# ZenGo-X/multi-party-ecdsa

Hardware: AMD Instinct MI355X
Metric: GG20 signatures/sec (t=1, n=3; all parties of each session on the node's GPUs) + Paillier-2048 modexp/s per GPU (higher is better)
Workload: dtype u32 limbs (radix 2^29) / u64 accumulators

## Files before the change

### multi_party_ecdsa_amd/csrc/mpe_gg20.h

```cpp
#pragma once
#include <cstdio>
#include <cstdlib>

#include "mpe_gg20_msg.h"
#include "mpe_gg20_nonces.h"
#include "mpe_proofs.h"

namespace mpe {
namespace smp {
struct Bounds { uint32_t *q, *q3, *Nm2, *qNt, *q3Nt; };
__global__ void bounds_kernel(int count, const uint32_t* __restrict__ N, const uint32_t* __restrict__ Nt, Bounds b) {
  const int g = blockIdx.x * blockDim.x + threadIdx.x;
  if (g > count) return;
  const uint32_t q[8] = {0xD0364141u, 0xBFD25E8Cu, 0xAF48A03Bu, 0xBAAEDCE6u, 0xFFFFFFFEu, 0xFFFFFFFFu, 0xFFFFFFFFu, 0xFFFFFFFFu};
  uint32_t q2[16], q3[24];
  sm::mul(q2, q, 8, q, 8);
  sm::mul(q3, q2, 16, q, 8);
  if (g == count) {
    for (int j = 0; j < 8; ++j) b.q[j] = q[j];
    for (int j = 0; j < 24; ++j) b.q3[j] = q3[j];
    return;
  }
  const uint32_t two[1] = {2u};
  sm::sub(b.Nm2 + (size_t)g * 64, 64, N + (size_t)g * 64, 64, two, 1);
// ... 668 lines not shown
  int st = 0;
  for (int li = 0; li < L; ++li) { const int s = pst[(size_t)li * B + b]; if (s && (!st || s < st)) st = s; }
  const size_t o = (size_t)b0 + b;
  for (int j = 0; j < 8; ++j) { r_out[o * 8 + j] = st ? 0u : pr[(size_t)b * 8 + j]; s_out[o * 8 + j] = st ? 0u : ps[(size_t)b * 8 + j]; }
  recid_out[o] = st ? 0 : prec[b];
  if (R_out) for (int j = 0; j < 16; ++j) R_out[o * 16 + j] = pR[(size_t)b * 16 + j];
  status[o] = st;
}

enum class PdlStage { idle, first_queued, ready };
struct Ahead {
  bool lockstep = false;
  uint32_t* cinv = nullptr;
  uint8_t* cinv_ok = nullptr; bool cinv_done = false;
  uint32_t* ped = nullptr;
  uint32_t *pdl_bn = nullptr, *pdl_scratch = nullptr;
  PdlStage pdl = PdlStage::idle;
};

}
}

struct mpe_gg20_session {
  mpe_ctx* ctx = nullptr;
  const mpe_gg20_keys* K = nullptr;
  int B = 0, L = 0, dedup = 0, next_round = 0;
  bool tweaked = false;
  bool any_set = false;
  uint32_t *tw = nullptr, *ty = nullptr, *tgw = nullptr;
  bool failed = false;
  mpe::gg::Dim d{};
  mpe_gg20_nonces Z{};
  void* mem = nullptr;
  size_t mem_bytes = 0;
  bool from_cache = false;
  mpe::gg::Idx ix{};
  uint32_t *kq = nullptr, *gq = nullptr, *w = nullptr, *k64 = nullptr, *g_gamma = nullptr, *com = nullptr, *c_a = nullptr, *beta = nullptr;
  uint32_t *ca_all = nullptr, *com_all = nullptr, *bpk_in = nullptr, *delta_i = nullptr, *sigma_i = nullptr, *lq = nullptr, *pedT = nullptr;
  uint32_t *tvec = nullptr, *dinv = nullptr, *R = nullptr, *Rbar = nullptr, *mq = nullptr, *rq = nullptr, *s_i = nullptr, *bad = nullptr;
  uint32_t *sig_r = nullptr, *sig_s = nullptr;
  uint32_t* miu = nullptr;
  int32_t *status = nullptr, *sig_recid = nullptr;
  int32_t *sub0_vi = nullptr, *sub4_pv = nullptr, *rdash_pv = nullptr;
  uint8_t *ok_vi = nullptr, *ok_pv = nullptr;
  mpe::gg::Ahead ahead{};
  int fault_step = 0;
  uint32_t fault_mask = 0;
  char* tmp = nullptr;
  size_t tmp_bytes = 0;
};

namespace mpe {
namespace gg {

static void gg_trace(const mpe_ctx* ctx, hipStream_t st, const char* what, int rc) {
  if (!ctx->gg20_trace) return;
  const hipError_t e = hipStreamSynchronize(st);
  fprintf(stderr, "[gg20] %-28s rc=%d sync=%s\n", what, rc, hipGetErrorString(e));
  fflush(stderr);
}
#define GG_LAUNCH(kernel, nitems, ...)                                                                   \
  do {                                                                                                    \
    if (rc == MPE_OK && (nitems) > 0)                                                                     \
      hipLaunchKernelGGL(kernel, dim3(blocks_for((int)(nitems), 64)), dim3(64), 0, st, __VA_ARGS__);      \
    gg_trace(s->ctx, st, #kernel, rc);                                                                            \
  } while (0)

static Counts counts_of(const Dim& d) { return counts_of(d.B, d.S, d.n, d.L, d.V, d.PV); }
static void dim_of_keys(Dim& d, const mpe_gg20_keys* K, const int32_t* d_keyset, const int32_t* d_sigset) {
  d.S = K->S; d.n = K->n; d.K = K->K; d.n_own = K->n_own; d.ks = d_keyset;
  d.ss = d_sigset; d.sets = K->d_sets; d.sg4 = K->sets4[0]; d.nsets = K->nsets; d.lparty = -1;
  for (int i = 0; i < 8; ++i) { d.sg[i] = K->signers[i]; d.oslot[i] = K->own_slot[i] < 0 ? 0 : K->own_slot[i]; }
}
static int local_parties(Dim& d, const mpe_gg20_keys* K, int n_local, const int32_t* h_local, const int32_t* d_sigset, int by_party) {
  if (n_local < 1 || n_local > K->S || !h_local) return MPE_E_ARG;
  d.L = n_local;
  for (int i = 0; i < 8; ++i) d.loc[i] = 0;
  if (by_party) {
    if (n_local != 1) { mpe_set_error_msg("gg20: one local party by index"); return MPE_E_ARG; }
    const int p = h_local[0];
    if (p < 0 || p >= K->n || K->own_slot[p] < 0) { mpe_set_error_msg("gg20: the local party's secrets are not in the key object"); return MPE_E_ARG; }
    if (d_sigset) { d.lparty = p; return MPE_OK; }
    for (int i = 0; i < K->S; ++i) if (K->signers[i] == p) { d.loc[0] = i; return MPE_OK; }
    mpe_set_error_msg("gg20: the local party is not a signer"); return MPE_E_ARG;
  }
  for (int i = 0; i < n_local; ++i) {
    if (h_local[i] < 0 || h_local[i] >= K->S || (i && h_local[i] <= h_local[i - 1])) return MPE_E_ARG;
    d.loc[i] = h_local[i];
    for (int k = 0; k < (d_sigset ? K->nsets : 1); ++k)
      if (K->own_slot[(K->sets4[k] >> (4 * h_local[i])) & 15u] < 0) { mpe_set_error_msg("gg20: a local party's secrets are not in the key object"); return MPE_E_ARG; }
  }
  return MPE_OK;
}
static bool small_batch(const mpe_ctx* ctx, size_t items) { return ctx->allow_par && items <= (size_t)ctx->par_items; }
static size_t ec_lanes_fit(const mpe_ctx* ctx) { return ctx->ec_lane_groups ? (size_t)ctx->cus * 4 * 64 * 2 / ctx->device_share : 0; }
static size_t layout(mpe_gg20_session* s, char* base) {
  const Dim& d = s->d;
  const Counts c = counts_of(d);
  Bump m(base);
  Idx& x = s->ix;
  x.kown_pi = m.i(c.nPI);
  x.pi_ap = m.i(c.nAP); x.kown_ap = m.i(c.nAP); x.st_ap = m.i(c.nAP);
  x.ca_vi = m.i(c.nVI); x.kpub_vi = m.i(c.nVI); x.st_vi = m.i(c.nVI);
  x.ca_mb = m.i(c.nMB); x.kpub_mb = m.i(c.nMB); x.kown_mb = m.i(c.nMB);
  x.pi_pp = m.i(c.nPP); x.kown_pp = m.i(c.nPP); x.st_pp = m.i(c.nPP);
  x.ca_pv = m.i(c.nPV); x.pi_pv = m.i(c.nPV); x.kpub_pv = m.i(c.nPV); x.st_pv = m.i(c.nPV);
  if (s->tweaked) { s->tw = m.w((size_t)d.B * 8); s->ty = m.w((size_t)d.B * 16); s->tgw = m.w((size_t)d.B * d.S * 16); }
  s->kq = m.w(c.nPI * 8); s->gq = m.w(c.nPI * 8); s->w = m.w(c.nPI * 8); s->k64 = m.w(c.nPI * 64);
  s->g_gamma = m.w(c.nPI * 16); s->com = m.w(c.nPI * 8); s->c_a = m.w(c.nPI * 128); s->beta = m.w(c.nMB * 8);
  s->ca_all = m.w(c.SB * 128); s->com_all = m.w(c.SB * 8); s->bpk_in = m.w(c.nPP * 16);
  s->delta_i = m.w(c.nPI * 8); s->sigma_i = m.w(c.nPI * 8); s->lq = m.w(c.nPI * 8); s->pedT = m.w(c.nPI * 16);
  s->tvec = m.w(c.SB * 16); s->dinv = m.w(c.nPI * 8); s->R = m.w(c.nPI * 16); s->Rbar = m.w(c.nPI * 16);
  s->mq = m.w(c.nPI * 8); s->rq = m.w(c.nPI * 8); s->s_i = m.w(c.nPI * 8); s->bad = m.w(c.nPI * NR);
  s->sig_r = m.w(c.nPI * 8); s->sig_s = m.w(c.nPI * 8); s->miu = m.w(c.nPP * 64);
  s->status = m.i(c.nPI * NR); s->sig_recid = m.i(c.nPI);
  s->sub0_vi = m.i(c.nVI); s->ok_vi = m.f(c.nVI); s->sub4_pv = m.i(c.nPV); s->rdash_pv = m.i(c.nPV); s->ok_pv = m.f(c.nPV);
  Ahead& a = s->ahead; const bool small = small_batch(s->ctx, c.nVI);
  a.cinv = small ? m.w(c.nVI * 128) : nullptr; a.cinv_ok = small ? m.f(c.nVI) : nullptr;
  a.ped = m.w(c.nPI * 48);
  a.pdl_bn = small ? m.w(c.nPP * 128) : nullptr; a.pdl_scratch = small ? m.w(modexp_nn_scratch_words(c.nPP)) : nullptr;
  s->tmp_bytes = tmp_bytes_of(c);
  s->tmp = (char*)m.take(s->tmp_bytes);
  return m.off;
}
static Slab slab_of(const mpe_gg20_session* s, const uint32_t* p, const int64_t* h_off, int round) {
  Slab sl;
  sl.p = p; sl.W = msg_words(s->d.S, s->d.n, round);
  for (int j = 0; j < 8; ++j) sl.off[j] = j < s->d.S ? (h_off ? (long long)h_off[j] : (long long)j * s->B) : 0;
  return sl;
}
static int round_enter(mpe_gg20_session* s, int round, const void* in, const void* out, bool need_in, bool need_out) {
  if (!s || (need_in && !in) || (need_out && !out)) return MPE_E_ARG;
  if (s->failed) { mpe_set_error_msg("gg20: a round call of this batch failed (or the batch was aborted): re-arm the session"); return MPE_E_ARG; }
  if (s->next_round != round) { mpe_set_error_msg("gg20: rounds must be run in order"); return MPE_E_ARG; }
  s->d.enc = s->ctx->enc;
  return MPE_OK;
}
static int round_exit(mpe_gg20_session* s, int rc, const char* what) {
  if (rc != MPE_OK) { s->failed = true; return rc; }
  const hipError_t e = hipGetLastError();
  if (e != hipSuccess) { s->failed = true; mpe_set_error(what, e); return MPE_E_HIP; }
  s->next_round++;
  return MPE_OK;
}
#define STAT(r) (s->status + (size_t)(r) * c.nPI)
#define BADR(r) (s->bad + (size_t)(r) * c.nPI)
#define PACK(nitems, per, nsub, sub0, subw, field, src)                                                                                 \
  GG_LAUNCH(pack_field_kernel, (size_t)(nitems) * (field).words, (int)(nitems), (int)(per), d.L, d.B, (int)(nsub), (int)(sub0), (int)(subw),   \
            (field).off, (const uint32_t*)(src), (field).words, s->status, s->next_round, d_out)

static bool round1_merges(const mpe_ctx* ctx, const Counts& c) {
  const bool par = small_batch(ctx, c.nVI);
  const size_t resident_groups = (size_t)ctx->cus * ctx->modexp_waves_per_cu * 16 / ctx->device_share;
  return ctx->merge_r1 && ctx->use_pair && ctx->use_multiexp && c.nVI > 0 && c.nMB > 0 && c.nVI + c.nMB < ((size_t)1 << 30) &&
         (!par || 4 * (c.nVI + c.nMB) > (size_t)ctx->merge_r1_quarters * resident_groups);
}
__global__ void ca_all_from_local_kernel(int S, int B, const uint32_t* __restrict__ c_a, uint32_t* __restrict__ ca_all) {
  const size_t g = (size_t)blockIdx.x * blockDim.x + threadIdx.x;
  if (g >= (size_t)S * B * 128) return;
  const int w = (int)(g % 128);
  const size_t jb = g / 128;
  const int ind = (int)(jb / B), b = (int)(jb % B);
  ca_all[g] = c_a[((size_t)b * S + ind) * 128 + w];
}

static bool pdl_ahead_eligible(const mpe_gg20_session* s, const Counts& c) {
  const mpe_ctx* ctx = s->ctx; const Ahead& a = s->ahead;
  return a.lockstep && a.pdl_bn && ctx->use_prio && !ctx->no_pdl_ahead && ctx->use_pair && ctx->use_crt && ctx->use_pown && c.nPP > 0 && small_batch(ctx, c.nPP);
}
static int pdl_ahead_queue(mpe_gg20_session* s, const Counts& c, bool finish) {
  mpe_ctx* ctx = s->ctx; const mpe_paillier* prv = s->K->prv; Ahead& a = s->ahead; hipStream_t sa = ctx->aux[1];
  const int phase = !finish ? 1 : (a.pdl == PdlStage::first_queued ? 2 : 0);
  const int keep = ctx->ladder_prio;
  ctx->ladder_prio = 0;
  const int rc = modexp_nn(ctx, prv, (int)c.nPP, sel_of(s->ix.kown_pp, prv->nkeys), rows(s->Z.pdl_beta, 64, nullptr, 64),
                           tab_rows(prv->N, 64, s->ix.kown_pp, prv->nkeys), 64, true, a.pdl_bn, sa, true, a.pdl_scratch, phase);
  ctx->ladder_prio = keep;
  if (rc == MPE_OK && !finish) a.pdl = PdlStage::first_queued;
  else if (rc == MPE_OK) { (void)hipEventRecord(ctx->ev_ahead, sa); a.pdl = PdlStage::ready; }
  gg_trace(ctx, sa, finish ? "PDL beta^N, ahead" : "PDL beta^N, first ladder, ahead", rc);
  return rc;
}
static Handed pdl_ahead_take(const mpe_gg20_session* s) { return s->ahead.pdl == PdlStage::ready ? Handed{s->ahead.pdl_bn, s->ctx->ev_ahead} : Handed{}; }
static void pdl_ahead_consumed(mpe_gg20_session* s) { if (s->ahead.pdl == PdlStage::ready) s->ahead.pdl = PdlStage::idle; }
static void ahead_drain(mpe_gg20_session* s, hipStream_t st) {
  mpe_ctx* ctx = s->ctx; Ahead& a = s->ahead;
  if (a.pdl == PdlStage::idle) return;
  if (a.pdl == PdlStage::first_queued) (void)hipEventRecord(ctx->ev_ahead, ctx->aux[1]);
  (void)hipStreamWaitEvent(st, ctx->ev_ahead, 0);
  a.pdl = PdlStage::idle;
}

static int round0(mpe_gg20_session* s, uint32_t* d_out, hipStream_t st) {
  int rc = round_enter(s, 0, nullptr, d_out, false, true);
  if (rc != MPE_OK) return rc;
  mpe_ctx* ctx = s->ctx; const mpe_gg20_keys* K = s->K; const Dim& d = s->d; const Counts c = counts_of(d); const mpe_gg20_nonces& Z = s->Z; Ahead& a = s->ahead;
  const int n = d.n;
  (void)hipMemsetAsync(d_out, 0, c.nPI * (size_t)msg_words(d.S, n, 0) * 4, st);
  const bool par = small_batch(ctx, c.nAP);
  const size_t nXN = c.nPI + c.nAP;
  bool all_local_in_order = d.L == d.S;
  for (int l = 0; l < d.L && all_local_in_order; ++l) all_local_in_order = d.loc[l] == l;
  const bool ahead = par && a.lockstep && a.cinv && all_local_in_order && !ctx->no_r1_inversion_ahead && round1_merges(ctx, c);
  a.cinv_done = false;
  if (par && rc == MPE_OK) rc = ws_begin(ctx, st);
  const bool held = par && rc == MPE_OK;
  WsHold hold(ctx->ws, held);
  const uint32_t *rn_pre = nullptr, *bn_pre = nullptr;
  Fork g(ctx, st, 2, held, 2);
  GG_LAUNCH(r0_kernel, c.nPI, d, K->x, Z.k, Z.gamma, Z.blind, s->kq, s->gq, s->w, s->k64, s->g_gamma, s->com, STAT(0), BADR(0));
  if (g.on) (void)hipEventRecord(ctx->ev_fork[0], st);
  GG_LAUNCH(ped_ahead_kernel, c.nPI, d, Z.l, Z.ped_s1, Z.ped_s2, a.ped);
  hipEvent_t xn_ready = nullptr;
  if (held && ctx->merge_xn) {
    hipStream_t sx = g.s(1);
    uint32_t* xs = ws_array<uint32_t>(ctx, nXN * 64);
    uint32_t* xn = ws_array<uint32_t>(ctx, nXN * 128);
    int32_t* kx = ws_array<int32_t>(ctx, nXN);
    rc = ws_ok(ctx);
    if (rc == MPE_OK) {
      (void)hipMemcpyAsync(xs, Z.r_a, c.nPI * 64 * 4, hipMemcpyDeviceToDevice, sx);
      (void)hipMemcpyAsync(xs + c.nPI * 64, Z.al_beta, c.nAP * 64 * 4, hipMemcpyDeviceToDevice, sx);
      (void)hipMemcpyAsync(kx, s->ix.kown_pi, c.nPI * 4, hipMemcpyDeviceToDevice, sx);
      (void)hipMemcpyAsync(kx + c.nPI, s->ix.kown_ap, c.nAP * 4, hipMemcpyDeviceToDevice, sx);
      rc = modexp_nn(ctx, K->prv, (int)nXN, key_selector(K->prv, kx), rows(xs, 64, nullptr, 64), key_rows(K->prv, K->prv->N, 64, kx), 64, true, xn, sx, true);
      rn_pre = xn; bn_pre = xn + c.nPI * 128;
      if (rc == MPE_OK && g.on) { (void)hipEventRecord(ctx->ev_mid, sx); xn_ready = ctx->ev_mid; }
    }
  }
  if (g.on) (void)hipStreamWaitEvent(g.s(1), ctx->ev_fork[0], 0);
  if (rc == MPE_OK) rc = paillier_encrypt(ctx, K->prv, (int)c.nPI, s->ix.kown_pi, s->k64, Z.r_a, s->c_a, true, g.s(1), rn_pre);
  gg_trace(s->ctx, st, "encrypt k", rc);
  hipEvent_t c_ready = nullptr;
  if (ahead && held && g.on && xn_ready && rc == MPE_OK) {
    hipStream_t sx = g.s(1);
    (void)hipEventRecord(ctx->ev_mid, sx); c_ready = ctx->ev_mid;
    hipLaunchKernelGGL(ca_all_from_local_kernel, dim3((unsigned)((c.SB * 128 + 255) / 256)), dim3(256), 0, sx, d.S, d.B, s->c_a, s->ca_all);
    Seq q{ctx, sx, (int)c.nVI};
    const Rows ksel = sel_of(s->ix.kpub_vi, K->pub->nkeys);
    uint8_t* ok = q.flags();
    uint32_t* cred = q.modmul(K->pub->ms_nn, ksel, rows(s->ca_all, 128, s->ix.ca_vi), rows(K->pub->ms_nn->one_words, 0, nullptr, 1));
    uint32_t* cinv = q.modinv(K->pub->ms_nn, ksel, rows(cred, 128), ok);
    rc = q.rc;
    if (rc == MPE_OK) {
      (void)hipMemcpyAsync(a.cinv, cinv, c.nVI * 128 * 4, hipMemcpyDeviceToDevice, sx);
      (void)hipMemcpyAsync(a.cinv_ok, ok, c.nVI, hipMemcpyDeviceToDevice, sx);
      a.cinv_done = true;
    }
    gg_trace(s->ctx, sx, "round 1's inversion, ahead", rc);
  }
  Bump t(s->tmp);
  const Round0Tmp r0 = Round0Tmp::carve(t, c);
  mpe_alice_proof ap{r0.z, r0.e, r0.s, r0.s1, r0.s2};
  mpe_alice_nonces an{Z.al_alpha, Z.al_beta, Z.al_gamma, Z.al_rho};
  if (rc == MPE_OK)
    rc = alice_generate(ctx, K->prv, K->stm, (int)c.nAP, s->ix.kown_ap, s->ix.st_ap, rows(s->kq, 8, s->ix.pi_ap),
                        rows(s->c_a, 128, s->ix.pi_ap), rows(Z.r_a, 64, s->ix.pi_ap), &an, &ap, st, &g, Handed{bn_pre, c_ready ? c_ready : xn_ready}, c_ready);
  g.join();
  if (rc == MPE_OK && c_ready && pdl_ahead_eligible(s, c)) { (void)hipStreamWaitEvent(ctx->aux[1], c_ready, 0); rc = pdl_ahead_queue(s, c, false); }
  gg_trace(s->ctx, st, "alice_generate", rc);
  PACK(c.nAP, n, n + 1, 0, SUB0, M0A.z, ap.z); PACK(c.nAP, n, n + 1, 0, SUB0, M0A.e, ap.e); PACK(c.nAP, n, n + 1, 0, SUB0, M0A.s, ap.s);
  PACK(c.nAP, n, n + 1, 0, SUB0, M0A.s1, ap.s1); PACK(c.nAP, n, n + 1, 0, SUB0, M0A.s2, ap.s2);
  PACK(c.nPI, 1, n + 1, n, SUB0, M0L.c, s->c_a); PACK(c.nPI, 1, n + 1, n, SUB0, M0L.com, s->com);
  return round_exit(s, rc, "gg20 round0");
}

__global__ void gather_rows_kernel(int n, Rows src, int src_words, int words, uint32_t* __restrict__ dst) {
  const size_t g = (size_t)blockIdx.x * blockDim.x + threadIdx.x;
  if (g >= (size_t)n * words) return;
  const int w = (int)(g % words), i = (int)(g / words);
  dst[g] = w < src_words ? row_of(src, i)[w] : 0u;
}
static int round1_merged_ladders(mpe_ctx* ctx, const mpe_paillier* pk, size_t nVI, const int32_t* kpub_vi, Rows cipher_vi, Rows s_vi, Rows e_vi,
                                 size_t nMB, const int32_t* kpub_mb, Rows ca_mb, const uint32_t* bsel, const uint32_t* mb_r,
                                 const uint32_t** m_vi, const uint8_t** inv_ok_vi, const uint32_t** x_mb, hipStream_t st,
                                 Handed cinv_pre = {}, const uint8_t* cinv_ok_pre = nullptr) {
  const size_t n = nVI + nMB;
  Seq q{ctx, st, (int)nVI};
  const Rows ksel = sel_of(kpub_vi, pk->nkeys);
  const uint8_t* inv_ok = cinv_ok_pre;
  const uint32_t* cinv = cinv_pre.p;
  cinv_pre.wait(st);
  if (!cinv_pre) {
    uint8_t* ok = q.flags();
    uint32_t* cred = q.modmul(pk->ms_nn, ksel, cipher_vi, rows(pk->ms_nn->one_words, 0, nullptr, 1));
    cinv = q.modinv(pk->ms_nn, ksel, rows(cred, 128), ok);
    inv_ok = ok;
  }
  if (q.rc != MPE_OK) return q.rc;
  uint32_t* b1 = ws_array<uint32_t>(ctx, n * 64);
  uint32_t* b2 = ws_array<uint32_t>(ctx, n * 128);
  uint32_t* e2 = ws_array<uint32_t>(ctx, n * 8);
  int32_t* key = ws_array<int32_t>(ctx, n);
  uint32_t* out = ws_array<uint32_t>(ctx, n * 128);
  MPE_TRY(ws_ok(ctx));
  auto gather = [&](size_t cnt, Rows src, int sw, int words, uint32_t* dst) {
    if (cnt) hipLaunchKernelGGL(gather_rows_kernel, dim3((unsigned)((cnt * words + 255) / 256)), dim3(256), 0, st, (int)cnt, src, sw, words, dst);
  };
  gather(nVI, s_vi, 64, 64, b1);              gather(nMB, rows(mb_r, 64), 64, 64, b1 + nVI * 64);
  gather(nVI, rows(cinv, 128), 128, 128, b2); gather(nMB, ca_mb, 128, 128, b2 + nVI * 128);
  gather(nVI, e_vi, 8, 8, e2);                gather(nMB, rows(bsel, 8), 8, 8, e2 + nVI * 8);
  (void)hipMemcpyAsync(key, kpub_vi, nVI * 4, hipMemcpyDeviceToDevice, st);
  (void)hipMemcpyAsync(key + nVI, kpub_mb, nMB * 4, hipMemcpyDeviceToDevice, st);
  MPE_TRY(modexp_nn2(ctx, pk, (int)n, key_selector(pk, key), rows(b1, 64, nullptr, 64), key_rows(pk, pk->N, 64, key), 64, rows(b2, 128), rows(e2, 8), 8, out, st));
  *m_vi = out; *inv_ok_vi = inv_ok; *x_mb = out + nVI * 128;
  return MPE_OK;
}

static int round1(mpe_gg20_session* s, const uint32_t* d_in, const int64_t* h_off, uint32_t* d_out, hipStream_t st) {
  int rc = round_enter(s, 1, d_in, d_out, true, true);
  if (rc != MPE_OK) return rc;
  mpe_ctx* ctx = s->ctx; const mpe_gg20_keys* K = s->K; const Dim& d = s->d; const Counts c = counts_of(d); const mpe_gg20_nonces& Z = s->Z;
  const int n = d.n, P1 = d.S - 1;
  const Slab in0 = slab_of(s, d_in, h_off, 0);
  (void)hipMemsetAsync(d_out, 0, c.nPI * (size_t)msg_words(d.S, n, 1) * 4, st);
  GG_LAUNCH(gather_field_kernel, c.SB * M0L.c.words, in0, d.S, d.B, n * SUB0 + M0L.c.off, M0L.c.words, s->ca_all);
  GG_LAUNCH(gather_field_kernel, c.SB * M0L.com.words, in0, d.S, d.B, n * SUB0 + M0L.com.off, M0L.com.words, s->com_all);
  Bump t(s->tmp);
  int32_t* sub0_vi = s->sub0_vi;
  uint8_t* ok_vi = s->ok_vi;
  const Round1Tmp r1 = Round1Tmp::carve(t, c);
  uint32_t *bsel = r1.bsel, *btq = r1.btq, *c_b = r1.c_b;
  uint32_t *Bpk = r1.Bpk, *BR = r1.BR, *Bz = r1.Bz, *BTpk = r1.BTpk, *BTR = r1.BTR, *BTz = r1.BTz;
  GG_LAUNCH(idx1_kernel, c.nVI, d, in0, sub0_vi);
  const bool par = small_batch(ctx, c.nVI);
  const bool merged = round1_merges(ctx, c);
  const bool ahead = merged && s->ahead.cinv_done;
  s->ahead.cinv_done = false;
  if ((par || merged) && rc == MPE_OK) rc = ws_begin(ctx, st);
  const bool held = (par || merged) && rc == MPE_OK;
  WsHold hold(ctx->ws, held);
  const uint32_t *m_vi = nullptr, *x_mb = nullptr;
  const uint8_t* inv_ok_vi = nullptr;
  AliceProofRows pr{rows(d_in + M0A.z.off, SUB0, sub0_vi), rows(d_in + M0A.e.off, SUB0, sub0_vi), rows(d_in + M0A.s.off, SUB0, sub0_vi),
                    rows(d_in + M0A.s1.off, SUB0, sub0_vi), rows(d_in + M0A.s2.off, SUB0, sub0_vi)};
  if (rc == MPE_OK && c.nMB > 0)
    hipLaunchKernelGGL(mb_prep_kernel, dim3(blocks_for((int)c.nMB, 64)), dim3(64), 0, st, d, s->gq, s->w, Z.mb_beta_tag, bsel, btq, s->beta);
  Fork g(ctx, st, 2, held && par, 2);
  hipEvent_t m_ready = nullptr;
  auto dlog_proofs = [&](hipStream_t sd) {
    if (rc != MPE_OK || c.nMB == 0) return;
    hipLaunchKernelGGL(dlog_prove_kernel, dim3(blocks_for((int)c.nMB, 64)), dim3(64), 0, sd, (int)c.nMB, ctx->enc, bsel, Z.mb_nonce_b, Bpk, BR, Bz);
    hipLaunchKernelGGL(dlog_prove_kernel, dim3(blocks_for((int)c.nMB, 64)), dim3(64), 0, sd, (int)c.nMB, ctx->enc, btq, Z.mb_nonce_bt, BTpk, BTR, BTz);
  };
  const bool dlog_first = ahead && g.on && !ctx->no_r1_dlog_first;
  if (dlog_first) dlog_proofs(st);
  {
    hipStream_t st2 = g.s(1);
    if (merged && rc == MPE_OK) {
      rc = round1_merged_ladders(ctx, K->pub, c.nVI, s->ix.kpub_vi, rows(s->ca_all, 128, s->ix.ca_vi), with_words(pr.s, 64), pr.e, c.nMB, s->ix.kpub_mb,
                                 rows(s->ca_all, 128, s->ix.ca_mb), bsel, Z.mb_r, &m_vi, &inv_ok_vi, &x_mb, st2,
                                 ahead ? Handed{s->ahead.cinv} : Handed{}, ahead ? s->ahead.cinv_ok : nullptr);
      if (rc == MPE_OK && g.on) { (void)hipEventRecord(ctx->ev_mid, st2); m_ready = ctx->ev_mid; }
      gg_trace(s->ctx, st2, "round 1 merged ladders", rc);
    }
    if (rc == MPE_OK)
      rc = paillier_mul_add_enc(ctx, K->pub, (int)c.nMB, s->ix.kpub_mb, rows(s->ca_all, 128, s->ix.ca_mb), rows(bsel, 8), 8, Z.mb_beta_tag,
                                Z.mb_r, c_b, st2, x_mb);
    gg_trace(s->ctx, st2, "MessageB ciphertext", rc);
    if (!dlog_first) dlog_proofs(st2);
  }
  if (rc == MPE_OK)
    rc = alice_verify(ctx, K->pub, K->stm, (int)c.nVI, s->ix.kpub_vi, s->ix.st_vi, rows(s->ca_all, 128, s->ix.ca_vi), pr, ok_vi, st, Handed{m_vi, m_ready}, inv_ok_vi);
  gg_trace(s->ctx, st, "alice_verify", rc);
  g.join();
  GG_LAUNCH(status1_kernel, c.nPI, d, ok_vi, STAT(1), BADR(1));
  const int per = 2 * P1;
  PACK(c.nMB, per, per, 0, SUB1, M1.c, c_b); PACK(c.nMB, per, per, 0, SUB1, M1.b_pk, Bpk); PACK(c.nMB, per, per, 0, SUB1, M1.b_R, BR);
  PACK(c.nMB, per, per, 0, SUB1, M1.b_z, Bz); PACK(c.nMB, per, per, 0, SUB1, M1.bt_pk, BTpk); PACK(c.nMB, per, per, 0, SUB1, M1.bt_R, BTR);
  PACK(c.nMB, per, per, 0, SUB1, M1.bt_z, BTz);
  return round_exit(s, rc, "gg20 round1");
}

static int round2(mpe_gg20_session* s, const uint32_t* d_in, const int64_t* h_off, uint32_t* d_out, hipStream_t st) {
  int rc = round_enter(s, 2, d_in, d_out, true, true);
  if (rc != MPE_OK) return rc;
  mpe_ctx* ctx = s->ctx; const mpe_gg20_keys* K = s->K; const Dim& d = s->d; const Counts c = counts_of(d); const mpe_gg20_nonces& Z = s->Z;
  const Slab in1 = slab_of(s, d_in, h_off, 1);
  (void)hipMemsetAsync(d_out, 0, c.nPI * (size_t)W2 * 4, st);
  GG_LAUNCH(validate_kernel, c.nPI, d, in1, 2, STAT(2), BADR(2));
  Bump t(s->tmp);
  const Round2Tmp r2 = Round2Tmp::carve(t, c);
  int32_t* sub1_rv = r2.sub1_rv;
  uint32_t *alpha_full = r2.alpha_full, *alpha = r2.alpha;
  uint8_t* code = r2.code;
  Ped ped{s->pedT, r2.e, r2.a1, r2.a2, r2.z1, r2.z2};
  GG_LAUNCH(idx2_kernel, c.nMB, d, in1, sub1_rv);
  const bool pdl_ahead = rc == MPE_OK && pdl_ahead_eligible(s, c) && ensure_aux(ctx);
  if (pdl_ahead) { (void)hipEventRecord(ctx->ev_fork[0], st); (void)hipStreamWaitEvent(ctx->aux[1], ctx->ev_fork[0], 0); }
  if (rc == MPE_OK)
    rc = paillier_decrypt(ctx, K->prv, (int)c.nMB, s->ix.kown_mb, rows(d_in + M1.c.off, SUB1, sub1_rv), alpha_full, st);
  gg_trace(s->ctx, st, "decrypt", rc);
  if (pdl_ahead && rc == MPE_OK) rc = pdl_ahead_queue(s, c, true);
  if (c.nMB * 4 <= ec_lanes_fit(ctx)) GG_LAUNCH(r2a_group_kernel, c.nMB * 4, d, sub1_rv, d_in, alpha_full, s->kq, K->gw, alpha, s->bpk_in, code);
  else GG_LAUNCH(r2a_kernel, c.nMB, d, sub1_rv, d_in, alpha_full, s->kq, K->gw, alpha, s->bpk_in, code);
  GG_LAUNCH(r2b_kernel, c.nPI, d, s->kq, s->gq, s->w, alpha, s->beta, code, Z.l, Z.ped_s1, Z.ped_s2, s->delta_i, s->sigma_i, s->lq, ped,
            STAT(2), BADR(2), alpha_full, s->miu, s->fault_step, s->fault_mask, s->ahead.ped);
  PACK(c.nPI, 1, 1, 0, W2, M2.delta, s->delta_i); PACK(c.nPI, 1, 1, 0, W2, M2.T, ped.T); PACK(c.nPI, 1, 1, 0, W2, M2.e, ped.e);
  PACK(c.nPI, 1, 1, 0, W2, M2.a1, ped.a1); PACK(c.nPI, 1, 1, 0, W2, M2.a2, ped.a2); PACK(c.nPI, 1, 1, 0, W2, M2.com, ped.T);
  PACK(c.nPI, 1, 1, 0, W2, M2.z1, ped.z1); PACK(c.nPI, 1, 1, 0, W2, M2.z2, ped.z2);
  return round_exit(s, rc, "gg20 round2");
}

static int round3(mpe_gg20_session* s, const uint32_t* d_in, const int64_t* h_off, uint32_t* d_out, hipStream_t st) {
  int rc = round_enter(s, 3, d_in, d_out, true, true);
  if (rc != MPE_OK) return rc;
  mpe_ctx* ctx = s->ctx; const Dim& d = s->d; const Counts c = counts_of(d);
  const Slab in2 = slab_of(s, d_in, h_off, 2);
  (void)hipMemsetAsync(d_out, 0, c.nPI * (size_t)W3 * 4, st);
  GG_LAUNCH(validate_kernel, c.nPI, d, in2, 3, STAT(3), BADR(3));
  GG_LAUNCH(gather_field_kernel, c.SB * M2.T.words, in2, d.S, d.B, M2.T.off, M2.T.words, s->tvec);
  const int g3 = 2 * d.S <= 4 ? 4 : (2 * d.S <= 8 ? 8 : 16);
  if (c.nPI * g3 <= ec_lanes_fit(ctx)) GG_LAUNCH(r3_group_kernel, c.nPI * g3, d, g3, in2, s->dinv, STAT(3), BADR(3));
  else GG_LAUNCH(r3_kernel, c.nPI, d, in2, s->dinv, STAT(3), BADR(3));
  PACK(c.nPI, 1, 1, 0, W3, M3.blind, s->Z.blind); PACK(c.nPI, 1, 1, 0, W3, M3.g_gamma, s->g_gamma);
  return round_exit(s, rc, "gg20 round3");
}

static int round4(mpe_gg20_session* s, const uint32_t* d_in, const int64_t* h_off, uint32_t* d_out, hipStream_t st) {
  int rc = round_enter(s, 4, d_in, d_out, true, true);
  if (rc != MPE_OK) return rc;
  mpe_ctx* ctx = s->ctx; const mpe_gg20_keys* K = s->K; const Dim& d = s->d; const Counts c = counts_of(d); const mpe_gg20_nonces& Z = s->Z;
  const int S = d.S, P1 = S - 1;
  const Slab in3 = slab_of(s, d_in, h_off, 3);
  (void)hipMemsetAsync(d_out, 0, c.nPI * (size_t)msg_words(S, d.n, 4) * 4, st);
  GG_LAUNCH(validate_kernel, c.nPI, d, in3, 4, STAT(4), BADR(4));
  Fork g(ctx, st, 2, small_batch(ctx, c.nPP), 2);
  hipEvent_t R_ready = nullptr;
  if (rc == MPE_OK && c.nPI > 0) {
    hipLaunchKernelGGL(r4_kernel, dim3(blocks_for((int)c.nPI, 64)), dim3(64), 0, g.s(1), d, in3, s->dinv, s->com_all, s->bpk_in, s->kq, s->R, s->Rbar,
                       STAT(4), BADR(4), g.on ? 0 : 1);
    if (g.on) {
      (void)hipEventRecord(ctx->ev_mid, g.s(1)); R_ready = ctx->ev_mid;
      hipLaunchKernelGGL(r4_rbar_kernel, dim3(blocks_for((int)c.nPI, 64)), dim3(64), 0, g.s(1), d, s->kq, s->R, s->Rbar);
    }
  }
  Bump t(s->tmp);
  const Round4Tmp r4 = Round4Tmp::carve(t, c);
  mpe_pdl_proof pp{r4.z, r4.u1, r4.u2, r4.u3, r4.s1, r4.s2, r4.s3};
  mpe_pdl_nonces pn{Z.pdl_alpha, Z.pdl_beta, Z.pdl_rho, Z.pdl_gamma};
  if (rc == MPE_OK)
    rc = pdl_prove(ctx, K->prv, K->stm, (int)c.nPP, s->ix.kown_pp, s->ix.st_pp, rows(s->c_a, 128, s->ix.pi_pp), rows(s->Rbar, 16, s->ix.pi_pp),
                   rows(s->R, 16, s->ix.pi_pp), rows(s->kq, 8, s->ix.pi_pp), rows(Z.r_a, 64, s->ix.pi_pp), &pn, &pp, st, &g,
                   pdl_ahead_take(s), R_ready);
  else g.join();
  if (rc == MPE_OK) pdl_ahead_consumed(s);
  gg_trace(s->ctx, st, "pdl_prove", rc);
  PACK(c.nPP, P1, S, 0, SUB4, M4P.z, pp.z); PACK(c.nPP, P1, S, 0, SUB4, M4P.u1, pp.u1); PACK(c.nPP, P1, S, 0, SUB4, M4P.u2, pp.u2);
  PACK(c.nPP, P1, S, 0, SUB4, M4P.u3, pp.u3); PACK(c.nPP, P1, S, 0, SUB4, M4P.s1, pp.s1); PACK(c.nPP, P1, S, 0, SUB4, M4P.s2, pp.s2);
  PACK(c.nPP, P1, S, 0, SUB4, M4P.s3, pp.s3);
  PACK(c.nPI, 1, S, P1, SUB4, M4R.R_dash, s->Rbar);
  return round_exit(s, rc, "gg20 round4");
}

static int round5(mpe_gg20_session* s, const uint32_t* d_in, const int64_t* h_off, uint32_t* d_out, hipStream_t st) {
  int rc = round_enter(s, 5, d_in, d_out, true, true);
  if (rc != MPE_OK) return rc;
  mpe_ctx* ctx = s->ctx; const mpe_gg20_keys* K = s->K; const Dim& d = s->d; const Counts c = counts_of(d); const mpe_gg20_nonces& Z = s->Z;
  const Slab in4 = slab_of(s, d_in, h_off, 4);
  (void)hipMemsetAsync(d_out, 0, c.nPI * (size_t)W5 * 4, st);
  GG_LAUNCH(validate_kernel, c.nPI, d, in4, 5, STAT(5), BADR(5));
  Bump t(s->tmp);
  int32_t *sub4_pv = s->sub4_pv, *rdash_pv = s->rdash_pv;
  uint8_t* ok_pv = s->ok_pv;
  const Round5Tmp r5 = Round5Tmp::carve(t, c);
  Heg heg{r5.S, r5.T, r5.A3, r5.z1, r5.z2};
  GG_LAUNCH(idx5_kernel, c.nPV, d, in4, sub4_pv, rdash_pv);
  const bool par = small_batch(ctx, c.nPV);
  PdlProofRows pr{rows(d_in + M4P.z.off, SUB4, sub4_pv), rows(d_in + M4P.u1.off, SUB4, sub4_pv), rows(d_in + M4P.u2.off, SUB4, sub4_pv),
                  rows(d_in + M4P.u3.off, SUB4, sub4_pv), rows(d_in + M4P.s1.off, SUB4, sub4_pv), rows(d_in + M4P.s2.off, SUB4, sub4_pv),
                  rows(d_in + M4P.s3.off, SUB4, sub4_pv)};
  Fork g(ctx, st, 2, par, 2);
  if (rc == MPE_OK && c.nPI > 0)
    hipLaunchKernelGGL(r5_prove_kernel, dim3(blocks_for((int)c.nPI, 64)), dim3(64), 0, g.s(1), d, s->R, s->sigma_i, s->lq, s->pedT, Z.heg_s1, Z.heg_s2, heg);
  if (rc == MPE_OK)
    rc = pdl_verify(ctx, K->pub, K->stm, (int)c.nPV, s->ix.kpub_pv, s->ix.st_pv, rows(s->ca_all, 128, s->ix.ca_pv), rows(d_in + M4R.R_dash.off, SUB4, rdash_pv),
                    rows(s->R, 16, s->ix.pi_pv), pr, ok_pv, st);
  gg_trace(s->ctx, st, "pdl_verify", rc);
  g.join();
  GG_LAUNCH(r5_status_kernel, c.nPI, d, in4, ok_pv, STAT(5), BADR(5));
  PACK(c.nPI, 1, 1, 0, W5, M5.S, heg.S); PACK(c.nPI, 1, 1, 0, W5, M5.T, heg.T); PACK(c.nPI, 1, 1, 0, W5, M5.A3, heg.A3);
  PACK(c.nPI, 1, 1, 0, W5, M5.z1, heg.z1); PACK(c.nPI, 1, 1, 0, W5, M5.z2, heg.z2);
  return round_exit(s, rc, "gg20 round5");
}

static int round6(mpe_gg20_session* s, const uint32_t* d_in, const int64_t* h_off, hipStream_t st) {
  int rc = round_enter(s, 6, d_in, nullptr, true, false);
  if (rc != MPE_OK) return rc;
  mpe_ctx* ctx = s->ctx; const Dim& d = s->d; const Counts c = counts_of(d);
  const Slab in5 = slab_of(s, d_in, h_off, 5);
  GG_LAUNCH(validate_kernel, c.nPI, d, in5, 6, STAT(6), BADR(6));
  const int g6 = 3 * d.S <= 8 ? 8 : (3 * d.S <= 16 ? 16 : 32);
  if (c.nPI * g6 <= ec_lanes_fit(ctx)) GG_LAUNCH(r6_group_kernel, c.nPI * g6, d, g6, in5, s->R, s->tvec, s->K->y, STAT(6), BADR(6));
  else GG_LAUNCH(r6_kernel, c.nPI, d, in5, s->R, s->tvec, s->K->y, STAT(6), BADR(6));
  return round_exit(s, rc, "gg20 round6");
}

static int round7(mpe_gg20_session* s, const uint32_t* d_msg, uint32_t* d_out, hipStream_t st) {
  int rc = round_enter(s, 7, d_msg, d_out, true, true);
  if (rc != MPE_OK) return rc;
  const Dim& d = s->d; const Counts c = counts_of(d);
  GG_LAUNCH(r7_kernel, c.nPI, d, d_msg, s->R, s->kq, s->sigma_i, s->mq, s->rq, s->s_i, s->fault_step, s->fault_mask);
  PACK(c.nPI, 1, 1, 0, W6, M7.s_i, s->s_i);
  return round_exit(s, rc, "gg20 round7");
}
static int complete(mpe_gg20_session* s, const uint32_t* d_in, const int64_t* h_off, hipStream_t st) {
  int rc = round_enter(s, 8, d_in, nullptr, true, false);
  if (rc != MPE_OK) return rc;
  const Dim& d = s->d; const Counts c = counts_of(d);
  const Slab in6 = slab_of(s, d_in, h_off, 7);
  GG_LAUNCH(complete_kernel, c.nPI, d, in6, s->R, s->mq, s->rq, s->s_i, s->K->y, s->status, s->bad, s->sig_r, s->sig_s, s->sig_recid);
  return round_exit(s, rc, "gg20 complete");
}

static void launch_idx(mpe_gg20_session* s, hipStream_t st) {
  const Counts c = counts_of(s->d);
  size_t total = 0;
  for (const size_t v : {c.nVI, c.nMB, c.nAP, c.nPV, c.nPI}) if (v > total) total = v;
  hipLaunchKernelGGL(idx_kernel, dim3(blocks_for((int)total, 64)), dim3(64), 0, st, s->d, s->ix, (int)total);
}
static void launch_tweaks(mpe_gg20_session* s, const uint32_t* d_tweak, hipStream_t st) {
  Dim& d = s->d;
  d.tw = d.ty = d.tgw = nullptr;
  if (!d_tweak) return;
  (void)hipMemcpyAsync(s->tw, d_tweak, (size_t)d.B * 32, hipMemcpyDeviceToDevice, st);
  hipLaunchKernelGGL(tweak_kernel, dim3(blocks_for(d.B * (d.S + 1), 64)), dim3(64), 0, st, d, s->tw, s->K->gw, s->K->y, s->tgw, s->ty);
  d.tw = s->tw; d.ty = s->ty; d.tgw = s->tgw;
}
static hipError_t wipe_batch_state(mpe_gg20_session* s, hipStream_t st) {
  ahead_drain(s, st);
  return hipMemsetAsync(s->kq, 0, (size_t)((char*)s->mem + s->mem_bytes - (char*)s->kq), st);
}

static void session_release(mpe_gg20_session* s, hipStream_t st) {
  if (!s) return;
  ahead_drain(s, st);
  if (s->mem) {
    (void)hipMemsetAsync(s->mem, 0, s->mem_bytes, st);
    if (s->from_cache) s->ctx->sess_in_use = false;
    else { (void)hipStreamSynchronize(st); (void)hipFree(s->mem); }
  }
  delete s;
}

}
}

extern "C" {

int mpe_gg20_keys_create(mpe_ctx* ctx, int t, int n, int n_signers, const int32_t* h_signers, int nkeysets, int n_own,
                         const int32_t* h_own, const uint32_t* d_x, const uint32_t* d_p, const uint32_t* d_q, const uint32_t* d_N,
                         const uint32_t* d_Nt, const uint32_t* d_h1, const uint32_t* d_h2, const uint32_t* d_y, const uint32_t* d_X,
                         mpe_gg20_keys** out, void* stream) {
  return mpe_gg20_keys_create_sets(ctx, t, n, n_signers, 1, h_signers, nkeysets, n_own, h_own, d_x, d_p, d_q, d_N, d_Nt, d_h1, d_h2, d_y, d_X, out, stream);
}

int mpe_gg20_keys_create_sets(mpe_ctx* ctx, int t, int n, int n_signers, int n_sets, const int32_t* h_sets, int nkeysets, int n_own,
                              const int32_t* h_own, const uint32_t* d_x, const uint32_t* d_p, const uint32_t* d_q, const uint32_t* d_N,
                              const uint32_t* d_Nt, const uint32_t* d_h1, const uint32_t* d_h2, const uint32_t* d_y, const uint32_t* d_X,
                              mpe_gg20_keys** out, void* stream) {
  const int32_t* h_signers = h_sets;
  if (!ctx || !h_signers || !h_own || !d_x || !d_p || !d_q || !d_N || !d_Nt || !d_h1 || !d_h2 || !d_y || !d_X || !out) return MPE_E_ARG;
  if (n < 2 || n > 8 || n_signers < 2 || n_signers > n || t < 1 || n_signers <= t || nkeysets < 1 || n_own < 1 || n_own > n) return MPE_E_ARG;
  if (n_sets < 1 || n_sets > 256) return MPE_E_ARG;
  uint32_t sets4[256], masks[256];
  for (int k = 0; k < n_sets; ++k) {
    const int32_t* row = h_sets + (size_t)k * n_signers;
    sets4[k] = 0; masks[k] = 0;
    for (int i = 0; i < n_signers; ++i) {
      if (row[i] < 0 || row[i] >= n || (i && row[i] <= row[i - 1])) return MPE_E_ARG;
      sets4[k] |= (uint32_t)row[i] << (4 * i); masks[k] |= 1u << row[i];
    }
    for (int m = 0; m < k; ++m) if (sets4[m] == sets4[k]) { mpe_set_error_msg("gg20 keys: two equal signer sets"); return MPE_E_ARG; }
  }
  for (int i = 0; i < n_own; ++i)
    if (h_own[i] < 0 || h_own[i] >= n || (i && h_own[i] <= h_own[i - 1])) return MPE_E_ARG;
  hipStream_t st = (hipStream_t)stream;
  mpe_gg20_keys* K = new (std::nothrow) mpe_gg20_keys();
  if (!K) return MPE_E_NOMEM;
  K->t = t; K->n = n; K->S = n_signers; K->K = nkeysets; K->n_own = n_own; K->nsets = n_sets;
  for (int k = 0; k < n_sets; ++k) { K->sets4[k] = sets4[k]; K->masks[k] = masks[k]; }
  for (int a = 0; a < 8; ++a) K->own_slot[a] = -1;
  for (int i = 0; i < n_signers; ++i) K->signers[i] = h_signers[i];
  for (int i = 0; i < n_own; ++i) { K->own[i] = h_own[i]; K->own_slot[h_own[i]] = i; }
  const size_t kk = (size_t)nkeysets;
  const size_t ngw = kk * n_sets * n_signers;
  const size_t words = kk * n_own * 8 + kk * n * 16 + kk * 16 + ngw * 16 + 32 + kk * n * (64 + 72 + 88) + 2 * (size_t)n_sets;
  hipError_t e = hipMalloc(&K->blob, words * 4);
  if (e != hipSuccess) { delete K; mpe_set_error("hipMalloc(gg20 keys)", e); return MPE_E_NOMEM; }
  K->blob_bytes = words * 4;
  K->x = (uint32_t*)K->blob; K->X = K->x + kk * n_own * 8; K->y = K->X + kk * n * 16; K->gw = K->y + kk * 16;
  K->bounds.q = K->gw + ngw * 16; K->bounds.q3 = K->bounds.q + 8; K->bounds.Nm2 = K->bounds.q3 + 24;
  K->bounds.qNt = K->bounds.Nm2 + kk * n * 64; K->bounds.q3Nt = K->bounds.qNt + kk * n * 72;
  K->d_sets = K->bounds.q3Nt + kk * n * 88;
  (void)hipMemcpyAsync(K->d_sets, K->sets4, (size_t)n_sets * 4, hipMemcpyHostToDevice, st);
  (void)hipMemcpyAsync(K->d_sets + n_sets, K->masks, (size_t)n_sets * 4, hipMemcpyHostToDevice, st);
  hipLaunchKernelGGL(mpe::smp::bounds_kernel, dim3(mpe::blocks_for(nkeysets * n + 1, 64)), dim3(64), 0, st, nkeysets * n, d_N, d_Nt, K->bounds);
  (void)hipMemcpyAsync(K->x, d_x, kk * n_own * 8 * 4, hipMemcpyDeviceToDevice, st);
  (void)hipMemcpyAsync(K->X, d_X, kk * n * 16 * 4, hipMemcpyDeviceToDevice, st);
  (void)hipMemcpyAsync(K->y, d_y, kk * 16 * 4, hipMemcpyDeviceToDevice, st);
  {
    mpe::gg::Dim d{};
    d.S = n_signers; d.n = n; d.K = nkeysets; d.nsets = n_sets; d.sets = K->d_sets; d.lparty = -1;
    hipLaunchKernelGGL(mpe::gg::gw_kernel, dim3(mpe::blocks_for((int)ngw, 64)), dim3(64), 0, st, d, K->X, K->gw);
  }
  int rc = mpe_paillier_create_public(ctx, nkeysets * n, d_N, &K->pub, stream);
  if (rc == MPE_OK) rc = mpe_paillier_create_private(ctx, nkeysets * n_own, d_p, d_q, &K->prv, stream);
// ... 282 lines not shown
```

### multi_party_ecdsa_amd/csrc/mpe_internal.h

```cpp
#pragma once
#include <hip/hip_runtime.h>
#include <stdint.h>
#include <new>
#include <utility>
#include <string>
#include <vector>

#include "../../include/mpecdsa_hip.h"
#include "mpe_kernels_heavy.h"
#include "mpe_sched.h"
#include "mpe_ws.h"

void mpe_set_error(const char* what, hipError_t e);
void mpe_set_error_msg(const char* what);

namespace mpe {
struct WsHip {
  static void* alloc(size_t bytes) {
    void* p = nullptr;
    const hipError_t e = hipMalloc(&p, bytes);
    if (e != hipSuccess) { mpe_set_error("hipMalloc(workspace)", e); return nullptr; }
    return p;
  }
  static void free(void* p) { (void)hipFree(p); }
  static void zero(void* p, size_t bytes, void* stream) { (void)hipMemsetAsync(p, 0, bytes, (hipStream_t)stream); }
  static void sync(void* stream) { (void)hipStreamSynchronize((hipStream_t)stream); }
};
}

struct mpe_ctx {
  int device = 0;
  int cus = 256;
  int fb_window_bits = 13;
  int window_bits = 0;
  bool ec_lane_groups = true;
  bool adaptive_lanes = true;
  bool use_pown = true;
  bool use_pair = true;
  bool use_multiexp = true;
  bool use_crt = true;
  bool use_fixed_base = true;
  bool use_sliding = true;
  int wide_div = 4;
  int device_share = 1;
  int xwide_div = 16;
  bool merge_xn = true;
  int use_prio = 1;
  int ladder_prio = 1;
  int use_crt_n = 1;
  int no_pdl_ahead = 0;
  int no_r1_dlog_first = 0;
  int no_r1_inversion_ahead = 0;
  int merge_r1_quarters = 1;
  bool merge_r1 = true;
  size_t fb_budget_bytes = 0;
  int modexp_waves_per_cu = 8;
  int fb_split = 0;
  int gg20_trace = 0;
  int safe_pass_log = 24;
  int sampler_max_attempts = 128;
  int no_primaries = 0;
  int no_elect = 0;
  int grid_mode = 2;
  void* tables[4] = {nullptr, nullptr, nullptr, nullptr};
  size_t tables_bytes[4] = {0, 0, 0, 0};
  hipStream_t aux[3] = {nullptr, nullptr, nullptr};
  hipEvent_t ev_fork[2] = {nullptr, nullptr}, ev_join[3] = {nullptr, nullptr, nullptr};
  hipEvent_t ev_ahead = nullptr;
  hipEvent_t ev_mid = nullptr;
  bool aux_ready = false;
  bool allow_par = true;
  int par_items = 32768;
  mpe::WsArena<mpe::WsHip> ws;
  void* sess_buf = nullptr;
  size_t sess_bytes = 0;
  bool sess_in_use = false;
  void* slab_buf = nullptr;
  size_t slab_bytes = 0;
  mpe_launch_info last = {};
  long long search_counts[9] = {0, 0, 0, 0, 0, 0, 0, 0, 0};
  mpe_encoding enc = {};
  bool prof_on = false;
  struct ProfEvt { hipEvent_t a, b; int kind, bits, exp_words, batch, exp2_words; int wave_trips; };
  std::vector<ProfEvt> prof;
  uint32_t* prof_ctr = nullptr;
  int prof_ctr_cap = 0;
};

struct mpe_modset {
  int bits = 0;
  int count = 0;
  int K = 0;
  void* blob = nullptr;
  uint32_t* n_limbs = nullptr;
  uint32_t* one_limbs = nullptr;
  uint32_t* r2_limbs = nullptr;
  uint32_t* r2h_limbs = nullptr;
  uint32_t* n0inv = nullptr;
  uint32_t* words = nullptr;
  uint32_t* one_words = nullptr;
};

struct mpe_pairset {
  int half_bits = 0;
  int count = 0;
  void* blob = nullptr;
  uint32_t *n_limbs = nullptr, *n0inv = nullptr, *one = nullptr, *r2 = nullptr, *tp = nullptr, *kc = nullptr;
  const uint32_t* mod_words = nullptr;
};

namespace mpe {

inline Rows rows(const uint32_t* p, int stride, const int32_t* idx = nullptr, int words = 0) {
  return Rows{p, idx, stride, words};
}
inline Rows no_rows() { return Rows{nullptr, nullptr, 0, 0}; }

int launch_modexp(mpe_ctx* ctx, const mpe_modset* ms, int batch, Rows mod_sel, Rows base_lo, Rows base_hi, Rows exps,
                  int exp_words, uint32_t* out, hipStream_t st);
int launch_modexp2(mpe_ctx* ctx, const mpe_modset* ms, int batch, Rows mod_sel, Rows base, Rows exps, int exp_words,
                   Rows base2, Rows exps2, int exp2_words, uint32_t* out, hipStream_t st);
int launch_modmul(mpe_ctx* ctx, const mpe_modset* ms, int batch, Rows mod_sel, Rows a, Rows b, uint32_t* out,
                  hipStream_t st);
int modset_create_dev(mpe_ctx* ctx, int bits, int count, const uint32_t* d_moduli, mpe_modset** out, hipStream_t st);

void ctx_copy_options(mpe_ctx* dst, const mpe_ctx* src);
void prof_begin(mpe_ctx* ctx, hipStream_t st, int kind, int bits, int exp_words, int batch, int exp2_words = 0);
void prof_end(mpe_ctx* ctx, hipStream_t st);
uint32_t* prof_counter(mpe_ctx* ctx, int wave_trips);

int pairset_create_2048(int count, const uint32_t* d_moduli, mpe_pairset** out, hipStream_t st);
int pairset_create_1024(int count, const uint32_t* d_moduli, mpe_pairset** out, hipStream_t st);
int pair_modexp_2048(mpe_ctx* ctx, const mpe_pairset* ps, int batch, Rows mod_sel, Rows base, Rows exps, int exp_words,
                     Rows base2, Rows exps2, int exp2_words, int half, uint32_t* out, hipStream_t st, int public_exp);
int pair_modexp_1024(mpe_ctx* ctx, const mpe_pairset* ps, int batch, Rows mod_sel, Rows base, Rows exps, int exp_words,
                     Rows base2, Rows exps2, int exp2_words, int half, uint32_t* out, hipStream_t st, int public_exp);

inline int ws_begin(mpe_ctx* ctx, hipStream_t st) { return ctx->ws.begin(st) ? MPE_OK : MPE_E_NOMEM; }
inline void* ws_alloc(mpe_ctx* ctx, size_t bytes) { return ctx->ws.alloc(bytes); }
inline int ws_ok(const mpe_ctx* ctx) { return ctx->ws.failed ? MPE_E_NOMEM : MPE_OK; }
using WsHold = WsArena<WsHip>::Hold;
using WsKeep = WsArena<WsHip>::Keep;
uint32_t* tables_for(mpe_ctx* ctx, size_t need, hipStream_t st);
bool ensure_aux(mpe_ctx* ctx);

struct Fork {
  mpe_ctx* ctx; hipStream_t main; int n, first; bool on;
  Fork(mpe_ctx* c, hipStream_t m, int branches, bool enable, int first_aux = 0);
  hipStream_t s(int i) const { return (on && i > 0) ? ctx->aux[first + i - 1] : main; }
  void join();
  void branch_done_wait(int i, hipStream_t waiter);
};
template <class T>
inline T* ws_array(mpe_ctx* ctx, size_t count) { return (T*)ws_alloc(ctx, count * sizeof(T)); }

inline int blocks_for(int n, int threads) { return (n + threads - 1) / threads; }

inline int persistent_grid(const mpe_ctx* ctx, int need, int cap);
inline int ladder_grid(const mpe_ctx* ctx, int units, int cap) {
  if (ctx->no_elect) return persistent_grid(ctx, units, cap);
  if (units <= cap) return (2 * units <= cap && !ctx->no_primaries) ? 2 * units : units;
  return cap;
}
inline SchedArgs ladder_sched(const mpe_ctx* ctx, int units, int cap, int32_t* state, hipStream_t st) {
  SchedArgs a{nullptr, SCHED_STATIC, units, ctx->use_prio ? ctx->ladder_prio : 0};
  if (ctx->no_elect || !state) return a;
  if (2 * units <= cap) { if (!ctx->no_primaries) { a.state = state; a.mode = SCHED_PRIMARIES; } }
  else if (units > cap) { a.state = state; a.mode = SCHED_ALL; }
  if (a.state) (void)hipMemsetAsync(a.state, 0, SCHED_WORDS * sizeof(int32_t), st);
  return a;
}
inline int persistent_grid(const mpe_ctx* ctx, int need, int cap) {
  if (need <= cap) return need;
  const int rem = need % cap;
  if (rem == 0) return cap;
  if (ctx->grid_mode == 1 || (ctx->grid_mode == 2 && 2 * rem <= cap)) return cap;
  const int trips = (need + cap - 1) / cap;
  return (need + trips - 1) / trips;
}

}
```

### multi_party_ecdsa_amd/csrc/mpe_lib.hip

```cpp
#include <string.h>
#include <array>
#include <initializer_list>
#include <mutex>
#include "mpe_internal.h"
#include "mpe_ec.h"

using namespace mpe;

thread_local std::string g_last_error;
void mpe_set_error(const char* what, hipError_t e) { g_last_error = std::string(what) + ": " + hipGetErrorString(e); }
void mpe_set_error_msg(const char* what) { g_last_error = what; }

namespace mpe {

static int slot_of(const mpe_ctx* ctx, hipStream_t st) {
  for (int i = 0; i < 3; ++i) if (ctx->aux[i] && st == ctx->aux[i]) return i + 1;
  return 0;
}
uint32_t* tables_for(mpe_ctx* ctx, size_t need, hipStream_t st) {
  const int sl = slot_of(ctx, st);
  if (need > ctx->tables_bytes[sl]) {
    if (ctx->tables[sl]) { (void)hipStreamSynchronize(st); (void)hipFree(ctx->tables[sl]); ctx->tables[sl] = nullptr; ctx->tables_bytes[sl] = 0; }
    hipError_t e = hipMalloc(&ctx->tables[sl], need);
    if (e != hipSuccess) { mpe_set_error("hipMalloc(window tables)", e); return nullptr; }
    ctx->tables_bytes[sl] = need;
  }
  return (uint32_t*)ctx->tables[sl];
}
bool ensure_aux(mpe_ctx* ctx) {
  if (ctx->aux_ready) return true;
  for (int i = 0; i < 3; ++i) if (hipStreamCreateWithFlags(&ctx->aux[i], hipStreamNonBlocking) != hipSuccess) return false;
  for (int i = 0; i < 2; ++i) if (hipEventCreateWithFlags(&ctx->ev_fork[i], hipEventDisableTiming) != hipSuccess) return false;
  for (int i = 0; i < 3; ++i) if (hipEventCreateWithFlags(&ctx->ev_join[i], hipEventDisableTiming) != hipSuccess) return false;
  if (hipEventCreateWithFlags(&ctx->ev_mid, hipEventDisableTiming) != hipSuccess) return false;
  if (hipEventCreateWithFlags(&ctx->ev_ahead, hipEventDisableTiming) != hipSuccess) return false;
  ctx->aux_ready = true;
  return true;
}
Fork::Fork(mpe_ctx* c, hipStream_t m, int branches, bool enable, int first_aux) : ctx(c), main(m), n(branches), first(first_aux) {
  on = enable && c->allow_par && branches > 1 && first_aux + branches - 1 <= 3 && ensure_aux(c);
  if (!on) return;
  hipEvent_t ev = c->ev_fork[first_aux ? 1 : 0];
  (void)hipEventRecord(ev, m);
  for (int i = 1; i < n; ++i) (void)hipStreamWaitEvent(c->aux[first + i - 1], ev, 0);
}
void Fork::branch_done_wait(int i, hipStream_t waiter) {
  if (!on || i <= 0 || waiter == ctx->aux[first + i - 1]) return;
  (void)hipEventRecord(ctx->ev_join[first + i - 1], ctx->aux[first + i - 1]);
  (void)hipStreamWaitEvent(waiter, ctx->ev_join[first + i - 1], 0);
}
void Fork::join() {
  if (!on) return;
  for (int i = 1; i < n; ++i) {
    (void)hipEventRecord(ctx->ev_join[first + i - 1], ctx->aux[first + i - 1]);
    (void)hipStreamWaitEvent(main, ctx->ev_join[first + i - 1], 0);
  }
}

void prof_begin(mpe_ctx* ctx, hipStream_t st, int kind, int bits, int exp_words, int batch, int exp2_words) {
  if (!ctx->prof_on) return;
  mpe_ctx::ProfEvt ev;
  ev.kind = kind; ev.bits = bits; ev.exp_words = exp_words; ev.batch = batch; ev.exp2_words = exp2_words; ev.wave_trips = 0;
  (void)hipEventCreate(&ev.a);
  (void)hipEventCreate(&ev.b);
  (void)hipEventRecord(ev.a, st);
  ctx->prof.push_back(ev);
}
uint32_t* prof_counter(mpe_ctx* ctx, int wave_trips) {
  if (!ctx->prof_on || ctx->prof.empty() || !ctx->prof_ctr || (int)ctx->prof.size() > ctx->prof_ctr_cap) return nullptr;
  ctx->prof.back().wave_trips = wave_trips;
  return ctx->prof_ctr + (ctx->prof.size() - 1);
}
void prof_end(mpe_ctx* ctx, hipStream_t st) {
  if (ctx->prof_on && !ctx->prof.empty()) (void)hipEventRecord(ctx->prof.back().b, st);
}

static ModsetView view_of(const mpe_modset* ms) {
  ModsetView v;
  v.n_limbs = ms->n_limbs; v.one_limbs = ms->one_limbs; v.r2_limbs = ms->r2_limbs; v.r2h_limbs = ms->r2h_limbs;
  v.n0inv = ms->n0inv; v.count = ms->count;
  return v;
}

template <class C>
static int grid_for(const mpe_ctx* ctx, int batch, int waves_per_cu) {
  return persistent_grid(ctx, (batch + C::GROUPS - 1) / C::GROUPS, ctx->cus * waves_per_cu);
}

template <class C>
static int modset_create_impl(int count, const uint32_t* d_moduli, mpe_modset** out, hipStream_t st) {
  mpe_modset* ms = new (std::nothrow) mpe_modset();
  if (!ms) return MPE_E_NOMEM;
  ms->bits = C::BITS;
  ms->count = count;
  ms->K = C::K;
  const size_t words = (size_t)count * C::K;
  const size_t iw = (size_t)count * C::K32;
  const size_t total = (4 * words + (size_t)count + iw + 4) * sizeof(uint32_t);
  hipError_t e = hipMalloc(&ms->blob, total);
  if (e != hipSuccess) { delete ms; mpe_set_error("hipMalloc(modset)", e); return MPE_E_NOMEM; }
  uint32_t* p = (uint32_t*)ms->blob;
  ms->n_limbs = p;
  ms->one_limbs = p + words;
  ms->r2_limbs = p + 2 * words;
  ms->r2h_limbs = p + 3 * words;
  ms->n0inv = p + 4 * words;
  ms->words = ms->n0inv + count;
  ms->one_words = ms->words + iw;
  (void)hipMemcpyAsync(ms->words, d_moduli, iw * sizeof(uint32_t), hipMemcpyDeviceToDevice, st);
  (void)hipMemsetD32Async((hipDeviceptr_t)ms->one_words, 1, 1, st);
  const int blocks = (count + C::GROUPS - 1) / C::GROUPS;
  hipLaunchKernelGGL(modset_setup_kernel<C>, dim3(blocks), dim3(64), 0, st, count, d_moduli, ms->n_limbs,
                     ms->one_limbs, ms->r2_limbs, ms->r2h_limbs, ms->n0inv);
  e = hipGetLastError();
  if (e != hipSuccess) { (void)hipFree(ms->blob); delete ms; mpe_set_error("modset_setup_kernel", e); return MPE_E_HIP; }
  *out = ms;
  return MPE_OK;
}

int modset_create_dev(mpe_ctx* ctx, int bits, int count, const uint32_t* d_moduli, mpe_modset** out, hipStream_t st) {
  (void)ctx;
  if (bits == 4096) return modset_create_impl<Cfg4096>(count, d_moduli, out, st);
  if (bits == 2048) return modset_create_impl<Cfg2048>(count, d_moduli, out, st);
  return MPE_E_ARG;
}

template <class C>
static int modexp_impl(mpe_ctx* ctx, const mpe_modset* ms, int batch, Rows mod_sel, Rows base_lo, Rows base_hi, Rows exps,
                       int exp_words, Rows base2, Rows exps2, int exp2_words, uint32_t* d_out, hipStream_t st) {
  const int units = (batch + C::GROUPS - 1) / C::GROUPS, cap = ctx->cus * ctx->modexp_waves_per_cu;
  const int grid = ladder_grid(ctx, units, cap);
  int wb = exp_words <= 8 ? 4 : (exp_words < 48 ? 5 : 6);
  if (ctx->window_bits) wb = ctx->window_bits;
  const bool dual = base2.p != nullptr;
  if (dual && (base_hi.p != nullptr || exp2_words <= 0 || 32 * exp2_words > ((exp_words * 32 + wb - 1) / wb - 1) * wb)) {
    mpe_set_error_msg("modexp: the second exponent must be shorter than the first");
    return MPE_E_ARG;
  }
  const size_t need = (size_t)grid * C::GROUPS * (((size_t)1 << wb) + (dual ? 16 : 0)) * C::K * sizeof(uint32_t);
  uint32_t* tabs = tables_for(ctx, need + SCHED_WORDS * sizeof(int32_t), st);
  if (!tabs) return MPE_E_NOMEM;
  const SchedArgs sched = ladder_sched(ctx, units, cap, (int32_t*)((char*)tabs + need), st);
  prof_begin(ctx, st, 0, C::BITS, exp_words, batch, dual ? exp2_words : 0);
  hipLaunchKernelGGL(modexp_kernel<C>, dim3(grid), dim3(64), 0, st, batch, view_of(ms), mod_sel, base_lo, base_hi, exps,
                     exp_words, wb, base2, exps2, exp2_words, d_out, tabs, sched);
  prof_end(ctx, st);
  hipError_t e = hipGetLastError();
  if (e != hipSuccess) { mpe_set_error("modexp_kernel", e); return MPE_E_HIP; }
  ctx->last.waves = grid;
  ctx->last.ints_per_wave = C::GROUPS;
  ctx->last.limbs = C::K;
  ctx->last.limb_bits = C::W;
  ctx->last.lds_bytes_per_wave = C::LDS_WORDS * 4;
  ctx->last.table_scratch_bytes = need;
  return MPE_OK;
}

int launch_modexp2(mpe_ctx* ctx, const mpe_modset* ms, int batch, Rows mod_sel, Rows base, Rows exps, int exp_words,
                   Rows base2, Rows exps2, int exp2_words, uint32_t* out, hipStream_t st) {
  if (batch == 0) return MPE_OK;
  if (ms->bits == 4096)
    return modexp_impl<Cfg4096>(ctx, ms, batch, mod_sel, base, no_rows(), exps, exp_words, base2, exps2, exp2_words, out, st);
  if (ms->bits == 2048)
    return modexp_impl<Cfg2048>(ctx, ms, batch, mod_sel, base, no_rows(), exps, exp_words, base2, exps2, exp2_words, out, st);
  return MPE_E_ARG;
}
int launch_modexp(mpe_ctx* ctx, const mpe_modset* ms, int batch, Rows mod_sel, Rows base_lo, Rows base_hi, Rows exps,
                  int exp_words, uint32_t* out, hipStream_t st) {
  if (batch == 0) return MPE_OK;
  if (ms->bits == 4096)
    return modexp_impl<Cfg4096>(ctx, ms, batch, mod_sel, base_lo, base_hi, exps, exp_words, no_rows(), no_rows(), 0, out, st);
  if (ms->bits == 2048)
    return modexp_impl<Cfg2048>(ctx, ms, batch, mod_sel, base_lo, base_hi, exps, exp_words, no_rows(), no_rows(), 0, out, st);
  return MPE_E_ARG;
}

template <class C>
static int modmul_impl(mpe_ctx* ctx, const mpe_modset* ms, int batch, Rows mod_sel, Rows a, Rows b, uint32_t* d_out,
                       hipStream_t st) {
  const int grid = grid_for<C>(ctx, batch, 16);
  prof_begin(ctx, st, 1, C::BITS, 0, batch);
  hipLaunchKernelGGL(modmul_kernel<C>, dim3(grid), dim3(64), 0, st, batch, view_of(ms), mod_sel, a, b, d_out);
  prof_end(ctx, st);
  hipError_t e = hipGetLastError();
  if (e != hipSuccess) { mpe_set_error("modmul_kernel", e); return MPE_E_HIP; }
  return MPE_OK;
}

int launch_modmul(mpe_ctx* ctx, const mpe_modset* ms, int batch, Rows mod_sel, Rows a, Rows b, uint32_t* out,
                  hipStream_t st) {
  if (batch == 0) return MPE_OK;
  if (ms->bits == 4096) return modmul_impl<Cfg4096>(ctx, ms, batch, mod_sel, a, b, out, st);
  if (ms->bits == 2048) return modmul_impl<Cfg2048>(ctx, ms, batch, mod_sel, a, b, out, st);
  return MPE_E_ARG;
}

static Rows mod_selector(const mpe_modset* ms, const int32_t* d_mod_idx) {
  return Rows{nullptr, d_mod_idx, (d_mod_idx == nullptr && ms->count != 1) ? 1 : 0, 0};
}

}

#include "mpe_small.h"

namespace mpe {
static void pairset_free(mpe_pairset* ps) {
  if (!ps) return;
  if (ps->blob) (void)hipFree(ps->blob);
  delete ps;
}
static int pairset_create(int half_bits, int count, const uint32_t* d_moduli, mpe_pairset** out, hipStream_t st) {
  if (half_bits == 2048) return pairset_create_2048(count, d_moduli, out, st);
  if (half_bits == 1024) return pairset_create_1024(count, d_moduli, out, st);
  return MPE_E_ARG;
}
static int launch_pair_modexp(mpe_ctx* ctx, const mpe_pairset* ps, int batch, Rows mod_sel, Rows base, Rows exps, int exp_words,
                              Rows base2, Rows exps2, int exp2_words, uint32_t* out, hipStream_t st, int half = 0, int public_exp = 0) {
  if (batch == 0) return MPE_OK;
  if (ps->half_bits == 2048)
    return pair_modexp_2048(ctx, ps, batch, mod_sel, base, exps, exp_words, base2, exps2, exp2_words, half, out, st, public_exp);
  if (ps->half_bits == 1024)
    return pair_modexp_1024(ctx, ps, batch, mod_sel, base, exps, exp_words, base2, exps2, exp2_words, half, out, st, public_exp);
  return MPE_E_ARG;
}
}
#include "mpe_paillier.h"
#include "mpe_proofs.h"
#include "mpe_mta.h"
#include "mpe_bob.h"
#include "mpe_gg20.h"
#include "mpe_presig.h"
#include "mpe_sample.h"
#include "mpe_seal.h"
#include "mpe_sha512.h"
#include "mpe_bip32.h"
#include "mpe_pipeline.h"
#include "mpe_comm.h"
#include "mpe_sigma.h"
#include "mpe_blame.h"
#include "mpe_keygen.h"
#include "mpe_keygen_deal.h"
#include "mpe_primes.h"
#include "mpe_lindell.h"
#include "mpe_lindell_keygen.h"
#include "mpe_gg18.h"

extern "C" {

const char* mpe_version(void) { return "mpecdsa-hip 0.7.0 (gfx950)"; }
const char* mpe_last_error(void) { return g_last_error.c_str(); }

void mpe_encoding_default(mpe_encoding* e) {
  if (!e) return;
  memset(e, 0, sizeof *e);
  e->ck_salt = 0x4B5A656Eu;
  for (int i = 0; i < 4; ++i) e->ord_dlog[i] = e->ord_cdlog[i] = (uint8_t)i;
  for (int i = 0; i < 8; ++i) e->ord_pedersen[i] = e->ord_heg[i] = e->ord_ecddh[i] = (uint8_t)i;
}
static bool is_perm(const uint8_t* o, int n) {
  unsigned seen = 0;
  for (int i = 0; i < n; ++i) { if (o[i] >= n || (seen >> o[i]) & 1u) return false; seen |= 1u << o[i]; }
  return true;
}
int mpe_ctx_set_encoding(mpe_ctx* ctx, const mpe_encoding* e) {
  if (!ctx || !e) return MPE_E_ARG;
  if (e->chain_point > 1 || e->zero_bytes > 1 || e->ck_mask_order > 1 || e->reserved != 0 || !is_perm(e->ord_dlog, 3) ||
      !is_perm(e->ord_pedersen, 5) || !is_perm(e->ord_heg, 7) || !is_perm(e->ord_ecddh, 6) || !is_perm(e->ord_cdlog, 4)) {
    mpe_set_error_msg("mpe_ctx_set_encoding: a flag is not 0/1 or an order is not a permutation");
    return MPE_E_ARG;
  }
  ctx->enc = *e;
  return MPE_OK;
}
int mpe_ctx_set_device_share(mpe_ctx* ctx, int contexts) {
  if (!ctx || contexts < 1 || contexts > 64) return MPE_E_ARG;
  ctx->device_share = contexts;
  return MPE_OK;
}
int mpe_ctx_get_encoding(const mpe_ctx* ctx, mpe_encoding* out) {
  if (!ctx || !out) return MPE_E_ARG;
  *out = ctx->enc;
  return MPE_OK;
}

namespace mpe {
struct CtxOption {
  const char* key;
  long lo, hi;
  void (*set)(mpe_ctx*, long);
  long (*get)(const mpe_ctx*);
};
#define MPE_OPT_BOOL_OFF(name, field) {name, 0, 1, [](mpe_ctx* c, long v) { c->field = !v; }, [](const mpe_ctx* c) -> long { return c->field ? 0 : 1; }}
#define MPE_OPT_INT(name, lo, hi, field) {name, lo, hi, [](mpe_ctx* c, long v) { c->field = (decltype(c->field))v; }, [](const mpe_ctx* c) -> long { return (long)c->field; }}
static const CtxOption kCtxOptions[] = {
    MPE_OPT_BOOL_OFF("no_fixed_base", use_fixed_base),
    MPE_OPT_BOOL_OFF("no_crt", use_crt),
    MPE_OPT_BOOL_OFF("no_multiexp", use_multiexp),
    MPE_OPT_BOOL_OFF("no_pair", use_pair),
    MPE_OPT_BOOL_OFF("no_pown", use_pown),
    MPE_OPT_BOOL_OFF("no_sliding", use_sliding),
    MPE_OPT_BOOL_OFF("no_par", allow_par),
    MPE_OPT_BOOL_OFF("no_wide", adaptive_lanes),
    MPE_OPT_BOOL_OFF("no_ec_lane_groups", ec_lane_groups),
    MPE_OPT_BOOL_OFF("no_merge_xn", merge_xn),
    MPE_OPT_BOOL_OFF("no_merge_r1", merge_r1),
    MPE_OPT_INT("fb_window_bits", 4, 16, fb_window_bits),
    MPE_OPT_INT("window_bits", 0, 6, window_bits),
    MPE_OPT_INT("wide_div", 1, 64, wide_div),
    MPE_OPT_INT("merge_r1_quarters", 0, 64, merge_r1_quarters),
    MPE_OPT_INT("no_r1_inversion_ahead", 0, 1, no_r1_inversion_ahead),
    MPE_OPT_BOOL_OFF("no_prio", use_prio),
    MPE_OPT_INT("no_pdl_ahead", 0, 1, no_pdl_ahead),
    MPE_OPT_BOOL_OFF("no_crt_n", use_crt_n),
    MPE_OPT_INT("no_r1_dlog_first", 0, 1, no_r1_dlog_first),
    MPE_OPT_INT("xwide_div", 0, 1 << 20, xwide_div),
    MPE_OPT_INT("waves_per_cu", 1, 8, modexp_waves_per_cu),
    MPE_OPT_INT("grid_mode", 0, 2, grid_mode),
    MPE_OPT_INT("fb_split", 0, 64, fb_split),
    MPE_OPT_INT("gg20_trace", 0, 1, gg20_trace),
    MPE_OPT_INT("sampler_max_attempts", 1, 1 << 20, sampler_max_attempts),
    MPE_OPT_INT("safe_pass_log", 16, 26, safe_pass_log),
    MPE_OPT_INT("no_primaries", 0, 1, no_primaries),
    MPE_OPT_INT("no_elect", 0, 1, no_elect),
    {"fb_budget_mb", 0, 1 << 20, [](mpe_ctx* c, long v) { c->fb_budget_bytes = (size_t)v << 20; }, [](const mpe_ctx* c) -> long { return (long)(c->fb_budget_bytes >> 20); }},
};
#undef MPE_OPT_BOOL_OFF
#undef MPE_OPT_INT
extern "C++" void ctx_copy_options(mpe_ctx* dst, const mpe_ctx* src) {
  for (const CtxOption& o : kCtxOptions) o.set(dst, o.get(src));
}
}

int mpe_ctx_set_option(mpe_ctx* ctx, const char* key, const char* value) {
  if (!ctx || !key || !value) return MPE_E_ARG;
  if (!strcmp(key, "grid")) {
    const int m = !strcmp(value, "equal") ? 0 : (!strcmp(value, "full") ? 1 : (!strcmp(value, "hybrid") ? 2 : -1));
    if (m < 0) { mpe_set_error_msg("mpe_ctx_set_option: grid = equal | full | hybrid"); return MPE_E_ARG; }
    ctx->grid_mode = m;
    return MPE_OK;
  }
  if (!strcmp(key, "no_adaptive_lanes")) {
    const bool off = atoi(value) != 0;
    ctx->adaptive_lanes = !off; ctx->ec_lane_groups = !off;
    return MPE_OK;
  }
  for (const mpe::CtxOption& o : mpe::kCtxOptions) {
    if (strcmp(key, o.key)) continue;
    char* end = nullptr;
    const long v = strtol(value, &end, 10);
    if (end == value || *end || v < o.lo || v > o.hi) {
      mpe_set_error_msg((std::string("mpe_ctx_set_option: ") + key + " takes an integer in [" + std::to_string(o.lo) + ", " + std::to_string(o.hi) + "]").c_str());
      return MPE_E_ARG;
    }
    if (!strcmp(key, "window_bits") && v == 1) { mpe_set_error_msg("mpe_ctx_set_option: window_bits takes 0 (auto) or 2..6"); return MPE_E_ARG; }
    o.set(ctx, v);
    return MPE_OK;
  }
  mpe_set_error_msg((std::string("mpe_ctx_set_option: unknown option ") + key).c_str());
  return MPE_E_ARG;
}
int mpe_ctx_get_option(const mpe_ctx* ctx, const char* key, long* value) {
  if (!ctx || !key || !value) return MPE_E_ARG;
  for (const mpe::CtxOption& o : mpe::kCtxOptions)
    if (!strcmp(key, o.key)) { *value = o.get(ctx); return MPE_OK; }
  return MPE_E_ARG;
}
int mpe_ctx_option_count(void) { return (int)(sizeof(mpe::kCtxOptions) / sizeof(mpe::kCtxOptions[0])); }
const char* mpe_ctx_option_name(int i) { return (i >= 0 && i < mpe_ctx_option_count()) ? mpe::kCtxOptions[i].key : nullptr; }

int mpe_ctx_create(mpe_ctx** out, int device) {
  if (!out) return MPE_E_ARG;
  hipError_t e = hipSetDevice(device);
  if (e != hipSuccess) { mpe_set_error("hipSetDevice", e); return MPE_E_HIP; }
  hipDeviceProp_t prop;
  e = hipGetDeviceProperties(&prop, device);
  if (e != hipSuccess) { mpe_set_error("hipGetDeviceProperties", e); return MPE_E_HIP; }
  mpe_ctx* c = new (std::nothrow) mpe_ctx();
  if (!c) return MPE_E_NOMEM;
  c->device = device;
  c->cus = prop.multiProcessorCount;
  mpe_encoding_default(&c->enc);
  static std::once_flag comb_once[64];
  static hipError_t comb_err[64];
  if (device < 0 || device >= 64) { delete c; return MPE_E_ARG; }
  std::call_once(comb_once[device], [device]() {
    hipLaunchKernelGGL(mpe::ec::ec_comb_build_kernel, dim3(2), dim3(64), 0, 0);
    comb_err[device] = hipDeviceSynchronize();
  });
  e = comb_err[device];
  if (e != hipSuccess) { mpe_set_error("ec_comb_build_kernel", e); delete c; return MPE_E_HIP; }
  *out = c;
  return MPE_OK;
}

struct CtxBuf { void* p; size_t bytes; };
static std::vector<CtxBuf> ctx_bufs(const mpe_ctx* ctx, bool all) {
  std::vector<CtxBuf> b;
  for (int i = 0; i < 4; ++i) b.push_back({ctx->tables[i], ctx->tables_bytes[i]});
  for (const auto& blk : ctx->ws.blocks) b.push_back({blk.p, blk.bytes});
  if (all) { b.push_back({ctx->sess_buf, ctx->sess_bytes}); b.push_back({ctx->slab_buf, ctx->slab_bytes}); }
  return b;
}

int mpe_ctx_wipe(mpe_ctx* ctx, void* stream) {
  if (!ctx) return MPE_E_ARG;
  hipStream_t st = (hipStream_t)stream;
  for (const CtxBuf& b : ctx_bufs(ctx, false)) if (b.p) (void)hipMemsetAsync(b.p, 0, b.bytes, st);
  const hipError_t e = hipGetLastError();
  if (e != hipSuccess) { mpe_set_error("mpe_ctx_wipe", e); return MPE_E_HIP; }
  return MPE_OK;
}

__global__ void count_nonzero_kernel(const uint32_t* __restrict__ p, size_t words, unsigned long long* __restrict__ out) {
  size_t g = (size_t)blockIdx.x * blockDim.x + threadIdx.x;
  const size_t step = (size_t)gridDim.x * blockDim.x;
  unsigned long long c = 0;
  for (; g < words; g += step) c += p[g] != 0u;
  if (c) atomicAdd(out, c);
}
int mpe_ctx_scratch_audit(mpe_ctx* ctx, uint64_t* nonzero_words, uint64_t* total_bytes, void* stream) {
  if (!ctx || !nonzero_words) return MPE_E_ARG;
  hipStream_t st = (hipStream_t)stream;
  unsigned long long* d = nullptr;
  hipError_t e = hipMalloc((void**)&d, 8);
  if (e != hipSuccess) { mpe_set_error("hipMalloc(audit)", e); return MPE_E_NOMEM; }
  (void)hipMemsetAsync(d, 0, 8, st);
  uint64_t tot = 0;
  for (const CtxBuf& b : ctx_bufs(ctx, true)) {
    if (!b.p || !b.bytes) continue;
    tot += b.bytes;
    hipLaunchKernelGGL(count_nonzero_kernel, dim3(4096), dim3(256), 0, st, (const uint32_t*)b.p, b.bytes / 4, d);
  }
  unsigned long long h = 0;
  e = hipMemcpyAsync(&h, d, 8, hipMemcpyDeviceToHost, st);
  if (e == hipSuccess) e = hipStreamSynchronize(st);
  (void)hipFree(d);
  if (e != hipSuccess) { mpe_set_error("mpe_ctx_scratch_audit", e); return MPE_E_HIP; }
  *nonzero_words = h;
  if (total_bytes) *total_bytes = tot;
  return MPE_OK;
}

int mpe_ctx_destroy(mpe_ctx* ctx) {
  if (!ctx) return MPE_E_ARG;
  for (const CtxBuf& b : ctx_bufs(ctx, true)) if (b.p) (void)hipMemsetAsync(b.p, 0, b.bytes, nullptr);
  (void)hipDeviceSynchronize();
  for (const CtxBuf& b : ctx_bufs(ctx, true)) if (b.p) (void)hipFree(b.p);
  if (ctx->aux_ready) {
    for (int i = 0; i < 3; ++i) { (void)hipStreamDestroy(ctx->aux[i]); (void)hipEventDestroy(ctx->ev_join[i]); }
    for (int i = 0; i < 2; ++i) (void)hipEventDestroy(ctx->ev_fork[i]);
    if (ctx->ev_mid) (void)hipEventDestroy(ctx->ev_mid);
    if (ctx->ev_ahead) (void)hipEventDestroy(ctx->ev_ahead);
  }
  for (auto& ev : ctx->prof) { (void)hipEventDestroy(ev.a); (void)hipEventDestroy(ev.b); }
  if (ctx->prof_ctr) (void)hipFree(ctx->prof_ctr);
  delete ctx;
  return MPE_OK;
}

int mpe_sync(mpe_ctx* ctx, void* stream) {
  (void)ctx;
  hipError_t e = hipStreamSynchronize((hipStream_t)stream);
  if (e != hipSuccess) { mpe_set_error("hipStreamSynchronize", e); return MPE_E_HIP; }
  return MPE_OK;
}

int mpe_last_launch_info(const mpe_ctx* ctx, mpe_launch_info* out) {
  if (!ctx || !out) return MPE_E_ARG;
  *out = ctx->last;
  return MPE_OK;
}

int mpe_prof_enable(mpe_ctx* ctx, int on) {
  if (!ctx) return MPE_E_ARG;
  for (auto& ev : ctx->prof) { (void)hipEventDestroy(ev.a); (void)hipEventDestroy(ev.b); }
  ctx->prof.clear();
  ctx->prof_on = on != 0;
  if (ctx->prof_on) {
    if (!ctx->prof_ctr) {
      ctx->prof_ctr_cap = 1 << 16;
      if (hipMalloc((void**)&ctx->prof_ctr, (size_t)ctx->prof_ctr_cap * sizeof(uint32_t)) != hipSuccess) { ctx->prof_ctr = nullptr; ctx->prof_ctr_cap = 0; }
    }
    if (ctx->prof_ctr) (void)hipMemset(ctx->prof_ctr, 0, (size_t)ctx->prof_ctr_cap * sizeof(uint32_t));
  }
  return MPE_OK;
}

int mpe_prof_collect(mpe_ctx* ctx, mpe_prof_rec* out, int max_records, int* n_out) {
  if (!ctx || !out || !n_out) return MPE_E_ARG;
  int n = 0;
  std::vector<uint32_t> ctr;
  size_t ix = 0;
  if (ctx->prof_ctr && !ctx->prof.empty()) (void)hipDeviceSynchronize();
  for (auto& ev : ctx->prof) {
    const size_t my = ix++;
    if (n >= max_records) break;
    if (hipEventSynchronize(ev.b) != hipSuccess) continue;
    float ms = 0.f;
    if (hipEventElapsedTime(&ms, ev.a, ev.b) != hipSuccess) continue;
    if (ctr.empty() && ctx->prof_ctr) {
      ctr.resize(ctx->prof.size() < (size_t)ctx->prof_ctr_cap ? ctx->prof.size() : (size_t)ctx->prof_ctr_cap);
      if (hipMemcpy(ctr.data(), ctx->prof_ctr, ctr.size() * sizeof(uint32_t), hipMemcpyDeviceToHost) != hipSuccess) ctr.assign(ctr.size(), 0u);
    }
    out[n].kind = ev.kind; out[n].bits = ev.bits; out[n].exp_words = ev.exp_words; out[n].batch = ev.batch; out[n].ms = ms;
    out[n].exp2_words = ev.exp2_words;
    out[n].sliding_frac = (ev.wave_trips > 0 && my < ctr.size()) ? (float)ctr[my] / (float)ev.wave_trips : (ev.kind == 6 ? -1.f : 0.f);
    ++n;
  }
  *n_out = n;
  return MPE_OK;
}

int mpe_modset_count(const mpe_modset* ms) { return ms ? ms->count : MPE_E_ARG; }
int mpe_modset_bits(const mpe_modset* ms) { return ms ? ms->bits : MPE_E_ARG; }

int mpe_modset_destroy(mpe_modset* ms) {
  if (!ms) return MPE_E_ARG;
  if (ms->blob) (void)hipFree(ms->blob);
  delete ms;
  return MPE_OK;
}

int mpe_modset_create(mpe_ctx* ctx, int bits, int count, const uint32_t* d_moduli, mpe_modset** out, void* stream) {
  if (!ctx || !out || !d_moduli || count <= 0) return MPE_E_ARG;
  return modset_create_dev(ctx, bits, count, d_moduli, out, (hipStream_t)stream);
// ... 33 lines not shown
```

### multi_party_ecdsa_amd/csrc/mpe_paillier.h

```cpp
#pragma once
#include "mpe_internal.h"
#include "mpe_small.h"

struct mpe_paillier {
  int nkeys = 0;
  bool has_private = false;
  void* blob = nullptr;
  uint32_t* N = nullptr;
  uint32_t* NN = nullptr;
  mpe_modset* ms_nn = nullptr;
  mpe_modset* ms_n = nullptr;
  uint32_t* pq32 = nullptr;
  uint32_t* pq64 = nullptr;
  uint32_t* sq64 = nullptr;
  uint32_t* em1 = nullptr;
  uint32_t* em2 = nullptr;
  uint32_t* inv2 = nullptr;
  uint32_t* h64 = nullptr;
  uint32_t* ab64 = nullptr;
  uint32_t* eq1 = nullptr;
  uint32_t* ecrt = nullptr;
  uint32_t* e128 = nullptr;
  int32_t* swap_idx = nullptr;
  mpe_modset* ms_pp = nullptr;
  mpe_modset* ms_p = nullptr;
  mpe_pairset* ps_nn = nullptr;
  mpe_pairset* ps_pp = nullptr;
};

namespace mpe {

__device__ __forceinline__ int key_of(const int32_t* key_idx, int nkeys, int i) {
  return key_idx ? key_idx[i] : (nkeys == 1 ? 0 : i);
}

__global__ void pk_square_kernel(int nk, const uint32_t* __restrict__ N, uint32_t* __restrict__ NN) {
  const int k = blockIdx.x * blockDim.x + threadIdx.x;
  if (k >= nk) return;
  uint32_t n[64], r[128];
  sm::copy(n, N + (size_t)k * 64, 64);
  sm::mul(r, n, 64, n, 64);
  sm::copy(NN + (size_t)k * 128, r, 128);
}

__global__ void sk_setup_a_kernel(int nk, const uint32_t* __restrict__ p, const uint32_t* __restrict__ q,
                                  uint32_t* __restrict__ N, uint32_t* __restrict__ pq32, uint32_t* __restrict__ pq64,
                                  uint32_t* __restrict__ sq64, uint32_t* __restrict__ em1, uint32_t* __restrict__ em2,
                                  uint32_t* __restrict__ inv2, uint32_t* __restrict__ ecrt, uint32_t* __restrict__ eq1,
                                  int32_t* __restrict__ swap_idx) {
  const int j = blockIdx.x * blockDim.x + threadIdx.x;
  if (j >= 2 * nk) return;
  const int k = j >> 1;
  uint32_t x[32], y[32], r[64], t1[32], t2[32], one[1] = {1}, two[1] = {2};
  sm::copy(x, ((j & 1) ? q : p) + (size_t)k * 32, 32);
  sm::copy(y, ((j & 1) ? p : q) + (size_t)k * 32, 32);
  sm::copy(pq32 + (size_t)j * 32, x, 32);
  sm::copy(pq64 + (size_t)j * 64, x, 32);
  sm::zero(pq64 + (size_t)j * 64 + 32, 32);
  sm::mul(r, x, 32, x, 32);
  sm::copy(sq64 + (size_t)j * 64, r, 64);
  sm::sub(t1, 32, x, 32, one, 1);
  sm::copy(em1 + (size_t)j * 32, t1, 32);
  {
    uint32_t e[32];
    sm::copy(e, y, 32);
    for (int it = 0; it < 3; ++it)
      if (sm::cmp(e, 32, t1, 32) >= 0) sm::sub(e, 32, e, 32, t1, 32);
    sm::copy(eq1 + (size_t)j * 32, e, 32);
  }
  sm::mul(r, x, 32, t1, 32);
  sm::sub(r, 64, r, 64, one, 1);
  sm::copy(ecrt + (size_t)j * 64, r, 64);
  sm::sub(t1, 32, x, 32, two, 1);
  sm::copy(em2 + (size_t)j * 32, t1, 32);
  uint32_t iv[32];
  sm::inv2adic(iv, x, 32, t1, t2);
  sm::copy(inv2 + (size_t)j * 32, iv, 32);
  swap_idx[j] = j ^ 1;
  if ((j & 1) == 0) {
    sm::mul(r, x, 32, y, 32);
    sm::copy(N + (size_t)k * 64, r, 64);
  }
}

__global__ void sk_setup_b_kernel(int nk2, const uint32_t* __restrict__ pq32, const uint32_t* __restrict__ inv_other,
                                  uint32_t* __restrict__ h64, uint32_t* __restrict__ ab64) {
  const int j = blockIdx.x * blockDim.x + threadIdx.x;
  if (j >= nk2) return;
  uint32_t x[32], y[32], iv[32], r[64];
  sm::copy(x, pq32 + (size_t)j * 32, 32);
  sm::copy(y, pq32 + (size_t)(j ^ 1) * 32, 32);
  sm::copy(iv, inv_other + (size_t)j * 64, 32);
  sm::sub(r, 32, x, 32, iv, 32);
  sm::copy(h64 + (size_t)j * 64, r, 32);
  sm::zero(h64 + (size_t)j * 64 + 32, 32);
  sm::mul(r, y, 32, iv, 32);
  sm::copy(ab64 + (size_t)j * 64, r, 64);
}

__global__ void sk_setup_c_kernel(int nk2, const uint32_t* __restrict__ sq64, const uint32_t* __restrict__ inv_sq,
                                  uint32_t* __restrict__ e128) {
  const int j = blockIdx.x * blockDim.x + threadIdx.x;
  if (j >= nk2) return;
  uint32_t a[64], b[64], r[128];
  sm::copy(a, sq64 + (size_t)(j ^ 1) * 64, 64);
  sm::copy(b, inv_sq + (size_t)j * 64, 64);
  sm::mul(r, a, 64, b, 64);
  sm::copy(e128 + (size_t)j * 128, r, 128);
}

__global__ void crt_half_kernel(int B2, Rows ksel, int32_t* __restrict__ half_of) {
  MPE_FOREGROUND();
  const int j = blockIdx.x * blockDim.x + threadIdx.x;
  if (j >= B2) return;
  half_of[j] = 2 * sel_index(ksel, j >> 1) + (j & 1);
}
__global__ void crt_add_kernel(int B, Rows ksel, const uint32_t* __restrict__ NN, const uint32_t* __restrict__ y,
                               uint32_t* __restrict__ out) {
  MPE_FOREGROUND();
  const int i = blockIdx.x * blockDim.x + threadIdx.x;
  if (i >= B) return;
  uint32_t a[129], b[128];
  sm::copy(a, y + (size_t)(2 * i) * 128, 128);
  sm::copy(b, y + (size_t)(2 * i + 1) * 128, 128);
  a[128] = sm::add(a, 128, a, 128, b, 128);
  sm::copy(b, NN + (size_t)sel_index(ksel, i) * 128, 128);
  if (sm::cmp(a, 129, b, 128) >= 0) sm::sub(a, 129, a, 129, b, 128);
  sm::copy(out + (size_t)i * 128, a, 128);
}

__global__ void enc_gm_kernel(int B, int nkeys, const uint32_t* __restrict__ m, const int32_t* __restrict__ key_idx,
                              const uint32_t* __restrict__ N, uint32_t* __restrict__ gm) {
  const int i = blockIdx.x * blockDim.x + threadIdx.x;
  if (i >= B) return;
  uint32_t a[64], n[64], r[128], one[1] = {1};
  sm::copy(a, m + (size_t)i * 64, 64);
  sm::copy(n, N + (size_t)key_of(key_idx, nkeys, i) * 64, 64);
  sm::mul(r, a, 64, n, 64);
  sm::add(r, 128, r, 128, one, 1);
  sm::copy(gm + (size_t)i * 128, r, 128);
}

__global__ void dec_index_kernel(int B2, int nkeys, const int32_t* __restrict__ key_idx, int32_t* __restrict__ item_of,
                                 int32_t* __restrict__ half_of, int32_t* __restrict__ keyj) {
  MPE_FOREGROUND();
  const int j = blockIdx.x * blockDim.x + threadIdx.x;
  if (j >= B2) return;
  const int i = j >> 1, k = key_of(key_idx, nkeys, i);
  item_of[j] = i;
  half_of[j] = 2 * k + (j & 1);
  keyj[j] = k;
}
__global__ void dec_lfunc_kernel(int B2, const uint32_t* __restrict__ u, const int32_t* __restrict__ half_of,
                                 const uint32_t* __restrict__ inv2, uint32_t* __restrict__ t) {
  MPE_FOREGROUND();
  const int j = blockIdx.x * blockDim.x + threadIdx.x;
  if (j >= B2) return;
  uint32_t a[32], iv[32], r[32], one[1] = {1};
  sm::copy(a, u + (size_t)j * 64, 32);
  sm::sub(a, 32, a, 32, one, 1);
  sm::copy(iv, inv2 + (size_t)half_of[j] * 32, 32);
  sm::mullo(r, a, iv, 32);
  sm::copy(t + (size_t)j * 32, r, 32);
}
__global__ void dec_combine_kernel(int B, int nkeys, const uint32_t* __restrict__ y, const int32_t* __restrict__ key_idx,
                                   const uint32_t* __restrict__ N, uint32_t* __restrict__ m) {
  MPE_FOREGROUND();
  const int i = blockIdx.x * blockDim.x + threadIdx.x;
  if (i >= B) return;
  uint32_t a[65], b[64], n[64];
  sm::copy(a, y + (size_t)(2 * i) * 64, 64);
  sm::copy(b, y + (size_t)(2 * i + 1) * 64, 64);
  sm::copy(n, N + (size_t)key_of(key_idx, nkeys, i) * 64, 64);
  a[64] = sm::add(a, 64, a, 64, b, 64);
  if (sm::cmp(a, 65, n, 64) >= 0) sm::sub(a, 65, a, 65, n, 64);
  sm::copy(m + (size_t)i * 64, a, 64);
}

#define MPE_LAUNCH_1D(kernel, n, st, ...)                                                        \
  do {                                                                                            \
    if ((n) > 0) {                                                                                \
      hipLaunchKernelGGL(kernel, dim3(blocks_for((n), 64)), dim3(64), 0, st, __VA_ARGS__);        \
      hipError_t e_ = hipGetLastError();                                                          \
      if (e_ != hipSuccess) { mpe_set_error(#kernel, e_); return MPE_E_HIP; }                     \
    }                                                                                             \
  } while (0)
#define MPE_TRY(expr) do { int rc_ = (expr); if (rc_ != MPE_OK) return rc_; } while (0)

static void paillier_free(mpe_paillier* pk) {
  if (!pk) return;
  if (pk->ms_nn) mpe_modset_destroy(pk->ms_nn);
  if (pk->ms_n) mpe_modset_destroy(pk->ms_n);
  if (pk->ms_pp) mpe_modset_destroy(pk->ms_pp);
  if (pk->ms_p) mpe_modset_destroy(pk->ms_p);
  pairset_free(pk->ps_nn);
  pairset_free(pk->ps_pp);
  if (pk->blob) (void)hipFree(pk->blob);
  delete pk;
}

static int paillier_create(mpe_ctx* ctx, int nk, const uint32_t* d_N, const uint32_t* d_p, const uint32_t* d_q,
                           mpe_paillier** out, hipStream_t st) {
  mpe_paillier* pk = new (std::nothrow) mpe_paillier();
  if (!pk) return MPE_E_NOMEM;
  pk->nkeys = nk;
  pk->has_private = d_p != nullptr;
  const size_t nk2 = 2 * (size_t)nk;
  size_t words = (size_t)nk * (64 + 128);
  if (pk->has_private) words += nk2 * (32 + 64 + 64 + 32 + 32 + 32 + 64 + 64 + 64 + 128 + 32 + 1);
  hipError_t e = hipMalloc(&pk->blob, words * 4);
  if (e != hipSuccess) { delete pk; mpe_set_error("hipMalloc(paillier keys)", e); return MPE_E_NOMEM; }
  uint32_t* w = (uint32_t*)pk->blob;
  pk->N = w; w += (size_t)nk * 64;
  pk->NN = w; w += (size_t)nk * 128;
  int rc = MPE_OK;
  auto fail = [&](int code) { paillier_free(pk); return code; };
  if (pk->has_private) {
    pk->pq32 = w; w += nk2 * 32;
    pk->pq64 = w; w += nk2 * 64;
    pk->sq64 = w; w += nk2 * 64;
    pk->em1 = w; w += nk2 * 32;
    pk->em2 = w; w += nk2 * 32;
    pk->inv2 = w; w += nk2 * 32;
    pk->h64 = w; w += nk2 * 64;
    pk->ab64 = w; w += nk2 * 64;
    pk->ecrt = w; w += nk2 * 64;
    pk->eq1 = w; w += nk2 * 32;
    pk->e128 = w; w += nk2 * 128;
    pk->swap_idx = (int32_t*)w; w += nk2;
    hipLaunchKernelGGL(sk_setup_a_kernel, dim3(blocks_for((int)nk2, 64)), dim3(64), 0, st, nk, d_p, d_q, pk->N, pk->pq32,
                       pk->pq64, pk->sq64, pk->em1, pk->em2, pk->inv2, pk->ecrt, pk->eq1, pk->swap_idx);
    if ((rc = modset_create_dev(ctx, 2048, (int)nk2, pk->sq64, &pk->ms_pp, st)) != MPE_OK) return fail(rc);
    if ((rc = modset_create_dev(ctx, 2048, (int)nk2, pk->pq64, &pk->ms_p, st)) != MPE_OK) return fail(rc);
    if ((rc = ws_begin(ctx, st)) != MPE_OK) return fail(rc);
    uint32_t* inv_other = ws_array<uint32_t>(ctx, nk2 * 64);
    uint32_t* inv_sq = ws_array<uint32_t>(ctx, nk2 * 64);
    if ((rc = ws_ok(ctx)) != MPE_OK) return fail(rc);
    rc = launch_modexp(ctx, pk->ms_p, (int)nk2, rows(nullptr, 1), rows(pk->pq32, 32, pk->swap_idx, 32), no_rows(),
                       rows(pk->em2, 32), 32, inv_other, st);
    if (rc != MPE_OK) return fail(rc);
    hipLaunchKernelGGL(sk_setup_b_kernel, dim3(blocks_for((int)nk2, 64)), dim3(64), 0, st, (int)nk2, pk->pq32, inv_other,
                       pk->h64, pk->ab64);
    rc = launch_modexp(ctx, pk->ms_pp, (int)nk2, rows(nullptr, 1), rows(pk->sq64, 64, pk->swap_idx, 64), no_rows(),
                       rows(pk->ecrt, 64), 64, inv_sq, st);
    if (rc != MPE_OK) return fail(rc);
    hipLaunchKernelGGL(sk_setup_c_kernel, dim3(blocks_for((int)nk2, 64)), dim3(64), 0, st, (int)nk2, pk->sq64, inv_sq, pk->e128);
  } else {
    e = hipMemcpyAsync(pk->N, d_N, (size_t)nk * 64 * 4, hipMemcpyDeviceToDevice, st);
    if (e != hipSuccess) { mpe_set_error("hipMemcpyAsync(N)", e); return fail(MPE_E_HIP); }
  }
  hipLaunchKernelGGL(pk_square_kernel, dim3(blocks_for(nk, 64)), dim3(64), 0, st, nk, pk->N, pk->NN);
  if ((rc = modset_create_dev(ctx, 4096, nk, pk->NN, &pk->ms_nn, st)) != MPE_OK) return fail(rc);
  if ((rc = modset_create_dev(ctx, 2048, nk, pk->N, &pk->ms_n, st)) != MPE_OK) return fail(rc);
  if ((rc = pairset_create(2048, nk, pk->N, &pk->ps_nn, st)) != MPE_OK) return fail(rc);
  if (pk->has_private && (rc = pairset_create(1024, (int)nk2, pk->pq32, &pk->ps_pp, st)) != MPE_OK) return fail(rc);
  e = hipGetLastError();
  if (e != hipSuccess) { mpe_set_error("paillier key set-up", e); return fail(MPE_E_HIP); }
  *out = pk;
  return MPE_OK;
}

static Rows key_selector(const mpe_paillier* pk, const int32_t* d_key_idx) {
  return Rows{nullptr, d_key_idx, (d_key_idx == nullptr && pk->nkeys != 1) ? 1 : 0, 0};
}
static Rows key_rows(const mpe_paillier* pk, const uint32_t* table, int stride, const int32_t* d_key_idx, int words = 0) {
  if (d_key_idx) return Rows{table, d_key_idx, stride, words};
  return Rows{table, nullptr, pk->nkeys == 1 ? 0 : stride, words};
}

static inline size_t modexp_nn_scratch_words(size_t B) { return 2 * B * (1 + 64 + 128) + 256; }
static int modexp_nn(mpe_ctx* ctx, const mpe_paillier* pk, int B, Rows ksel, Rows base, Rows exps, int ew, bool holder,
                     uint32_t* out, hipStream_t st, bool pow_n = false, uint32_t* scratch = nullptr, int phase = 0) {
  if (!(holder && pk->has_private && ctx->use_crt)) {
    if (ctx->use_pair) return launch_pair_modexp(ctx, pk->ps_nn, B, ksel, base, exps, ew, no_rows(), no_rows(), 0, out, st, 0, exps.p == pk->N);
    return launch_modexp(ctx, pk->ms_nn, B, ksel, base, no_rows(), exps, ew, out, st);
  }
  const int B2 = 2 * B;
  int32_t* half_of = scratch ? (int32_t*)scratch : ws_array<int32_t>(ctx, B2);
  uint32_t* u = scratch ? scratch + (((size_t)B2 + 63) & ~(size_t)63) : ws_array<uint32_t>(ctx, (size_t)B2 * 64);
  uint32_t* y = scratch ? u + (size_t)B2 * 64 : ws_array<uint32_t>(ctx, (size_t)B2 * 128);
  if (!scratch) MPE_TRY(ws_ok(ctx));
  if (phase != 2) MPE_LAUNCH_1D(crt_half_kernel, B2, st, B2, ksel, half_of);
  const int bw = base.words ? base.words : 128;
  Rows lo{base.p, base.idx, base.stride, bw < 64 ? bw : 64, 1};
  Rows hi = bw > 64 ? Rows{base.p + 64, base.idx, base.stride, bw - 64, 1} : no_rows();
  Rows ex{exps.p, exps.idx, exps.stride, exps.words, 1};
  if (ctx->use_pair && pow_n && ctx->use_pown) {
    const Rows hsel{nullptr, half_of, 0, 0};
    if (phase != 2)
      MPE_TRY(launch_pair_modexp(ctx, pk->ps_pp, B2, hsel, Rows{base.p, base.idx, base.stride, bw, 1}, rows(pk->eq1, 32, half_of), 32,
                                 no_rows(), no_rows(), 0, y, st, 1));
    if (phase == 1) return MPE_OK;
    MPE_TRY(launch_pair_modexp(ctx, pk->ps_pp, B2, hsel, rows(y, 64, nullptr, 32), rows(pk->pq32, 32, half_of), 32,
                               no_rows(), no_rows(), 0, u, st));
  } else if (ctx->use_pair) {
    MPE_TRY(launch_pair_modexp(ctx, pk->ps_pp, B2, Rows{nullptr, half_of, 0, 0}, Rows{base.p, base.idx, base.stride, bw, 1}, ex, ew,
                               no_rows(), no_rows(), 0, u, st));
  } else {
    MPE_TRY(launch_modexp(ctx, pk->ms_pp, B2, Rows{nullptr, half_of, 0, 0}, lo, hi, ex, ew, u, st));
  }
  MPE_TRY(launch_modmul(ctx, pk->ms_nn, B2, Rows{nullptr, ksel.idx, ksel.stride, 0, 1}, rows(u, 64, nullptr, 64),
                        rows(pk->e128, 128, half_of), y, st));
  MPE_LAUNCH_1D(crt_add_kernel, B, st, B, ksel, pk->NN, y, out);
  return MPE_OK;
}

static int modexp_nn2(mpe_ctx* ctx, const mpe_paillier* pk, int B, Rows ksel, Rows base, Rows exps, int ew, Rows base2,
                      Rows exps2, int ew2, uint32_t* out, hipStream_t st) {
  if (ctx->use_pair) return launch_pair_modexp(ctx, pk->ps_nn, B, ksel, base, exps, ew, base2, exps2, ew2, out, st, 0, exps.p == pk->N);
  return launch_modexp2(ctx, pk->ms_nn, B, ksel, base, exps, ew, base2, exps2, ew2, out, st);
}

static int modexp_n_holder(mpe_ctx* ctx, const mpe_paillier* pk, int B, const int32_t* key_idx, Rows base, Rows exps, int ew, uint32_t* out,
                           hipStream_t st) {
  const int B2 = 2 * B;
  int32_t* item_of = ws_array<int32_t>(ctx, B2);
  int32_t* half_of = ws_array<int32_t>(ctx, B2);
  int32_t* keyj = ws_array<int32_t>(ctx, B2);
  uint32_t* u = ws_array<uint32_t>(ctx, (size_t)B2 * 64);
  uint32_t* y = ws_array<uint32_t>(ctx, (size_t)B2 * 64);
  MPE_TRY(ws_ok(ctx));
  MPE_LAUNCH_1D(dec_index_kernel, B2, st, B2, pk->nkeys, key_idx, item_of, half_of, keyj);
  MPE_TRY(launch_pair_modexp(ctx, pk->ps_pp, B2, Rows{nullptr, half_of, 0, 0}, Rows{base.p, base.idx, base.stride, base.words ? base.words : 64, 1},
                             Rows{exps.p, exps.idx, exps.stride, exps.words, 1}, ew, no_rows(), no_rows(), 0, u, st, 1));
  MPE_TRY(launch_modmul(ctx, pk->ms_n, B2, Rows{nullptr, keyj, 0, 0}, rows(u, 64, nullptr, 32), rows(pk->ab64, 64, half_of), y, st));
  MPE_LAUNCH_1D(dec_combine_kernel, B, st, B, pk->nkeys, y, key_idx, pk->N, out);
  return MPE_OK;
}

static int paillier_encrypt(mpe_ctx* ctx, const mpe_paillier* pk, int B, const int32_t* key_idx, const uint32_t* d_m,
                            const uint32_t* d_r, uint32_t* d_c, bool holder, hipStream_t st, const uint32_t* rn_pre = nullptr) {
  MPE_TRY(ws_begin(ctx, st));
  uint32_t* x = ws_array<uint32_t>(ctx, (size_t)B * 128);
  uint32_t* gm = ws_array<uint32_t>(ctx, (size_t)B * 128);
  MPE_TRY(ws_ok(ctx));
  if (rn_pre) x = const_cast<uint32_t*>(rn_pre);
  else
    MPE_TRY(modexp_nn(ctx, pk, B, key_selector(pk, key_idx), rows(d_r, 64, nullptr, 64), key_rows(pk, pk->N, 64, key_idx), 64,
                      holder, x, st, true));
  MPE_LAUNCH_1D(enc_gm_kernel, B, st, B, pk->nkeys, d_m, key_idx, pk->N, gm);
  return launch_modmul(ctx, pk->ms_nn, B, key_selector(pk, key_idx), rows(x, 128), rows(gm, 128), d_c, st);
}

static int paillier_mul_add_enc(mpe_ctx* ctx, const mpe_paillier* pk, int B, const int32_t* key_idx, Rows c_a, Rows k, int kw,
                                const uint32_t* d_m, const uint32_t* d_r, uint32_t* d_out, hipStream_t st, const uint32_t* x_pre = nullptr) {
  MPE_TRY(ws_begin(ctx, st));
  uint32_t* x = ws_array<uint32_t>(ctx, (size_t)B * 128);
  uint32_t* gm = ws_array<uint32_t>(ctx, (size_t)B * 128);
  uint32_t* y = ctx->use_multiexp || x_pre ? nullptr : ws_array<uint32_t>(ctx, (size_t)B * 128);
  MPE_TRY(ws_ok(ctx));
  const Rows ksel = key_selector(pk, key_idx), Nrow = key_rows(pk, pk->N, 64, key_idx);
  MPE_LAUNCH_1D(enc_gm_kernel, B, st, B, pk->nkeys, d_m, key_idx, pk->N, gm);
  if (x_pre) {
    x = const_cast<uint32_t*>(x_pre);
  } else if (ctx->use_multiexp) {
    MPE_TRY(modexp_nn2(ctx, pk, B, ksel, rows(d_r, 64, nullptr, 64), Nrow, 64, c_a, k, kw, x, st));
  } else {
    MPE_TRY(modexp_nn(ctx, pk, B, ksel, rows(d_r, 64, nullptr, 64), Nrow, 64, false, x, st));
    MPE_TRY(modexp_nn(ctx, pk, B, ksel, c_a, k, kw, false, y, st));
    MPE_TRY(launch_modmul(ctx, pk->ms_nn, B, ksel, rows(x, 128), rows(y, 128), x, st));
  }
  return launch_modmul(ctx, pk->ms_nn, B, ksel, rows(x, 128), rows(gm, 128), d_out, st);
}

static int paillier_decrypt(mpe_ctx* ctx, const mpe_paillier* pk, int B, const int32_t* key_idx, Rows c, uint32_t* d_m,
                            hipStream_t st) {
  const int B2 = 2 * B;
  MPE_TRY(ws_begin(ctx, st));
  int32_t* item_of = ws_array<int32_t>(ctx, B2);
  int32_t* half_of = ws_array<int32_t>(ctx, B2);
  int32_t* keyj = ws_array<int32_t>(ctx, B2);
  uint32_t* u = ws_array<uint32_t>(ctx, (size_t)B2 * 64);
  uint32_t* t = ws_array<uint32_t>(ctx, (size_t)B2 * 32);
  uint32_t* mh = ws_array<uint32_t>(ctx, (size_t)B2 * 64);
  uint32_t* y = ws_array<uint32_t>(ctx, (size_t)B2 * 64);
  MPE_TRY(ws_ok(ctx));
  MPE_LAUNCH_1D(dec_index_kernel, B2, st, B2, pk->nkeys, key_idx, item_of, half_of, keyj);
  if (ctx->use_pair) {
    MPE_TRY(launch_pair_modexp(ctx, pk->ps_pp, B2, Rows{nullptr, half_of, 0, 0}, Rows{c.p, c.idx, c.stride, 128, 1},
                               rows(pk->em1, 32, half_of), 32, no_rows(), no_rows(), 0, u, st));
  } else {
    MPE_TRY(launch_modexp(ctx, pk->ms_pp, B2, Rows{nullptr, half_of, 0, 0}, Rows{c.p, c.idx, c.stride, 64, 1},
                          Rows{c.p + 64, c.idx, c.stride, 64, 1}, rows(pk->em1, 32, half_of), 32, u, st));
  }
  MPE_LAUNCH_1D(dec_lfunc_kernel, B2, st, B2, u, half_of, pk->inv2, t);
  MPE_TRY(launch_modmul(ctx, pk->ms_p, B2, Rows{nullptr, half_of, 0, 0}, rows(t, 32, nullptr, 32),
                        rows(pk->h64, 64, half_of), mh, st));
  MPE_TRY(launch_modmul(ctx, pk->ms_n, B2, Rows{nullptr, keyj, 0, 0}, rows(mh, 64), rows(pk->ab64, 64, half_of), y, st));
  MPE_LAUNCH_1D(dec_combine_kernel, B, st, B, pk->nkeys, y, key_idx, pk->N, d_m);
  return MPE_OK;
}

}

extern "C" {

int mpe_paillier_create_public(mpe_ctx* ctx, int nkeys, const uint32_t* d_N, mpe_paillier** out, void* stream) {
  if (!ctx || !d_N || !out || nkeys <= 0) return MPE_E_ARG;
  return mpe::paillier_create(ctx, nkeys, d_N, nullptr, nullptr, out, (hipStream_t)stream);
}
int mpe_paillier_create_private(mpe_ctx* ctx, int nkeys, const uint32_t* d_p, const uint32_t* d_q, mpe_paillier** out,
                                void* stream) {
  if (!ctx || !d_p || !d_q || !out || nkeys <= 0) return MPE_E_ARG;
  return mpe::paillier_create(ctx, nkeys, nullptr, d_p, d_q, out, (hipStream_t)stream);
}
int mpe_paillier_destroy(mpe_paillier* pk) {
  if (!pk) return MPE_E_ARG;
  mpe::paillier_free(pk);
  return MPE_OK;
}
int mpe_paillier_nkeys(const mpe_paillier* pk) { return pk ? pk->nkeys : MPE_E_ARG; }
const uint32_t* mpe_paillier_n(const mpe_paillier* pk) { return pk ? pk->N : nullptr; }

int mpe_paillier_encrypt(mpe_ctx* ctx, const mpe_paillier* pk, int batch, const int32_t* d_key_idx, const uint32_t* d_m,
                         const uint32_t* d_r, uint32_t* d_c, void* stream) {
  if (!ctx || !pk || !d_m || !d_r || !d_c || batch < 0) return MPE_E_ARG;
  if (!d_key_idx && pk->nkeys != 1 && pk->nkeys < batch) return MPE_E_ARG;
  if (batch == 0) return MPE_OK;
  return mpe::paillier_encrypt(ctx, pk, batch, d_key_idx, d_m, d_r, d_c, pk->has_private, (hipStream_t)stream);
}
int mpe_paillier_decrypt(mpe_ctx* ctx, const mpe_paillier* sk, int batch, const int32_t* d_key_idx, const uint32_t* d_c,
                         uint32_t* d_m, void* stream) {
  if (!ctx || !sk || !d_c || !d_m || batch < 0) return MPE_E_ARG;
  if (!sk->has_private) { mpe_set_error_msg("mpe_paillier_decrypt: key set has no private part"); return MPE_E_ARG; }
  if (!d_key_idx && sk->nkeys != 1 && sk->nkeys < batch) return MPE_E_ARG;
  if (batch == 0) return MPE_OK;
  return mpe::paillier_decrypt(ctx, sk, batch, d_key_idx, mpe::rows(d_c, 128), d_m, (hipStream_t)stream);
}
int mpe_paillier_add(mpe_ctx* ctx, const mpe_paillier* pk, int batch, const int32_t* d_key_idx, const uint32_t* d_c1,
                     const uint32_t* d_c2, uint32_t* d_out, void* stream) {
  if (!ctx || !pk || !d_c1 || !d_c2 || !d_out || batch < 0) return MPE_E_ARG;
  if (!d_key_idx && pk->nkeys != 1 && pk->nkeys < batch) return MPE_E_ARG;
  return mpe::launch_modmul(ctx, pk->ms_nn, batch, mpe::key_selector(pk, d_key_idx), mpe::rows(d_c1, 128),
                            mpe::rows(d_c2, 128), d_out, (hipStream_t)stream);
}
int mpe_paillier_mul(mpe_ctx* ctx, const mpe_paillier* pk, int batch, const int32_t* d_key_idx, const uint32_t* d_c,
                     const uint32_t* d_k, int k_words, uint32_t* d_out, void* stream) {
  if (!ctx || !pk || !d_c || !d_k || !d_out || batch < 0 || k_words <= 0) return MPE_E_ARG;
  if (!d_key_idx && pk->nkeys != 1 && pk->nkeys < batch) return MPE_E_ARG;
  return mpe::modexp_nn(ctx, pk, batch, mpe::key_selector(pk, d_key_idx), mpe::rows(d_c, 128), mpe::rows(d_k, k_words), k_words,
                        false, d_out, (hipStream_t)stream);
}

}
```

### multi_party_ecdsa_amd/csrc/mpe_pair1024.hip

```cpp
#include "mpe_pairexp.h"

namespace mpe {

int pairset_create_1024(int count, const uint32_t* d_moduli, mpe_pairset** out, hipStream_t st) {
  return pairset_create_impl<Cfg1024>(count, d_moduli, out, st);
}
int pair_modexp_1024(mpe_ctx* ctx, const mpe_pairset* ps, int batch, Rows mod_sel, Rows base, Rows exps, int exp_words,
                     Rows base2, Rows exps2, int exp2_words, int half, uint32_t* out, hipStream_t st, int public_exp) {
  return pair_modexp_dispatch<1024, 2>(ctx, ps, batch, mod_sel, base, exps, exp_words, base2, exps2, exp2_words, half, out, st, public_exp);
}

}

#ifdef MPE_WAVE_TRACE
extern "C" int mpe_wave_trace_arm_1024(void* d_buf, unsigned cap) { return mpe::wave_trace_arm_impl(d_buf, cap); }
extern "C" int mpe_wave_trace_count_1024(unsigned* n) { return mpe::wave_trace_count_impl(n); }
#endif
```

### multi_party_ecdsa_amd/csrc/mpe_pair2048.hip

```cpp
#include "mpe_pairexp.h"

namespace mpe {

int pairset_create_2048(int count, const uint32_t* d_moduli, mpe_pairset** out, hipStream_t st) {
  return pairset_create_impl<Cfg2048>(count, d_moduli, out, st);
}
int pair_modexp_2048(mpe_ctx* ctx, const mpe_pairset* ps, int batch, Rows mod_sel, Rows base, Rows exps, int exp_words,
                     Rows base2, Rows exps2, int exp2_words, int half, uint32_t* out, hipStream_t st, int public_exp) {
  return pair_modexp_dispatch<2048, 4>(ctx, ps, batch, mod_sel, base, exps, exp_words, base2, exps2, exp2_words, half, out, st, public_exp);
}

}

#ifdef MPE_WAVE_TRACE
extern "C" int mpe_wave_trace_arm_2048(void* d_buf, unsigned cap) { return mpe::wave_trace_arm_impl(d_buf, cap); }
extern "C" int mpe_wave_trace_count_2048(unsigned* n) { return mpe::wave_trace_count_impl(n); }
#endif
```

### multi_party_ecdsa_amd/csrc/mpe_pairexp.h

```cpp
#pragma once
#include <type_traits>
#include "mpe_internal.h"
#include "mpe_small.h"

namespace mpe {

template <class C>
struct PairLds {
  static constexpr int B0 = 0;
  static constexpr int B1 = C::K;
  static constexpr int M = 2 * C::K;
  static constexpr int KC = 3 * C::K;
  static constexpr int pick_stride() {
    constexpr int per_half = (C::GROUPS >= 2) ? C::GROUPS / 2 : 1;
    for (int s = 4 * C::K + 2;; s += 2) {
      bool ok = true;
      for (int a = 0; a < per_half && ok; ++a)
        for (int b = a + 1; b < per_half; ++b)
          if (((a * s) & 31) == ((b * s) & 31)) { ok = false; break; }
      if (ok) return s;
    }
  }
  static constexpr int STRIDE = pick_stride();
  static constexpr int WORDS = STRIDE * C::GROUPS;
// ... 379 lines not shown
  constexpr int K2 = 2 * C::K;
  const int slot = blockIdx.x * C::GROUPS + ln.g;
  const int nslots = gridDim.x * C::GROUPS;
  const bool dual = base2.p != nullptr;
  const int TE = 1 << wb;
  uint32_t* tab = tables + (size_t)slot * (TE + (dual ? 16 : 0)) * K2;
  uint32_t* tab2 = tab + (size_t)TE * K2;
  const int nwin = (exp_words * 32 + wb - 1) / wb;
  const int nwin2 = dual ? exp2_words * 8 : 0;
  const int top_bit = (nwin - 1) * wb;
  const int words1 = base.words ? base.words : 2 * C::K32, words2 = base2.words ? base2.words : 2 * C::K32;
  WaveSched ws;
  ws.init(sched);

#pragma unroll 1
  for (;;) {
    int ubase;
    if (!ws.next(sched, batch, nslots, C::GROUPS, ubase)) break;
#ifdef MPE_WAVE_TRACE
    const int trip = ws.trip - 1;
    const unsigned long long wt_m0 = __builtin_amdgcn_s_memtime(), wt_r0 = __builtin_amdgcn_s_memrealtime();
#endif
    const int inst = ubase + ln.g;
    const bool active = inst < batch;
    const int pos = active ? inst : batch - 1;
    const int idx = (SLIDE && perm) ? perm[pos] : pos;
    const int mi = sel_index(mod_sel, idx);
    const uint32_t* ex = row_of(exps, idx);
    const uint32_t* ex2 = dual ? row_of(exps2, idx) : ex;
    bool sl_rt = false;
    int sw_lo = -1;
    uint32_t sw_val = 0;
    UniformWords exu = nullptr;
    if (SLIDE && slide) {
      const uint64_t ea = (uint64_t)(uintptr_t)ex;
      const uint32_t e_lo = __builtin_amdgcn_readfirstlane((uint32_t)ea), e_hi = __builtin_amdgcn_readfirstlane((uint32_t)(ea >> 32));
      sl_rt = __ballot(ea != (((uint64_t)e_hi << 32) | e_lo)) == 0;
      exu = (UniformWords)(((uint64_t)e_hi << 32) | e_lo);
      if (sl_rt) {
        sw_lo = slide_window(exu, exp_words, exp_words * 32 - 1, wb, sw_val);
        if (sw_lo < 0 || (dual && sw_lo < 32 * exp2_words)) sl_rt = false;
      }
    }

    uint32_t n[C::L];
    constexpr int KS = pair_kstore(C::BITS);
    load_owner<C>(n, ps.n_limbs + (size_t)mi * KS, ln);
    const uint32_t n0inv = ps.n0inv[mi];
    {
      const uint32_t* kc = ps.kc + (size_t)mi * KS;
#pragma unroll
      for (int i = 0; i < C::L; ++i)
        gl[PL::KC + ln.t + C::TPI * i] = kc[ln.t + C::TPI * i] + ((ln.t + C::TPI * i) < C::STEPS ? C::MASK : 0u);
      uint32_t t0[C::L], t1[C::L];
      load_owner<C>(t0, ps.one + (size_t)mi * 2 * KS, ln);
      load_owner<C>(t1, ps.one + (size_t)mi * 2 * KS + KS, ln);
      store_owner<C>(tab, t0, ln);
      store_owner<C>(tab + C::K, t1, ln);
    }

    const bool sl = SLIDE && sl_rt;
    uint32_t cur0[C::L], cur1[C::L];
    int which = 0;
    const uint32_t* bw = row_of(base, idx);
    int kin = (words1 + C::K32 - 1) / C::K32 - 1;
    load_words_as_limbs<C>(cur0, gl, bw + kin * C::K32, words1 - kin * C::K32, ln);
#pragma unroll
    for (int i = 0; i < C::L; ++i) cur1[i] = 0;
    int ph = kin > 0 ? PP_IN : PP_MONT;
    --kin;
    int k = 0, b = top_bit;
#pragma unroll 1
    while (ph != PP_DONE) {
      if (ph == PP_SQ || (SLIDE && ph == PP_TSQ)) {
        int run = 1;
        if (ph == PP_SQ) {
          int stop = sl ? (sw_lo < b ? sw_lo : 0) : ((b - 1) / wb) * wb;
          if (dual) {
            int s2 = (b - 1) & ~3;
            if ((s2 >> 2) >= nwin2) s2 = (nwin2 - 1) * 4;
            if (s2 > stop) stop = s2;
          }
          if (stop < 0) stop = 0;
          run = b - stop;
          b = stop;
        }
        run = __builtin_amdgcn_readfirstlane(run);
#pragma unroll 1
        do {
          put_limbs<C>(gl + PL::B0, cur0, ln);
          wave_lds_sync();
          pairsq<C>(cur0, cur1, gl, n, n0inv, half != 0, ln);
          wave_lds_sync();
        } while (--run > 0);
        if (SLIDE && ph == PP_TSQ) {
          put_limbs<C>(gl + PL::B0, cur0, ln);
          put_limbs<C>(gl + PL::B1, cur1, ln);
          __builtin_amdgcn_fence(__ATOMIC_SEQ_CST, "workgroup");
          load_owner<C>(cur0, tab + K2, ln);
          load_owner<C>(cur1, tab + K2 + C::K, ln);
          ph = PP_TAB;
        } else {
          const bool m1 = sl ? b == sw_lo : (b % wb) == 0;
          const bool m2 = dual && (b & 3) == 0 && (b >> 2) < nwin2;
          ph = m1 ? PP_MUL1 : (m2 ? PP_MUL2 : PP_FINAL);
        }
        continue;
      }
      if (ph == PP_IN) {
        copy_pair_to_lds<C>(gl, ps.tp + (size_t)mi * 2 * KS, ln, KS);
      } else if (ph == PP_MONT) {
        copy_pair_to_lds<C>(gl, ps.r2 + (size_t)mi * 2 * KS, ln, KS);
      } else if (ph == PP_TAB) {
        if (k == 1 && !(sl && !which)) { put_limbs<C>(gl + PL::B0, cur0, ln); put_limbs<C>(gl + PL::B1, cur1, ln); }
      } else if (ph == PP_MUL1) {
        const uint32_t w = sl ? sw_val : exp_window(ex, exp_words, b / wb, wb);
#ifndef MPE_NARROW_COPY
        copy_row_to_lds<C>(gl, tab + (size_t)w * K2, ln);
#else
        copy_pair_to_lds<C>(gl, tab + (size_t)w * K2, ln);
#endif
      } else if (ph == PP_MUL2) {
        const int wi = b >> 2;
        const uint32_t w = (ex2[wi >> 3] >> ((wi & 7) * 4)) & 15u;
#ifndef MPE_NARROW_COPY
        copy_row_to_lds<C>(gl, w ? tab2 + (size_t)w * K2 : tab, ln);
#else
        copy_pair_to_lds<C>(gl, w ? tab2 + (size_t)w * K2 : tab, ln);
#endif
      } else {
#pragma unroll
        for (int i = 0; i < C::L; ++i) {
          gl[PL::B0 + ln.t * C::L + i] = (ln.t == 0 && i == 0) ? 1u : 0u;
          gl[PL::B1 + ln.t * C::L + i] = 0u;
        }
      }
      wave_lds_sync();
      pairmul<C>(cur0, cur1, gl, n, n0inv, half != 0, ln);
      wave_lds_sync();

      bool tables_done = false;
      if (ph == PP_IN) {
        uint32_t ch[C::L];
        load_words_as_limbs<C>(ch, gl, bw + kin * C::K32, C::K32, ln);
        int64_t z[C::L];
#pragma unroll
        for (int i = 0; i < C::L; ++i) z[i] = (int64_t)cur0[i] + (int64_t)ch[i];
        full_normalize<C>(z, ln);
#pragma unroll
        for (int i = 0; i < C::L; ++i) cur0[i] = (uint32_t)z[i];
        if (--kin < 0) ph = PP_MONT;
      } else if (ph == PP_MONT) {
        uint32_t* T = which ? tab2 : tab;
        store_owner<C>(T + K2, cur0, ln);
        store_owner<C>(T + K2 + C::K, cur1, ln);
        k = 1;
        ph = (sl && !which) ? PP_TSQ : PP_TAB;
      } else if (ph == PP_TAB) {
        uint32_t* T = which ? tab2 : tab;
        const int step = (sl && !which) ? 2 : 1;
        k += step;
        store_owner<C>(T + (size_t)k * K2, cur0, ln);
        store_owner<C>(T + (size_t)k * K2 + C::K, cur1, ln);
        if (k > (which ? 14 : TE - 2)) {
          if (!which && dual) {
            which = 1;
            bw = row_of(base2, idx);
            kin = (words2 + C::K32 - 1) / C::K32 - 1;
            load_words_as_limbs<C>(cur0, gl, bw + kin * C::K32, words2 - kin * C::K32, ln);
#pragma unroll
            for (int i = 0; i < C::L; ++i) cur1[i] = 0;
            ph = kin > 0 ? PP_IN : PP_MONT;
            --kin;
          } else {
            tables_done = true;
          }
        }
      } else if (ph == PP_FINAL) {
        ph = PP_DONE;
      } else {
        if (ph == PP_MUL1 && sl) sw_lo = slide_window(exu, exp_words, b - 1, wb, sw_val);
        const bool m2 = ph != PP_MUL2 && dual && (b & 3) == 0 && (b >> 2) < nwin2;
        ph = m2 ? PP_MUL2 : (b == 0 ? PP_FINAL : PP_SQ);
      }
      if (tables_done) {
        __builtin_amdgcn_fence(__ATOMIC_SEQ_CST, "workgroup");
        const uint32_t w = sl ? sw_val : exp_window(ex, exp_words, nwin - 1, wb);
        load_owner<C>(cur0, tab + (size_t)w * K2, ln);
        load_owner<C>(cur1, tab + (size_t)w * K2 + C::K, ln);
        if (half) {
#pragma unroll
          for (int i = 0; i < C::L; ++i) cur1[i] = 0;
        }
        b = sl ? sw_lo : top_bit;
        if (sl) sw_lo = slide_window(exu, exp_words, b - 1, wb, sw_val);
        ph = b == 0 ? PP_FINAL : PP_SQ;
      }
    }
    {
      int64_t z[C::L];
#pragma unroll
      for (int i = 0; i < C::L; ++i) z[i] = (int64_t)cur0[i];
      full_normalize<C>(z, ln);
      const bool ge = cmp_ge<C>(z, n, ln);
      if (ge) {
#pragma unroll
        for (int i = 0; i < C::L; ++i) z[i] -= (int64_t)n[i];
        full_normalize<C>(z, ln);
      }
#pragma unroll
      for (int i = 0; i < C::L; ++i) { cur0[i] = (uint32_t)z[i]; z[i] = (int64_t)cur1[i]; }
      if (ge && !half && ln.t == 0) z[0] += 1;
      full_normalize<C>(z, ln);
#pragma unroll 1
      for (int pass = 0; pass < 2; ++pass) {
        if (cmp_ge<C>(z, n, ln)) {
#pragma unroll
          for (int i = 0; i < C::L; ++i) z[i] -= (int64_t)n[i];
          full_normalize<C>(z, ln);
        }
      }
#pragma unroll
      for (int i = 0; i < C::L; ++i) cur1[i] = (uint32_t)z[i];
    }
    store_limbs_as_words<C>(out + (size_t)idx * 2 * C::K32, gl, cur0, active, ln);
    store_limbs_as_words<C>(out + (size_t)idx * 2 * C::K32 + C::K32, gl, cur1, active, ln);
#ifdef MPE_WAVE_TRACE
    if (g_wave_trace && threadIdx.x == 0) {
      const unsigned long long wt_m1 = __builtin_amdgcn_s_memtime(), wt_r1 = __builtin_amdgcn_s_memrealtime();
      const unsigned at = atomicAdd(&g_wave_trace_n, 1u);
      if (at < g_wave_trace_cap) {
        unsigned long long* w = g_wave_trace + (size_t)at * 8;
        w[0] = ((unsigned long long)gridDim.x << 32) | blockIdx.x;
        w[1] = ((unsigned long long)(unsigned)batch << 32) | ((unsigned)trip << 16) | ((unsigned)C::L << 8) | ((unsigned)(ws.role != 0) << 2) | ((unsigned)(half != 0) << 1) | (unsigned)(SLIDE ? 1 : 0);
        w[2] = ((unsigned long long)__builtin_amdgcn_s_getreg((31 << 11) | 20) << 32) | __builtin_amdgcn_s_getreg((31 << 11) | 4);
        w[3] = wt_m0; w[4] = wt_m1; w[5] = wt_r0; w[6] = wt_r1;
        w[7] = ((unsigned long long)(unsigned)C::BITS << 32) | (unsigned)exp_words;
      }
    }
#endif
  }
}

template <int H>
__global__ void pair_finish_kernel(int B, Rows mod_sel, const uint32_t* __restrict__ mod_words, uint32_t* __restrict__ out) {
  MPE_FOREGROUND();
  const int i = blockIdx.x * blockDim.x + threadIdx.x;
  if (i >= B) return;
  uint32_t z0[H], z1[H], nn[H], r[2 * H];
  sm::copy(z0, out + (size_t)i * 2 * H, H);
  sm::copy(z1, out + (size_t)i * 2 * H + H, H);
  sm::copy(nn, mod_words + (size_t)sel_index(mod_sel, i) * H, H);
  sm::mul(r, z1, H, nn, H);
  sm::add(r, 2 * H, r, 2 * H, z0, H);
  sm::copy(out + (size_t)i * 2 * H, r, 2 * H);
}

}

namespace mpe {

#ifdef MPE_WAVE_TRACE
static int wave_trace_arm_impl(void* buf, unsigned cap) {
  const unsigned zero = 0;
  if (hipMemcpyToSymbol(HIP_SYMBOL(g_wave_trace), &buf, sizeof buf) != hipSuccess) return MPE_E_HIP;
  if (hipMemcpyToSymbol(HIP_SYMBOL(g_wave_trace_cap), &cap, sizeof cap) != hipSuccess) return MPE_E_HIP;
  if (hipMemcpyToSymbol(HIP_SYMBOL(g_wave_trace_n), &zero, sizeof zero) != hipSuccess) return MPE_E_HIP;
  return MPE_OK;
}
static int wave_trace_count_impl(unsigned* n) {
  return hipMemcpyFromSymbol(n, HIP_SYMBOL(g_wave_trace_n), sizeof *n) == hipSuccess ? MPE_OK : MPE_E_HIP;
}
#endif

template <class C>
int pairset_create_impl(int count, const uint32_t* d_moduli, mpe_pairset** out, hipStream_t st) {
  mpe_pairset* ps = new (std::nothrow) mpe_pairset();
  if (!ps) return MPE_E_NOMEM;
  ps->half_bits = C::BITS;
  ps->count = count;
  ps->mod_words = d_moduli;
  const size_t K = pair_kstore(C::BITS), words = (size_t)count * (K + 1 + 3 * 2 * K + K);
  static_assert(pair_kstore(C::BITS) >= C::K, "the stored constants must hold the layout's limbs");
  hipError_t e = hipMalloc(&ps->blob, words * 4);
  if (e != hipSuccess) { delete ps; mpe_set_error("hipMalloc(pairset)", e); return MPE_E_NOMEM; }
  (void)hipMemsetAsync(ps->blob, 0, words * 4, st);
  uint32_t* p = (uint32_t*)ps->blob;
  ps->n_limbs = p; p += count * K;
  ps->n0inv = p; p += count;
  ps->one = p; p += count * 2 * K;
  ps->r2 = p; p += count * 2 * K;
  ps->tp = p; p += count * 2 * K;
  ps->kc = p;
  hipLaunchKernelGGL(pairset_setup_kernel<C>, dim3((count + C::GROUPS - 1) / C::GROUPS), dim3(64), 0, st, count, d_moduli,
                     ps->n_limbs, ps->n0inv, ps->one, ps->r2, ps->tp, ps->kc);
  e = hipGetLastError();
  if (e != hipSuccess) { (void)hipFree(ps->blob); delete ps; mpe_set_error("pairset_setup_kernel", e); return MPE_E_HIP; }
  *out = ps;
  return MPE_OK;
}

template <class C>
int pair_modexp_impl(mpe_ctx* ctx, const mpe_pairset* ps, int batch, Rows mod_sel, Rows base, Rows exps, int exp_words,
                     Rows base2, Rows exps2, int exp2_words, int half, uint32_t* d_out, hipStream_t st, int public_exp) {
  const int units = (batch + C::GROUPS - 1) / C::GROUPS;
  const int grid = ladder_grid(ctx, units, ctx->cus * ctx->modexp_waves_per_cu);
  int wb = exp_words <= 8 ? 4 : (exp_words < 48 ? 5 : 6);
  if (ctx->window_bits) wb = ctx->window_bits;
  const bool dual = base2.p != nullptr;
  if (dual && (exp2_words <= 0 || 32 * exp2_words > ((exp_words * 32 + wb - 1) / wb - 1) * wb)) {
    mpe_set_error_msg("pair modexp: the second exponent must be shorter than the first");
    return MPE_E_ARG;
  }
  const size_t need = (size_t)grid * C::GROUPS * (((size_t)1 << wb) + (dual ? 16 : 0)) * 2 * C::K * sizeof(uint32_t);
  const int slide = (public_exp && ctx->use_sliding && !half && exp_words >= 16 && wb >= 5) ? 1 : 0;
  const bool by_key = slide && ps->count > 1 && (mod_sel.idx || mod_sel.stride) && ps->count <= 4096 && batch > C::GROUPS;
  const size_t extra = (by_key ? ((size_t)batch + 2 * (size_t)ps->count + 64) * sizeof(int32_t) : 0) + SCHED_WORDS * sizeof(int32_t);
  uint32_t* tabs = tables_for(ctx, need + extra, st);
  if (!tabs) return MPE_E_NOMEM;
  SchedArgs sched = ladder_sched(ctx, units, ctx->cus * ctx->modexp_waves_per_cu, (int32_t*)((char*)tabs + need + extra) - SCHED_WORDS, st);
  if (sched.prio == 1) sched.prio = 2;
  const int32_t* perm = nullptr;
  if (by_key) {
    int32_t* pm = (int32_t*)((char*)tabs + need);
    int32_t *cnt = pm + batch, *cursor = cnt + ps->count;
    (void)hipMemsetAsync(cnt, 0, (size_t)ps->count * sizeof(int32_t), st);
    const int nb = (batch + 255) / 256;
    hipLaunchKernelGGL(key_hist_kernel, dim3(nb), dim3(256), (size_t)ps->count * 4, st, batch, mod_sel, ps->count, cnt);
    hipLaunchKernelGGL(key_scan_kernel, dim3(1), dim3(64), 0, st, ps->count, cnt, cursor);
    hipLaunchKernelGGL(key_scatter_kernel, dim3(nb), dim3(256), (size_t)ps->count * 8, st, batch, mod_sel, ps->count, cursor, pm);
    perm = pm;
  }
  PairsetView v{ps->n_limbs, ps->n0inv, ps->one, ps->r2, ps->tp, ps->kc, ps->count};
  prof_begin(ctx, st, half ? 4 : (slide ? 6 : 3), half ? C::BITS : 2 * C::BITS, exp_words, batch, dual ? exp2_words : 0);
  if (slide)
    hipLaunchKernelGGL((pair_modexp_kernel<C, true>), dim3(grid), dim3(64), 0, st, batch, v, mod_sel, base, exps, exp_words, wb, base2,
                       exps2, exp2_words, half, d_out, tabs, perm, slide, sched);
  else
    hipLaunchKernelGGL((pair_modexp_kernel<C, false>), dim3(grid), dim3(64), 0, st, batch, v, mod_sel, base, exps, exp_words, wb, base2,
                       exps2, exp2_words, half, d_out, tabs, perm, slide, sched);
  prof_end(ctx, st);
  if (slide) {
    if (uint32_t* ctr = prof_counter(ctx, units))
      hipLaunchKernelGGL(pair_slide_audit_kernel, dim3(blocks_for(units, 64)), dim3(64), 0, st, batch, (int)C::GROUPS, exps,
                         exp_words, wb, dual ? exp2_words : 0, perm, ctr);
  }
  hipLaunchKernelGGL(pair_finish_kernel<C::K32>, dim3(blocks_for(batch, 64)), dim3(64), 0, st, batch, mod_sel, ps->mod_words, d_out);
  hipError_t e = hipGetLastError();
  if (e != hipSuccess) { mpe_set_error("pair_modexp_kernel", e); return MPE_E_HIP; }
  ctx->last.waves = grid;
  ctx->last.ints_per_wave = C::GROUPS;
  ctx->last.limbs = 2 * C::K;
  ctx->last.limb_bits = C::W;
  ctx->last.lds_bytes_per_wave = PairLds<C>::WORDS * 4;
  ctx->last.table_scratch_bytes = need;
  return MPE_OK;
}

template <int BITS, int TPI>
int pair_modexp_dispatch(mpe_ctx* ctx, const mpe_pairset* ps, int batch, Rows mod_sel, Rows base, Rows exps, int exp_words,
                         Rows base2, Rows exps2, int exp2_words, int half, uint32_t* out, hipStream_t st, int public_exp) {
  using Base = Cfg<BITS, MPE_W, MPE_L, TPI>;
  using Wide = Cfg<BITS, MPE_W, MPE_L / 2, 2 * TPI>;
  using XWide = Cfg<BITS, MPE_W, 5, 4 * TPI>;
  static_assert(std::is_same<Base, Cfg2048>::value || std::is_same<Base, Cfg1024>::value, "the 18-limb layout is the one of mpe_bigint.h");
  static_assert(Wide::K == Base::K, "the two layouts share the limb arrays");
  const long resident = (long)ctx->cus * ctx->modexp_waves_per_cu * Base::GROUPS / ctx->device_share;
  const int xdiv = ctx->xwide_div;
  if (ctx->adaptive_lanes && xdiv > 0 && (long)xdiv * batch <= resident)
    return pair_modexp_impl<XWide>(ctx, ps, batch, mod_sel, base, exps, exp_words, base2, exps2, exp2_words, half, out, st, public_exp);
  if (ctx->adaptive_lanes && (long)ctx->wide_div * batch <= resident)
    return pair_modexp_impl<Wide>(ctx, ps, batch, mod_sel, base, exps, exp_words, base2, exps2, exp2_words, half, out, st, public_exp);
  return pair_modexp_impl<Base>(ctx, ps, batch, mod_sel, base, exps, exp_words, base2, exps2, exp2_words, half, out, st, public_exp);
}

}
```

### multi_party_ecdsa_amd/csrc/mpe_proofs.h

```cpp
#pragma once
#include "mpe_sigma_dev.h"
#include "mpe_internal.h"
#include "mpe_modinv.h"
#include "mpe_paillier.h"
#include "mpe_small.h"

struct mpe_statements {
  int count = 0;
  void* blob = nullptr;
  uint32_t* Nt = nullptr;
  uint32_t* h1 = nullptr;
  uint32_t* h2 = nullptr;
  mpe_modset* ms = nullptr;
  int fb_wb = 8;
  uint32_t* fb_tab = nullptr;
};

#include "mpe_fixedbase.h"

extern "C" int mpe_statements_create_wb(mpe_ctx* ctx, int count, const uint32_t* d_Nt, const uint32_t* d_h1, const uint32_t* d_h2,
                                        int wb, mpe_statements** out, void* stream);
static inline size_t mpe_statements_table_bytes(int count, int wb) {
  return (size_t)2 * count * mpe::fb_windows(wb) * ((size_t)1 << wb) * mpe::Cfg2048::K * sizeof(uint32_t);
}

namespace mpe {

static int launch_fb_modexp(mpe_ctx* ctx, const mpe_statements* stm, int B, Rows st_sel, int which, Rows exps, int ew,
                            uint32_t* out, hipStream_t st) {
  if (B == 0) return MPE_OK;
  using C = Cfg2048;
  const int cap = ctx->cus * ctx->modexp_waves_per_cu;
  int split = 1;
  if (ctx->fb_split > 0) { while (split * 2 <= ctx->fb_split && split * 2 <= (int)C::GROUPS) split *= 2; }
  else if (ctx->adaptive_lanes) { while (split * 2 <= (int)C::GROUPS && ((long)B * split * 2 + C::GROUPS - 1) / C::GROUPS <= cap / 2) split *= 2; }
  const int per_wave = C::GROUPS / split;
  const int units = (B + per_wave - 1) / per_wave;
  const int grid = ladder_grid(ctx, units, cap);
  int32_t* sst = (int32_t*)tables_for(ctx, SCHED_WORDS * sizeof(int32_t), st);
  if (!sst) return MPE_E_NOMEM;
  const SchedArgs sched = ladder_sched(ctx, units, cap, sst, st);
  ModsetView v;
  v.n_limbs = stm->ms->n_limbs; v.one_limbs = stm->ms->one_limbs; v.r2_limbs = stm->ms->r2_limbs;
  v.r2h_limbs = stm->ms->r2h_limbs; v.n0inv = stm->ms->n0inv; v.count = stm->ms->count;
  prof_begin(ctx, st, 5, C::BITS, ew, B, stm->fb_wb);
  hipLaunchKernelGGL(fb_modexp_kernel<C>, dim3(grid), dim3(64), 0, st, B, v, st_sel, which, stm->fb_tab, stm->fb_wb, exps, ew, out, sched, split);
  prof_end(ctx, st);
  hipError_t e = hipGetLastError();
  if (e != hipSuccess) { mpe_set_error("fb_modexp_kernel", e); return MPE_E_HIP; }
  return MPE_OK;
}

__global__ void __launch_bounds__(64) MPE_EC_OCC ec_mul_kernel(int B, const uint32_t* __restrict__ k, int kw, const uint32_t* __restrict__ P,
                              uint32_t* __restrict__ out) {
  const int i = blockIdx.x * blockDim.x + threadIdx.x;
  if (i >= B) return;
  const ec::U256 s = ec::sc_reduce(k + (size_t)i * kw, kw);
  const ec::Jac r = P ? ec::jac_mul(s, ec::aff_load(P + (size_t)i * 16)) : ec::jac_mul_gen(s);
  ec::aff_store(out + (size_t)i * 16, ec::jac_to_aff(r));
}
__global__ void __launch_bounds__(64) MPE_EC_OCC ec_add_kernel(int B, const uint32_t* __restrict__ P, const uint32_t* __restrict__ Q,
                              uint32_t* __restrict__ out) {
  const int i = blockIdx.x * blockDim.x + threadIdx.x;
  if (i >= B) return;
  const ec::Jac r = ec::jac_add(ec::jac_from_aff(ec::aff_load(P + (size_t)i * 16)),
                                ec::jac_from_aff(ec::aff_load(Q + (size_t)i * 16)));
  ec::aff_store(out + (size_t)i * 16, ec::jac_to_aff(r));
}

__global__ void __launch_bounds__(64) MPE_EC_OCC dlog_prove_kernel(int B, ec::Enc enc, const uint32_t* __restrict__ sk, const uint32_t* __restrict__ nonce,
                                  uint32_t* __restrict__ pk, uint32_t* __restrict__ R, uint32_t* __restrict__ z) {
  const int i = blockIdx.x * blockDim.x + threadIdx.x;
  if (i >= B) return;
  ec::Aff P, Rp;
  ec::U256 zz;
  sig::dlog_prove_body(ec::sc_reduce(sk + (size_t)i * 8, 8), ec::sc_reduce(nonce + (size_t)i * 8, 8), enc, P, Rp, zz);
  ec::aff_store(pk + (size_t)i * 16, P);
  ec::aff_store(R + (size_t)i * 16, Rp);
  ec::u256_store(z + (size_t)i * 8, zz);
}
__global__ void __launch_bounds__(64) MPE_EC_OCC dlog_verify_kernel(int B, ec::Enc enc, const uint32_t* __restrict__ pk, const uint32_t* __restrict__ R,
                                   const uint32_t* __restrict__ z, uint8_t* __restrict__ ok) {
  const int i = blockIdx.x * blockDim.x + threadIdx.x;
  if (i >= B) return;
  const ec::Aff P = ec::aff_load(pk + (size_t)i * 16), Rp = ec::aff_load(R + (size_t)i * 16);
  if (!ec::aff_valid(P) || !ec::aff_valid(Rp)) { ok[i] = 0; return; }
  ok[i] = sig::dlog_verify_body(P, Rp, ec::sc_reduce(z + (size_t)i * 8, 8), enc) ? 1 : 0;
}

__global__ void muladd_kernel(int B, Rows a, int na, Rows b, int nb, Rows c, int nc, uint32_t* __restrict__ r, int nr) {
  MPE_FOREGROUND();
  const int i = blockIdx.x * blockDim.x + threadIdx.x;
  if (i >= B) return;
  uint32_t x[90], y[90], t[180];
  sm::copy(x, row_of(a, i), na);
  sm::copy(y, row_of(b, i), nb);
  sm::mul(t, x, na, y, nb);
  for (int j = na + nb; j < nr; ++j) t[j] = 0;
  const uint32_t one[1] = {1};
  const uint32_t* cp = c.p ? row_of(c, i) : one;
  sm::add(t, nr, t, nr, cp, c.p ? nc : 1);
  uint32_t* o = r + (size_t)i * nr;
  for (int j = 0; j < nr; ++j) o[j] = t[j];
}

enum { HF_BIGINT = 0, HF_BIGINT_PLUS1 = 1, HF_POINT_COMPRESSED = 2 };
struct HashField { Rows r; int words; int kind; };
struct HashDesc { HashField f[14]; int n; };
__global__ void __launch_bounds__(64) MPE_EC_OCC hash_kernel(int B, ec::Enc enc, HashDesc d, uint32_t* __restrict__ out) {
  MPE_FOREGROUND();
  const int i = blockIdx.x * blockDim.x + threadIdx.x;
  if (i >= B) return;
  ec::Sha256 s;
  ec::sha_init(s);
  for (int k = 0; k < d.n; ++k) {
    const uint32_t* p = row_of(d.f[k].r, i);
    if (d.f[k].kind == HF_POINT_COMPRESSED) {
      ec::sha_point_compressed(s, ec::aff_load(p));
    } else if (d.f[k].kind == HF_BIGINT_PLUS1) {
      uint32_t t[130];
      const uint32_t one[1] = {1};
      t[d.f[k].words] = sm::add(t, d.f[k].words, p, d.f[k].words, one, 1);
      ec::sha_bigint(s, t, d.f[k].words + 1, enc);
    } else {
      ec::sha_bigint(s, p, d.f[k].words, enc);
    }
  }
  ec::u256_store(out + (size_t)i * 8, ec::sha_final(s));
}
static HashField hf(Rows r, int words, int kind = HF_BIGINT) { return HashField{r, words, kind}; }

__global__ void s1_range_kernel(int B, Rows s1, int words, uint8_t* __restrict__ ok) {
  const int i = blockIdx.x * blockDim.x + threadIdx.x;
  if (i >= B) return;
  uint32_t q[8], q2[16], q3[24];
  for (int j = 0; j < 8; ++j) q[j] = ec::FQ[j];
  sm::mul(q2, q, 8, q, 8);
  sm::mul(q3, q2, 16, q, 8);
  ok[i] = sm::cmp(row_of(s1, i), words, q3, 24) <= 0 ? 1 : 0;
}
__global__ void and_flags_kernel(int B, uint8_t* __restrict__ ok, const uint8_t* __restrict__ a, const uint8_t* __restrict__ b,
                                 const uint32_t* __restrict__ x, Rows y, int words) {
  const int i = blockIdx.x * blockDim.x + threadIdx.x;
  if (i >= B) return;
  bool v = ok[i] != 0;
  if (a) v = v && a[i];
  if (b) v = v && b[i];
  if (x) v = v && sm::cmp(x + (size_t)i * words, words, row_of(y, i), words) == 0;
  ok[i] = v ? 1 : 0;
}
__global__ void fill_u8_kernel(int B, uint8_t* p, uint8_t v) {
  const int i = blockIdx.x * blockDim.x + threadIdx.x;
  if (i < B) p[i] = v;
}
__global__ void __launch_bounds__(64) MPE_EC_OCC pdl_u1_check_kernel(int B, Rows s1, const uint32_t* __restrict__ e, Rows G, Rows Q, Rows u1,
                                    uint8_t* __restrict__ ok) {
  const int i = blockIdx.x * blockDim.x + threadIdx.x;
  if (i >= B) return;
  const ec::U256 a = ec::sc_reduce(row_of(s1, i), 25);
  const ec::U256 ne = ec::sc_neg(ec::sc_reduce(e + (size_t)i * 8, 8));
  const ec::Aff Gp = ec::aff_load(row_of(G, i)), Qp = ec::aff_load(row_of(Q, i)), U1 = ec::aff_load(row_of(u1, i));
  if (!ec::aff_valid(Gp) || !ec::aff_valid(Qp) || !ec::aff_valid(U1)) { ok[i] = 0; return; }
  const ec::Jac l = ec::jac_add(ec::jac_mul(a, Gp), ec::jac_mul(ne, Qp));
  if (!ec::jac_eq_aff(l, U1)) ok[i] = 0;
}
__global__ void __launch_bounds__(64) MPE_EC_OCC ec_mul_rows_kernel(int B, Rows k, int kw, Rows P, uint32_t* __restrict__ out) {
  MPE_FOREGROUND();
  const int i = blockIdx.x * blockDim.x + threadIdx.x;
  if (i >= B) return;
  const ec::U256 s = ec::sc_reduce(row_of(k, i), kw);
  const ec::Jac r = P.p ? ec::jac_mul(s, ec::aff_load(row_of(P, i))) : ec::jac_mul_gen(s);
  ec::aff_store(out + (size_t)i * 16, ec::jac_to_aff(r));
}

struct Seq {
  mpe_ctx* ctx;
  hipStream_t st;
  int B;
  int rc = MPE_OK;
  uint32_t* words(size_t per_item) {
    uint32_t* p = ws_array<uint32_t>(ctx, (size_t)B * per_item);
    if (!p && rc == MPE_OK) rc = MPE_E_NOMEM;
    return p;
  }
  uint8_t* flags() {
    uint8_t* p = ws_array<uint8_t>(ctx, (size_t)B);
    if (!p && rc == MPE_OK) rc = MPE_E_NOMEM;
    return p;
  }
  uint32_t* fb_modexp(const mpe_statements* stm, Rows sel, int which, Rows base, Rows exps, int ew) {
    if (!stm->fb_tab || !ctx->use_fixed_base) return modexp(stm->ms, sel, base, exps, ew);
    uint32_t* o = words(64);
    if (rc == MPE_OK) rc = launch_fb_modexp(ctx, stm, B, sel, which, exps, ew, o, st);
    return o;
  }
  uint32_t* modexp(const mpe_modset* ms, Rows sel, Rows base, Rows exps, int ew) {
    uint32_t* o = words(ms->bits / 32);
    if (rc == MPE_OK) rc = launch_modexp(ctx, ms, B, sel, base, no_rows(), exps, ew, o, st);
    return o;
  }
  uint32_t* modexp_nn(const mpe_paillier* pk, Rows sel, Rows base, Rows exps, int ew, bool holder, bool pow_n = false) {
    uint32_t* o = words(128);
    if (rc == MPE_OK) rc = mpe::modexp_nn(ctx, pk, B, sel, base, exps, ew, holder, o, st, pow_n);
    return o;
  }
  uint32_t* modexp_nn2(const mpe_paillier* pk, Rows sel, Rows base, Rows exps, int ew, Rows base2, Rows exps2, int ew2) {
    uint32_t* o = words(128);
    if (rc == MPE_OK) rc = mpe::modexp_nn2(ctx, pk, B, sel, base, exps, ew, base2, exps2, ew2, o, st);
    return o;
  }
  uint32_t* modexp_n(const mpe_paillier* pk, const int32_t* key_idx, Rows sel, Rows base, Rows exps, int ew) {
    if (!(pk->has_private && ctx->use_crt && ctx->use_pair && ctx->use_crt_n)) return modexp(pk->ms_n, sel, base, exps, ew);
    uint32_t* o = words(64);
    if (rc == MPE_OK) rc = mpe::modexp_n_holder(ctx, pk, B, key_idx, base, exps, ew, o, st);
    return o;
  }
  uint32_t* modmul(const mpe_modset* ms, Rows sel, Rows a, Rows b) {
    uint32_t* o = words(ms->bits / 32);
    if (rc == MPE_OK) rc = launch_modmul(ctx, ms, B, sel, a, b, o, st);
    return o;
  }
  void modmul_to(const mpe_modset* ms, Rows sel, Rows a, Rows b, uint32_t* o) {
    if (rc == MPE_OK) rc = launch_modmul(ctx, ms, B, sel, a, b, o, st);
  }
  uint32_t* modinv(const mpe_modset* ms, Rows sel, Rows a, uint8_t* ok) {
    uint32_t* o = words(ms->bits / 32);
    if (rc == MPE_OK) rc = launch_modinv(ctx, ms, B, sel, a, o, ok, st);
    return o;
  }
  void muladd(Rows a, int na, Rows b, int nb, Rows c, int nc, uint32_t* r, int nr) {
    if (rc != MPE_OK) return;
    hipLaunchKernelGGL(muladd_kernel, dim3(blocks_for(B, 64)), dim3(64), 0, st, B, a, na, b, nb, c, nc, r, nr);
  }
  void hash(const HashDesc& d, uint32_t* out) {
    if (rc != MPE_OK) return;
    hipLaunchKernelGGL(hash_kernel, dim3(blocks_for(B, 64)), dim3(64), 0, st, B, ctx->enc, d, out);
  }
  int finish(const char* what) {
    if (rc != MPE_OK) return rc;
    hipError_t e = hipGetLastError();
    if (e != hipSuccess) { mpe_set_error(what, e); return MPE_E_HIP; }
    return MPE_OK;
  }
};

static Rows sel_of(const int32_t* idx, int count) { return Rows{nullptr, idx, (idx == nullptr && count != 1) ? 1 : 0, 0}; }
static Rows tab_rows(const uint32_t* table, int stride, const int32_t* idx, int count, int words = 0) {
  if (idx) return Rows{table, idx, stride, words};
  return Rows{table, nullptr, count == 1 ? 0 : stride, words};
}

struct AliceProofRows { Rows z, e, s, s1, s2; };
struct PdlProofRows { Rows z, u1, u2, u3, s1, s2, s3; };
static AliceProofRows dense(const mpe_alice_proof* p) {
  return AliceProofRows{rows(p->z, 64), rows(p->e, 8), rows(p->s, 64), rows(p->s1, 25), rows(p->s2, 89)};
}
static PdlProofRows dense(const mpe_pdl_proof* p) {
  return PdlProofRows{rows(p->z, 64), rows(p->u1, 16), rows(p->u2, 128), rows(p->u3, 64), rows(p->s1, 25), rows(p->s2, 64),
                      rows(p->s3, 89)};
}
static Rows with_words(Rows r, int words) { r.words = words; return r; }
struct Handed {
  const uint32_t* p = nullptr; hipEvent_t ready = nullptr; explicit operator bool() const { return p != nullptr; }
  void wait(hipStream_t st) const { if (p && ready) (void)hipStreamWaitEvent(st, ready, 0); }
};

static int merge_rc(const Seq& a, const Seq& b, const Seq& c) { return a.rc != MPE_OK ? a.rc : (b.rc != MPE_OK ? b.rc : c.rc); }

static int alice_generate(mpe_ctx* ctx, const mpe_paillier* pk, const mpe_statements* stm, int B, const int32_t* key_idx,
                          const int32_t* st_idx, Rows a, Rows cipher, Rows r,
                          const mpe_alice_nonces* nn, const mpe_alice_proof* out, hipStream_t st, Fork* outer = nullptr,
                          Handed bn_pre = {}, hipEvent_t cipher_ready = nullptr) {
  MPE_TRY(ws_begin(ctx, st));
  Fork f(ctx, st, 3, B <= ctx->par_items);
  Seq q{ctx, f.s(0), B}, q1{ctx, f.s(1), B}, q2{ctx, f.s(2), B};
  const Rows ksel = sel_of(key_idx, pk->nkeys), ssel = sel_of(st_idx, stm->count);
  const Rows h1 = tab_rows(stm->h1, 64, st_idx, stm->count), h2 = tab_rows(stm->h2, 64, st_idx, stm->count);
  const Rows Nrow = tab_rows(pk->N, 64, key_idx, pk->nkeys);
  uint32_t* z1 = q1.fb_modexp(stm, ssel, 0, h1,a, 8);
  uint32_t* z2 = q1.fb_modexp(stm, ssel, 1, h2,rows(nn->rho, 72), 72);
  q1.modmul_to(stm->ms, ssel, rows(z1, 64), rows(z2, 64), out->z);
  uint32_t* gu = q.words(128);
  q.muladd(rows(nn->alpha, 24), 24, Nrow, 64, no_rows(), 0, gu, 128);
  bn_pre.wait(f.s(0));
  const uint32_t* bn = bn_pre ? bn_pre.p : q.modexp_nn(pk, ksel, rows(nn->beta, 64, nullptr, 64), Nrow, 64, true, true);
  uint32_t* u = q.modmul(pk->ms_nn, ksel, rows(gu, 128), rows(bn, 128));
  uint32_t* w1 = q2.fb_modexp(stm, ssel, 0, h1,rows(nn->alpha, 24), 24);
  uint32_t* w2 = q2.fb_modexp(stm, ssel, 1, h2,rows(nn->gamma, 88), 88);
  uint32_t* w = q2.modmul(stm->ms, ssel, rows(w1, 64), rows(w2, 64));
  f.join();
  if (cipher_ready) (void)hipStreamWaitEvent(st, cipher_ready, 0);
  else if (outer) outer->join();
  q.rc = merge_rc(q, q1, q2);
  HashDesc d;
  d.n = 6;
  d.f[0] = hf(Nrow, 64); d.f[1] = hf(Nrow, 64, HF_BIGINT_PLUS1); d.f[2] = hf(cipher, 128);
  d.f[3] = hf(rows(out->z, 64), 64); d.f[4] = hf(rows(u, 128), 128); d.f[5] = hf(rows(w, 64), 64);
  q.hash(d, out->e);
  uint32_t* re = q.modexp_n(pk, key_idx, ksel, r, rows(out->e, 8), 8);
  q.modmul_to(pk->ms_n, ksel, rows(re, 64), rows(nn->beta, 64), out->s);
  q.muladd(rows(out->e, 8), 8, a, 8, rows(nn->alpha, 24), 24, out->s1, 25);
  q.muladd(rows(out->e, 8), 8, rows(nn->rho, 72), 72, rows(nn->gamma, 88), 88, out->s2, 89);
  return q.finish("alice_generate");
}

static int alice_verify(mpe_ctx* ctx, const mpe_paillier* pk, const mpe_statements* stm, int B, const int32_t* key_idx,
                        const int32_t* st_idx, Rows cipher, const AliceProofRows& pr, uint8_t* ok, hipStream_t st,
                        Handed m_pre = {}, const uint8_t* inv_ok_pre = nullptr) {
  MPE_TRY(ws_begin(ctx, st));
  Fork f(ctx, st, 3, B <= ctx->par_items);
  Seq q{ctx, f.s(0), B}, q1{ctx, f.s(1), B}, q2{ctx, f.s(2), B};
  const Rows ksel = sel_of(key_idx, pk->nkeys), ssel = sel_of(st_idx, stm->count);
  const Rows h1 = tab_rows(stm->h1, 64, st_idx, stm->count), h2 = tab_rows(stm->h2, 64, st_idx, stm->count);
  const Rows Nrow = tab_rows(pk->N, 64, key_idx, pk->nkeys);
  MPE_LAUNCH_1D(s1_range_kernel, B, st, B, pr.s1, 25, ok);
  uint8_t *inv_ok1 = q.flags(), *inv_ok2 = q.flags();
  uint32_t* ze = q1.modexp(stm->ms, ssel, pr.z, pr.e, 8);
  uint32_t* zei = q1.modinv(stm->ms, ssel, rows(ze, 64), inv_ok1);
  uint32_t* a1 = q2.fb_modexp(stm, ssel, 0, h1,pr.s1, 25);
  uint32_t* a2 = q2.fb_modexp(stm, ssel, 1, h2,pr.s2, 89);
  uint32_t* a12 = q2.modmul(stm->ms, ssel, rows(a1, 64), rows(a2, 64));
  uint32_t* gs1 = q.words(128);
  q.muladd(pr.s1, 25, Nrow, 64, no_rows(), 0, gs1, 128);
  uint32_t *u = nullptr, *b12 = nullptr, *cie = nullptr;
  if (m_pre) {
    inv_ok2 = const_cast<uint8_t*>(inv_ok_pre);
    m_pre.wait(f.s(0));
    u = q.modmul(pk->ms_nn, ksel, rows(gs1, 128), rows(m_pre.p, 128));
  } else if (f.on) {
    uint32_t* sn = q.modexp_nn(pk, ksel, with_words(pr.s, 64), Nrow, 64, false);
    b12 = q.modmul(pk->ms_nn, ksel, rows(gs1, 128), rows(sn, 128));
    uint32_t* cred = q2.modmul(pk->ms_nn, ksel, cipher, rows(pk->ms_nn->one_words, 0, nullptr, 1));
    uint32_t* cinv = q2.modinv(pk->ms_nn, ksel, rows(cred, 128), inv_ok2);
    cie = q2.modexp_nn(pk, ksel, rows(cinv, 128), pr.e, 8, false);
  } else if (ctx->use_multiexp) {
    uint32_t* cred = q.modmul(pk->ms_nn, ksel, cipher, rows(pk->ms_nn->one_words, 0, nullptr, 1));
    uint32_t* cinv = q.modinv(pk->ms_nn, ksel, rows(cred, 128), inv_ok2);
    uint32_t* m = q.modexp_nn2(pk, ksel, with_words(pr.s, 64), Nrow, 64, rows(cinv, 128), pr.e, 8);
    u = q.modmul(pk->ms_nn, ksel, rows(gs1, 128), rows(m, 128));
  } else {
    uint32_t* ce = q.modexp_nn(pk, ksel, cipher, pr.e, 8, false);
    uint32_t* cei = q.modinv(pk->ms_nn, ksel, rows(ce, 128), inv_ok2);
    uint32_t* sn = q.modexp_nn(pk, ksel, with_words(pr.s, 64), Nrow, 64, false);
    uint32_t* b12n = q.modmul(pk->ms_nn, ksel, rows(gs1, 128), rows(sn, 128));
    u = q.modmul(pk->ms_nn, ksel, rows(b12n, 128), rows(cei, 128));
  }
  f.join();
  q.rc = merge_rc(q, q1, q2);
  if (f.on && !m_pre) u = q.modmul(pk->ms_nn, ksel, rows(b12, 128), rows(cie, 128));
  uint32_t* w = q.modmul(stm->ms, ssel, rows(a12, 64), rows(zei, 64));
  uint32_t* e2 = q.words(8);
  HashDesc d;
  d.n = 6;
  d.f[0] = hf(Nrow, 64); d.f[1] = hf(Nrow, 64, HF_BIGINT_PLUS1); d.f[2] = hf(cipher, 128);
  d.f[3] = hf(pr.z, 64); d.f[4] = hf(rows(u, 128), 128); d.f[5] = hf(rows(w, 64), 64);
  q.hash(d, e2);
  if (q.rc == MPE_OK)
    hipLaunchKernelGGL(and_flags_kernel, dim3(blocks_for(B, 64)), dim3(64), 0, st, B, ok, inv_ok1, inv_ok2, e2, pr.e, 8);
  return q.finish("alice_verify");
}

static int pdl_prove(mpe_ctx* ctx, const mpe_paillier* pk, const mpe_statements* stm, int B, const int32_t* key_idx,
                     const int32_t* st_idx, Rows cipher, Rows Qp, Rows Gp, Rows x, Rows r, const mpe_pdl_nonces* nn,
                     const mpe_pdl_proof* out, hipStream_t st, Fork* outer = nullptr, Handed bn_pre = {},
                     hipEvent_t G_ready = nullptr) {
  MPE_TRY(ws_begin(ctx, st));
  Fork f(ctx, st, 3, B <= ctx->par_items);
  Seq q{ctx, f.s(0), B}, q1{ctx, f.s(1), B}, q2{ctx, f.s(2), B};
  const Rows ksel = sel_of(key_idx, pk->nkeys), ssel = sel_of(st_idx, stm->count);
  const Rows h1 = tab_rows(stm->h1, 64, st_idx, stm->count), h2 = tab_rows(stm->h2, 64, st_idx, stm->count);
  const Rows Nrow = tab_rows(pk->N, 64, key_idx, pk->nkeys);
  uint32_t* z1 = q1.fb_modexp(stm, ssel, 0, h1,x, 8);
  uint32_t* z2 = q1.fb_modexp(stm, ssel, 1, h2,rows(nn->rho, 72), 72);
  q1.modmul_to(stm->ms, ssel, rows(z1, 64), rows(z2, 64), out->z);
  if (G_ready) (void)hipStreamWaitEvent(f.s(1), G_ready, 0);
  else if (outer) outer->branch_done_wait(1, f.s(1));
  if (B > 0) hipLaunchKernelGGL(ec_mul_rows_kernel, dim3(blocks_for(B, 64)), dim3(64), 0, f.s(1), B, rows(nn->alpha, 24), 24, Gp, out->u1);
  uint32_t* ga = q.words(128);
  q.muladd(rows(nn->alpha, 24), 24, Nrow, 64, no_rows(), 0, ga, 128);
  bn_pre.wait(f.s(0));
  const uint32_t* bn = bn_pre ? bn_pre.p : q.modexp_nn(pk, ksel, rows(nn->beta, 64, nullptr, 64), Nrow, 64, true, true);
  q.modmul_to(pk->ms_nn, ksel, rows(ga, 128), rows(bn, 128), out->u2);
  uint32_t* w1 = q2.fb_modexp(stm, ssel, 0, h1,rows(nn->alpha, 24), 24);
  uint32_t* w2 = q2.fb_modexp(stm, ssel, 1, h2,rows(nn->gamma, 88), 88);
  q2.modmul_to(stm->ms, ssel, rows(w1, 64), rows(w2, 64), out->u3);
  f.join();
  if (outer) outer->join();
  q.rc = merge_rc(q, q1, q2);
  uint32_t* e = q.words(8);
  HashDesc d;
  d.n = 7;
  d.f[0] = hf(Gp, 16, HF_POINT_COMPRESSED); d.f[1] = hf(Qp, 16, HF_POINT_COMPRESSED);
  d.f[2] = hf(cipher, 128); d.f[3] = hf(rows(out->z, 64), 64);
  d.f[4] = hf(rows(out->u1, 16), 16, HF_POINT_COMPRESSED); d.f[5] = hf(rows(out->u2, 128), 128);
  d.f[6] = hf(rows(out->u3, 64), 64);
  q.hash(d, e);
  q.muladd(rows(e, 8), 8, x, 8, rows(nn->alpha, 24), 24, out->s1, 25);
  uint32_t* re = q.modexp_n(pk, key_idx, ksel, r, rows(e, 8), 8);
  q.modmul_to(pk->ms_n, ksel, rows(re, 64), rows(nn->beta, 64), out->s2);
  q.muladd(rows(e, 8), 8, rows(nn->rho, 72), 72, rows(nn->gamma, 88), 88, out->s3, 89);
  return q.finish("pdl_prove");
}

static int pdl_verify(mpe_ctx* ctx, const mpe_paillier* pk, const mpe_statements* stm, int B, const int32_t* key_idx,
                      const int32_t* st_idx, Rows cipher, Rows Qp, Rows Gp, const PdlProofRows& pr, uint8_t* ok,
                      hipStream_t st) {
  MPE_TRY(ws_begin(ctx, st));
  const Rows ksel = sel_of(key_idx, pk->nkeys), ssel = sel_of(st_idx, stm->count);
  const Rows h1 = tab_rows(stm->h1, 64, st_idx, stm->count), h2 = tab_rows(stm->h2, 64, st_idx, stm->count);
  const Rows Nrow = tab_rows(pk->N, 64, key_idx, pk->nkeys);
  Seq q0{ctx, st, B};
  uint32_t* e = q0.words(8);
  HashDesc d;
  d.n = 7;
  d.f[0] = hf(Gp, 16, HF_POINT_COMPRESSED); d.f[1] = hf(Qp, 16, HF_POINT_COMPRESSED);
  d.f[2] = hf(cipher, 128); d.f[3] = hf(pr.z, 64);
  d.f[4] = hf(pr.u1, 16, HF_POINT_COMPRESSED); d.f[5] = hf(pr.u2, 128);
  d.f[6] = hf(pr.u3, 64);
  q0.hash(d, e);
  Fork f(ctx, st, 3, B <= ctx->par_items);
  Seq q{ctx, f.s(0), B}, q1{ctx, f.s(1), B}, q2{ctx, f.s(2), B};
  q.rc = q0.rc;
  if (B > 0) {
    hipLaunchKernelGGL(fill_u8_kernel, dim3(blocks_for(B, 64)), dim3(64), 0, f.s(1), B, ok, (uint8_t)1);
    hipLaunchKernelGGL(pdl_u1_check_kernel, dim3(blocks_for(B, 64)), dim3(64), 0, f.s(1), B, pr.s1, e, Gp, Qp, pr.u1, ok);
  }
  uint8_t *inv_ok1 = q.flags(), *inv_ok2 = q.flags();
  uint32_t* g1 = q.words(128);
  q.muladd(pr.s1, 25, Nrow, 64, no_rows(), 0, g1, 128);
  uint32_t *u2 = nullptr, *t2s = nullptr, *cies = nullptr;
  if (f.on) {
    uint32_t* s2n = q.modexp_nn(pk, ksel, with_words(pr.s2, 64), Nrow, 64, false);
    t2s = q.modmul(pk->ms_nn, ksel, rows(g1, 128), rows(s2n, 128));
    uint32_t* cred = q1.modmul(pk->ms_nn, ksel, cipher, rows(pk->ms_nn->one_words, 0, nullptr, 1));
    uint32_t* cinv = q1.modinv(pk->ms_nn, ksel, rows(cred, 128), inv_ok1);
    cies = q1.modexp_nn(pk, ksel, rows(cinv, 128), rows(e, 8), 8, false);
  } else {
    uint32_t* cred = q.modmul(pk->ms_nn, ksel, cipher, rows(pk->ms_nn->one_words, 0, nullptr, 1));
    uint32_t* cinv = q.modinv(pk->ms_nn, ksel, rows(cred, 128), inv_ok1);
    if (ctx->use_multiexp) {
      uint32_t* m = q.modexp_nn2(pk, ksel, with_words(pr.s2, 64), Nrow, 64, rows(cinv, 128), rows(e, 8), 8);
      u2 = q.modmul(pk->ms_nn, ksel, rows(g1, 128), rows(m, 128));
    } else {
      uint32_t* s2n = q.modexp_nn(pk, ksel, with_words(pr.s2, 64), Nrow, 64, false);
      uint32_t* t2 = q.modmul(pk->ms_nn, ksel, rows(g1, 128), rows(s2n, 128));
      uint32_t* cie = q.modexp_nn(pk, ksel, rows(cinv, 128), rows(e, 8), 8, false);
      u2 = q.modmul(pk->ms_nn, ksel, rows(t2, 128), rows(cie, 128));
    }
  }
  uint32_t* a1 = q2.fb_modexp(stm, ssel, 0, h1,pr.s1, 25);
  uint32_t* a2 = q2.fb_modexp(stm, ssel, 1, h2,pr.s3, 89);
  uint32_t* a12 = q2.modmul(stm->ms, ssel, rows(a1, 64), rows(a2, 64));
  uint32_t* zred = q2.modmul(stm->ms, ssel, pr.z, rows(stm->ms->one_words, 0, nullptr, 1));
  uint32_t* zinv = q2.modinv(stm->ms, ssel, rows(zred, 64), inv_ok2);
  uint32_t* zie = q2.modexp(stm->ms, ssel, rows(zinv, 64), rows(e, 8), 8);
  uint32_t* u3 = q2.modmul(stm->ms, ssel, rows(a12, 64), rows(zie, 64));
  f.join();
  q.rc = merge_rc(q, q1, q2);
  if (f.on) u2 = q.modmul(pk->ms_nn, ksel, rows(t2s, 128), rows(cies, 128));
  if (q.rc == MPE_OK) {
    hipLaunchKernelGGL(and_flags_kernel, dim3(blocks_for(B, 64)), dim3(64), 0, st, B, ok, inv_ok1, inv_ok2, u2, pr.u2, 128);
    hipLaunchKernelGGL(and_flags_kernel, dim3(blocks_for(B, 64)), dim3(64), 0, st, B, ok, (const uint8_t*)nullptr,
                       (const uint8_t*)nullptr, u3, pr.u3, 64);
  }
  return q.finish("pdl_verify");
}

}

extern "C" {

int mpe_statements_create(mpe_ctx* ctx, int count, const uint32_t* d_Nt, const uint32_t* d_h1, const uint32_t* d_h2,
                          mpe_statements** out, void* stream) {
  if (!ctx) return MPE_E_ARG;
  return mpe_statements_create_wb(ctx, count, d_Nt, d_h1, d_h2, ctx->fb_window_bits, out, stream);
}
int mpe_statements_create_wb(mpe_ctx* ctx, int count, const uint32_t* d_Nt, const uint32_t* d_h1, const uint32_t* d_h2, int wb,
                             mpe_statements** out, void* stream) {
  if (!ctx || !d_Nt || !d_h1 || !d_h2 || !out || count <= 0 || (wb != 0 && wb < 2) || wb > 16) return MPE_E_ARG;
  hipStream_t st = (hipStream_t)stream;
  mpe_statements* s = new (std::nothrow) mpe_statements();
  if (!s) return MPE_E_NOMEM;
  s->count = count;
  const size_t w = (size_t)count * 64;
  hipError_t e = hipMalloc(&s->blob, 3 * w * 4);
  if (e != hipSuccess) { delete s; mpe_set_error("hipMalloc(statements)", e); return MPE_E_NOMEM; }
  s->Nt = (uint32_t*)s->blob; s->h1 = s->Nt + w; s->h2 = s->h1 + w;
  (void)hipMemcpyAsync(s->Nt, d_Nt, w * 4, hipMemcpyDeviceToDevice, st);
  (void)hipMemcpyAsync(s->h1, d_h1, w * 4, hipMemcpyDeviceToDevice, st);
  (void)hipMemcpyAsync(s->h2, d_h2, w * 4, hipMemcpyDeviceToDevice, st);
  int rc = mpe::modset_create_dev(ctx, 2048, count, s->Nt, &s->ms, st);
  if (rc != MPE_OK) { (void)hipFree(s->blob); delete s; return rc; }
  s->fb_wb = 0;
  if (ctx->use_fixed_base && wb != 0) {
    using C = mpe::Cfg2048;
    s->fb_wb = wb;
    const int nwindows = mpe::fb_windows(s->fb_wb);
    const size_t bytes = (size_t)2 * count * nwindows * ((size_t)1 << s->fb_wb) * C::K * sizeof(uint32_t);
    e = hipMalloc((void**)&s->fb_tab, bytes);
    if (e != hipSuccess) { mpe_set_error("hipMalloc(fixed-base tables)", e); mpe_statements_destroy(s); return MPE_E_NOMEM; }
    mpe::ModsetView v;
    v.n_limbs = s->ms->n_limbs; v.one_limbs = s->ms->one_limbs; v.r2_limbs = s->ms->r2_limbs; v.r2h_limbs = s->ms->r2h_limbs;
    v.n0inv = s->ms->n0inv; v.count = s->ms->count;
    const int npairs = 2 * count, nrows = npairs * nwindows;
    hipLaunchKernelGGL(mpe::fb_bases_kernel<C>, dim3((npairs + C::GROUPS - 1) / C::GROUPS), dim3(64), 0, st, npairs, v, s->h1,
                       s->h2, s->fb_wb, s->fb_tab);
    hipLaunchKernelGGL(mpe::fb_fill_kernel<C>, dim3((nrows + C::GROUPS - 1) / C::GROUPS), dim3(64), 0, st, nrows, v, s->fb_wb,
                       s->fb_tab);
    e = hipGetLastError();
    if (e != hipSuccess) { mpe_set_error("fixed-base table build", e); mpe_statements_destroy(s); return MPE_E_HIP; }
  }
  *out = s;
  return MPE_OK;
}
int mpe_statements_destroy(mpe_statements* s) {
  if (!s) return MPE_E_ARG;
  if (s->ms) mpe_modset_destroy(s->ms);
  if (s->fb_tab) (void)hipFree(s->fb_tab);
  if (s->blob) (void)hipFree(s->blob);
  delete s;
  return MPE_OK;
}

int mpe_ec_mul_base(mpe_ctx* ctx, int batch, const uint32_t* d_k, int k_words, uint32_t* d_out, void* stream) {
  if (!ctx || !d_k || !d_out || batch < 0 || k_words <= 0 || k_words > 89) return MPE_E_ARG;
  hipStream_t st = (hipStream_t)stream;
  MPE_LAUNCH_1D(mpe::ec_mul_kernel, batch, st, batch, d_k, k_words, (const uint32_t*)nullptr, d_out);
  return MPE_OK;
}
int mpe_ec_mul(mpe_ctx* ctx, int batch, const uint32_t* d_k, int k_words, const uint32_t* d_P, uint32_t* d_out,
               void* stream) {
  if (!ctx || !d_k || !d_P || !d_out || batch < 0 || k_words <= 0 || k_words > 89) return MPE_E_ARG;
  hipStream_t st = (hipStream_t)stream;
  MPE_LAUNCH_1D(mpe::ec_mul_kernel, batch, st, batch, d_k, k_words, d_P, d_out);
  return MPE_OK;
}
int mpe_ec_add(mpe_ctx* ctx, int batch, const uint32_t* d_P, const uint32_t* d_Q, uint32_t* d_out, void* stream) {
  if (!ctx || !d_P || !d_Q || !d_out || batch < 0) return MPE_E_ARG;
  hipStream_t st = (hipStream_t)stream;
  MPE_LAUNCH_1D(mpe::ec_add_kernel, batch, st, batch, d_P, d_Q, d_out);
  return MPE_OK;
}
int mpe_dlog_prove(mpe_ctx* ctx, int batch, const uint32_t* d_sk, const uint32_t* d_nonce, uint32_t* d_pk,
                   uint32_t* d_R, uint32_t* d_z, void* stream) {
  if (!ctx || !d_sk || !d_nonce || !d_pk || !d_R || !d_z || batch < 0) return MPE_E_ARG;
  hipStream_t st = (hipStream_t)stream;
  MPE_LAUNCH_1D(mpe::dlog_prove_kernel, batch, st, batch, ctx->enc, d_sk, d_nonce, d_pk, d_R, d_z);
  return MPE_OK;
}
int mpe_dlog_verify(mpe_ctx* ctx, int batch, const uint32_t* d_pk, const uint32_t* d_R, const uint32_t* d_z,
                    uint8_t* d_ok, void* stream) {
  if (!ctx || !d_pk || !d_R || !d_z || !d_ok || batch < 0) return MPE_E_ARG;
  hipStream_t st = (hipStream_t)stream;
  MPE_LAUNCH_1D(mpe::dlog_verify_kernel, batch, st, batch, ctx->enc, d_pk, d_R, d_z, d_ok);
  return MPE_OK;
}
int mpe_modinv(mpe_ctx* ctx, const mpe_modset* ms, int batch, const int32_t* d_mod_idx, const uint32_t* d_a,
               uint32_t* d_out, uint8_t* d_ok, void* stream) {
  if (!ctx || !ms || !d_a || !d_out || !d_ok || batch < 0) return MPE_E_ARG;
  if (!d_mod_idx && ms->count != 1 && ms->count < batch) return MPE_E_ARG;
  MPE_TRY(mpe::ws_begin(ctx, (hipStream_t)stream));
  return mpe::launch_modinv(ctx, ms, batch, mpe::sel_of(d_mod_idx, ms->count), mpe::rows(d_a, ms->bits / 32), d_out, d_ok,
                            (hipStream_t)stream);
}

static bool proof_args_ok(const mpe_ctx* ctx, const mpe_paillier* pk, const mpe_statements* stm, int batch,
                          const int32_t* key_idx, const int32_t* st_idx) {
  if (!ctx || !pk || !stm || batch < 0) return false;
  if (!key_idx && pk->nkeys != 1 && pk->nkeys < batch) return false;
  if (!st_idx && stm->count != 1 && stm->count < batch) return false;
  return true;
}
int mpe_alice_generate(mpe_ctx* ctx, const mpe_paillier* pk, const mpe_statements* stm, int batch,
                       const int32_t* d_key_idx, const int32_t* d_st_idx, const uint32_t* d_a, const uint32_t* d_cipher,
                       const uint32_t* d_r, const mpe_alice_nonces* nonces, const mpe_alice_proof* out, void* stream) {
  if (!proof_args_ok(ctx, pk, stm, batch, d_key_idx, d_st_idx) || !d_a || !d_cipher || !d_r || !nonces || !out) return MPE_E_ARG;
  if (batch == 0) return MPE_OK;
  return mpe::alice_generate(ctx, pk, stm, batch, d_key_idx, d_st_idx, mpe::rows(d_a, 8), mpe::rows(d_cipher, 128),
                             mpe::rows(d_r, 64), nonces, out, (hipStream_t)stream);
}
int mpe_alice_verify(mpe_ctx* ctx, const mpe_paillier* pk, const mpe_statements* stm, int batch, const int32_t* d_key_idx,
                     const int32_t* d_st_idx, const uint32_t* d_cipher, const mpe_alice_proof* proof, uint8_t* d_ok,
                     void* stream) {
  if (!proof_args_ok(ctx, pk, stm, batch, d_key_idx, d_st_idx) || !d_cipher || !proof || !d_ok) return MPE_E_ARG;
  if (batch == 0) return MPE_OK;
  return mpe::alice_verify(ctx, pk, stm, batch, d_key_idx, d_st_idx, mpe::rows(d_cipher, 128), mpe::dense(proof), d_ok,
                           (hipStream_t)stream);
}
int mpe_pdl_prove(mpe_ctx* ctx, const mpe_paillier* pk, const mpe_statements* stm, int batch, const int32_t* d_key_idx,
                  const int32_t* d_st_idx, const uint32_t* d_cipher, const uint32_t* d_Q, const uint32_t* d_G,
                  const uint32_t* d_x, const uint32_t* d_r, const mpe_pdl_nonces* nonces, const mpe_pdl_proof* out,
                  void* stream) {
  if (!proof_args_ok(ctx, pk, stm, batch, d_key_idx, d_st_idx) || !d_cipher || !d_Q || !d_G || !d_x || !d_r || !nonces || !out)
    return MPE_E_ARG;
  if (batch == 0) return MPE_OK;
  return mpe::pdl_prove(ctx, pk, stm, batch, d_key_idx, d_st_idx, mpe::rows(d_cipher, 128), mpe::rows(d_Q, 16), mpe::rows(d_G, 16),
                        mpe::rows(d_x, 8), mpe::rows(d_r, 64), nonces, out, (hipStream_t)stream);
}
int mpe_pdl_verify(mpe_ctx* ctx, const mpe_paillier* pk, const mpe_statements* stm, int batch, const int32_t* d_key_idx,
                   const int32_t* d_st_idx, const uint32_t* d_cipher, const uint32_t* d_Q, const uint32_t* d_G,
                   const mpe_pdl_proof* proof, uint8_t* d_ok, void* stream) {
  if (!proof_args_ok(ctx, pk, stm, batch, d_key_idx, d_st_idx) || !d_cipher || !d_Q || !d_G || !proof || !d_ok) return MPE_E_ARG;
  if (batch == 0) return MPE_OK;
  return mpe::pdl_verify(ctx, pk, stm, batch, d_key_idx, d_st_idx, mpe::rows(d_cipher, 128), mpe::rows(d_Q, 16), mpe::rows(d_G, 16),
                         mpe::dense(proof), d_ok, (hipStream_t)stream);
}

}
```

Before: 19240.

## Fuse Paillier (1+N)^m scaling into raw pair-form modexp finish kernel

Adds a raw output mode to the pair modexp that leaves the result in its (z0, t) pair representation and skips pair_finish_kernel. A new pair_scale_finish_kernel then applies the (1+N)^m factor directly: it computes z0 + N·(t + z0·m mod N). This replaces the separate gm/muladd construction, the conversion finish and a full 4096-bit modmul mod N^2 in encryption, mul-add encryption and the range/PDL proofs. The cost is a new hand-written kernel with tricky limb handling, and the fused path applies only when the pair path is enabled.

```diff
diff --git a/multi_party_ecdsa_amd/csrc/mpe_gg20.h b/multi_party_ecdsa_amd/csrc/mpe_gg20.h
--- a/multi_party_ecdsa_amd/csrc/mpe_gg20.h
+++ b/multi_party_ecdsa_amd/csrc/mpe_gg20.h
@@ -994,7 +994,8 @@
   gather(nVI, e_vi, 8, 8, e2);                gather(nMB, rows(bsel, 8), 8, 8, e2 + nVI * 8);
   (void)hipMemcpyAsync(key, kpub_vi, nVI * 4, hipMemcpyDeviceToDevice, st);
   (void)hipMemcpyAsync(key + nVI, kpub_mb, nMB * 4, hipMemcpyDeviceToDevice, st);
-  MPE_TRY(modexp_nn2(ctx, pk, (int)n, key_selector(pk, key), rows(b1, 64, nullptr, 64), key_rows(pk, pk->N, 64, key), 64, rows(b2, 128), rows(e2, 8), 8, out, st));
+  MPE_TRY(modexp_nn2(ctx, pk, (int)n, key_selector(pk, key), rows(b1, 64, nullptr, 64), key_rows(pk, pk->N, 64, key), 64, rows(b2, 128), rows(e2, 8), 8, out, st,
+                     nn_pair_form(ctx)));
   *m_vi = out; *inv_ok_vi = inv_ok; *x_mb = out + nVI * 128;
   return MPE_OK;
 }
diff --git a/multi_party_ecdsa_amd/csrc/mpe_internal.h b/multi_party_ecdsa_amd/csrc/mpe_internal.h
--- a/multi_party_ecdsa_amd/csrc/mpe_internal.h
+++ b/multi_party_ecdsa_amd/csrc/mpe_internal.h
@@ -132,9 +132,9 @@
 int pairset_create_2048(int count, const uint32_t* d_moduli, mpe_pairset** out, hipStream_t st);
 int pairset_create_1024(int count, const uint32_t* d_moduli, mpe_pairset** out, hipStream_t st);
 int pair_modexp_2048(mpe_ctx* ctx, const mpe_pairset* ps, int batch, Rows mod_sel, Rows base, Rows exps, int exp_words,
-                     Rows base2, Rows exps2, int exp2_words, int half, uint32_t* out, hipStream_t st, int public_exp);
+                     Rows base2, Rows exps2, int exp2_words, int half, uint32_t* out, hipStream_t st, int public_exp, int raw);
 int pair_modexp_1024(mpe_ctx* ctx, const mpe_pairset* ps, int batch, Rows mod_sel, Rows base, Rows exps, int exp_words,
-                     Rows base2, Rows exps2, int exp2_words, int half, uint32_t* out, hipStream_t st, int public_exp);
+                     Rows base2, Rows exps2, int exp2_words, int half, uint32_t* out, hipStream_t st, int public_exp, int raw);
 
 inline int ws_begin(mpe_ctx* ctx, hipStream_t st) { return ctx->ws.begin(st) ? MPE_OK : MPE_E_NOMEM; }
 inline void* ws_alloc(mpe_ctx* ctx, size_t bytes) { return ctx->ws.alloc(bytes); }
diff --git a/multi_party_ecdsa_amd/csrc/mpe_lib.hip b/multi_party_ecdsa_amd/csrc/mpe_lib.hip
--- a/multi_party_ecdsa_amd/csrc/mpe_lib.hip
+++ b/multi_party_ecdsa_amd/csrc/mpe_lib.hip
@@ -215,12 +215,12 @@
   return MPE_E_ARG;
 }
 static int launch_pair_modexp(mpe_ctx* ctx, const mpe_pairset* ps, int batch, Rows mod_sel, Rows base, Rows exps, int exp_words,
-                              Rows base2, Rows exps2, int exp2_words, uint32_t* out, hipStream_t st, int half = 0, int public_exp = 0) {
+                              Rows base2, Rows exps2, int exp2_words, uint32_t* out, hipStream_t st, int half = 0, int public_exp = 0, int raw = 0) {
   if (batch == 0) return MPE_OK;
   if (ps->half_bits == 2048)
-    return pair_modexp_2048(ctx, ps, batch, mod_sel, base, exps, exp_words, base2, exps2, exp2_words, half, out, st, public_exp);
+    return pair_modexp_2048(ctx, ps, batch, mod_sel, base, exps, exp_words, base2, exps2, exp2_words, half, out, st, public_exp, raw);
   if (ps->half_bits == 1024)
-    return pair_modexp_1024(ctx, ps, batch, mod_sel, base, exps, exp_words, base2, exps2, exp2_words, half, out, st, public_exp);
+    return pair_modexp_1024(ctx, ps, batch, mod_sel, base, exps, exp_words, base2, exps2, exp2_words, half, out, st, public_exp, raw);
   return MPE_E_ARG;
 }
 }
diff --git a/multi_party_ecdsa_amd/csrc/mpe_paillier.h b/multi_party_ecdsa_amd/csrc/mpe_paillier.h
--- a/multi_party_ecdsa_amd/csrc/mpe_paillier.h
+++ b/multi_party_ecdsa_amd/csrc/mpe_paillier.h
@@ -139,6 +139,105 @@
   sm::mul(r, a, 64, n, 64);
   sm::add(r, 128, r, 128, one, 1);
   sm::copy(gm + (size_t)i * 128, r, 128);
+}
+
+struct ScaleLds {
+  static constexpr int NL = 2 * Cfg2048::K + 4;
+  static constexpr int STRIDE = NL + Cfg2048::K;
+};
+__global__ void __launch_bounds__(64) pair_scale_finish_kernel(int batch, ModsetView ms, Rows mod_sel, const uint32_t* zz, Rows x, int xw,
+                                                               uint32_t* out) {
+  MPE_FOREGROUND();
+  using C = Cfg2048;
+  constexpr int L = C::L, W = C::W;
+  static_assert(C::K % L == 0 && C::STRIDE <= ScaleLds::NL, "staging and the montmul operand fit in front of the limbs of N");
+  __shared__ uint32_t lds[ScaleLds::STRIDE * C::GROUPS];
+  const Lane ln = make_lane<C>();
+  uint32_t* gl = lds + ln.g * ScaleLds::STRIDE;
+  uint32_t* nl = gl + ScaleLds::NL;
+  const int slot = blockIdx.x * C::GROUPS + ln.g;
+  const int nslots = gridDim.x * C::GROUPS;
+  const int trips = (batch + nslots - 1) / nslots;
+#pragma unroll 1
+  for (int trip = 0; trip < trips; ++trip) {
+    if (trip * nslots + (int)blockIdx.x * C::GROUPS >= batch) break;
+    const int inst = trip * nslots + slot;
+    const bool active = inst < batch;
+    const int idx = active ? inst : batch - 1;
+    const int mi = sel_index(mod_sel, idx);
+    uint32_t n[L];
+    load_owner<C>(n, ms.n_limbs + (size_t)mi * C::K, ln);
+    const uint32_t n0inv = ms.n0inv[mi];
+    uint32_t z0[L], t[L];
+    load_words_as_limbs<C>(z0, gl, zz + (size_t)idx * 2 * C::K32, C::K32, ln);
+    load_words_as_limbs<C>(t, gl, zz + (size_t)idx * 2 * C::K32 + C::K32, C::K32, ln);
+    if (x.p) {
+      uint32_t cur[L], b[L];
+      load_words_as_limbs<C>(b, gl, row_of(x, idx), xw, ln);
+#pragma unroll
+      for (int i = 0; i < L; ++i) cur[i] = z0[i];
+#pragma unroll 1
+      for (int step = 0; step < 2; ++step) {
+        if (step == 0) put_limbs<C>(gl, b, ln);
+        else copy_to_lds<C>(gl, ms.r2_limbs + (size_t)mi * C::K, ln);
+        wave_lds_sync();
+        uint32_t r[L];
+        montmul<C>(r, cur, gl, n, n0inv, ln);
+        wave_lds_sync();
+#pragma unroll
+        for (int i = 0; i < L; ++i) cur[i] = r[i];
+      }
+      int64_t z[L];
+#pragma unroll
+      for (int i = 0; i < L; ++i) z[i] = (int64_t)cur[i] + (int64_t)t[i];
+      full_normalize<C>(z, ln);
+#pragma unroll 1
+      for (int pass = 0; pass < 2; ++pass) {
+        if (cmp_ge<C>(z, n, ln)) {
+#pragma unroll
+          for (int i = 0; i < L; ++i) z[i] -= (int64_t)n[i];
+          full_normalize<C>(z, ln);
+        }
+      }
+#pragma unroll
+      for (int i = 0; i < L; ++i) t[i] = (uint32_t)z[i];
+    }
+    store_owner<C>(nl, n, ln);
+    wave_lds_sync();
+    uint64_t c[L];
+#pragma unroll
+    for (int i = 0; i < L; ++i) c[i] = z0[i];
+    uint32_t maskv = C::MASK;
+    asm volatile("" : "+v"(maskv));
+#pragma unroll 1
+    for (int jj = 0; jj < C::TPI; ++jj) {
+      const uint32_t* bp = nl + jj * L;
+      uint32_t* lo = gl + jj * L;
+#pragma unroll
+      for (int r = 0; r < L; ++r) {
+        const uint32_t bj = bp[r];
+#pragma unroll
+        for (int i = 0; i < L; ++i) c[(r + i) % L] += (uint64_t)t[i] * bj;
+        const uint32_t low = (uint32_t)c[r] & maskv;
+        if (ln.t0) lo[r] = low;
+        c[(r + 1) % L] += c[r] >> W;
+        uint32_t in = pull_next(low);
+        if (ln.t == C::TPI - 1) in = 0;
+        c[r] = in;
+      }
+    }
+    int64_t hi[L];
+#pragma unroll
+    for (int i = 0; i < L; ++i) hi[i] = (int64_t)c[i];
+    full_normalize<C>(hi, ln);
+#pragma unroll
+    for (int i = 0; i < L; ++i) gl[C::K + ln.t * L + i] = (uint32_t)hi[i];
+    if (ln.t0) { gl[2 * C::K] = 0; gl[2 * C::K + 1] = 0; }
+    wave_lds_sync();
+    if (active)
+      for (int q = ln.t; q < 2 * C::K32; q += C::TPI) out[(size_t)idx * 2 * C::K32 + q] = word_from_limbs<C>(gl, q);
+    wave_lds_sync();
+  }
 }
 
 __global__ void dec_index_kernel(int B2, int nkeys, const int32_t* __restrict__ key_idx, int32_t* __restrict__ item_of,
@@ -270,9 +369,9 @@
 
 static inline size_t modexp_nn_scratch_words(size_t B) { return 2 * B * (1 + 64 + 128) + 256; }
 static int modexp_nn(mpe_ctx* ctx, const mpe_paillier* pk, int B, Rows ksel, Rows base, Rows exps, int ew, bool holder,
-                     uint32_t* out, hipStream_t st, bool pow_n = false, uint32_t* scratch = nullptr, int phase = 0) {
+                     uint32_t* out, hipStream_t st, bool pow_n = false, uint32_t* scratch = nullptr, int phase = 0, bool raw = false) {
   if (!(holder && pk->has_private && ctx->use_crt)) {
-    if (ctx->use_pair) return launch_pair_modexp(ctx, pk->ps_nn, B, ksel, base, exps, ew, no_rows(), no_rows(), 0, out, st, 0, exps.p == pk->N);
+    if (ctx->use_pair) return launch_pair_modexp(ctx, pk->ps_nn, B, ksel, base, exps, ew, no_rows(), no_rows(), 0, out, st, 0, exps.p == pk->N, raw);
     return launch_modexp(ctx, pk->ms_nn, B, ksel, base, no_rows(), exps, ew, out, st);
   }
   const int B2 = 2 * B;
@@ -306,9 +405,20 @@
 }
 
 static int modexp_nn2(mpe_ctx* ctx, const mpe_paillier* pk, int B, Rows ksel, Rows base, Rows exps, int ew, Rows base2,
-                      Rows exps2, int ew2, uint32_t* out, hipStream_t st) {
-  if (ctx->use_pair) return launch_pair_modexp(ctx, pk->ps_nn, B, ksel, base, exps, ew, base2, exps2, ew2, out, st, 0, exps.p == pk->N);
+                      Rows exps2, int ew2, uint32_t* out, hipStream_t st, bool raw = false) {
+  if (ctx->use_pair) return launch_pair_modexp(ctx, pk->ps_nn, B, ksel, base, exps, ew, base2, exps2, ew2, out, st, 0, exps.p == pk->N, raw);
   return launch_modexp2(ctx, pk->ms_nn, B, ksel, base, exps, ew, base2, exps2, ew2, out, st);
+}
+
+static inline bool nn_pair_form(const mpe_ctx* ctx) { return ctx->use_pair; }
+
+static int gamma_finish_nn(mpe_ctx* ctx, const mpe_paillier* pk, int B, Rows ksel, const uint32_t* zz, Rows x, int xw, uint32_t* out,
+                           hipStream_t st) {
+  if (B == 0) return MPE_OK;
+  hipLaunchKernelGGL(pair_scale_finish_kernel, dim3(grid_for<Cfg2048>(ctx, B, 16)), dim3(64), 0, st, B, view_of(pk->ms_n), ksel, zz, x, xw, out);
+  hipError_t e = hipGetLastError();
+  if (e != hipSuccess) { mpe_set_error("pair_scale_finish_kernel", e); return MPE_E_HIP; }
+  return MPE_OK;
 }
 
 static int modexp_n_holder(mpe_ctx* ctx, const mpe_paillier* pk, int B, const int32_t* key_idx, Rows base, Rows exps, int ew, uint32_t* out,
@@ -332,8 +442,14 @@
                             const uint32_t* d_r, uint32_t* d_c, bool holder, hipStream_t st, const uint32_t* rn_pre = nullptr) {
   MPE_TRY(ws_begin(ctx, st));
   uint32_t* x = ws_array<uint32_t>(ctx, (size_t)B * 128);
-  uint32_t* gm = ws_array<uint32_t>(ctx, (size_t)B * 128);
+  const bool pair_x = !rn_pre && !(holder && pk->has_private && ctx->use_crt) && nn_pair_form(ctx);
+  uint32_t* gm = pair_x ? nullptr : ws_array<uint32_t>(ctx, (size_t)B * 128);
   MPE_TRY(ws_ok(ctx));
+  if (pair_x) {
+    MPE_TRY(modexp_nn(ctx, pk, B, key_selector(pk, key_idx), rows(d_r, 64, nullptr, 64), key_rows(pk, pk->N, 64, key_idx), 64,
+                      false, x, st, true, nullptr, 0, true));
+    return gamma_finish_nn(ctx, pk, B, key_selector(pk, key_idx), x, rows(d_m, 64), 64, d_c, st);
+  }
   if (rn_pre) x = const_cast<uint32_t*>(rn_pre);
   else
     MPE_TRY(modexp_nn(ctx, pk, B, key_selector(pk, key_idx), rows(d_r, 64, nullptr, 64), key_rows(pk, pk->N, 64, key_idx), 64,
@@ -345,21 +461,23 @@
 static int paillier_mul_add_enc(mpe_ctx* ctx, const mpe_paillier* pk, int B, const int32_t* key_idx, Rows c_a, Rows k, int kw,
                                 const uint32_t* d_m, const uint32_t* d_r, uint32_t* d_out, hipStream_t st, const uint32_t* x_pre = nullptr) {
   MPE_TRY(ws_begin(ctx, st));
+  const bool pair_x = nn_pair_form(ctx) && (x_pre || ctx->use_multiexp);
   uint32_t* x = ws_array<uint32_t>(ctx, (size_t)B * 128);
-  uint32_t* gm = ws_array<uint32_t>(ctx, (size_t)B * 128);
+  uint32_t* gm = pair_x ? nullptr : ws_array<uint32_t>(ctx, (size_t)B * 128);
   uint32_t* y = ctx->use_multiexp || x_pre ? nullptr : ws_array<uint32_t>(ctx, (size_t)B * 128);
   MPE_TRY(ws_ok(ctx));
   const Rows ksel = key_selector(pk, key_idx), Nrow = key_rows(pk, pk->N, 64, key_idx);
-  MPE_LAUNCH_1D(enc_gm_kernel, B, st, B, pk->nkeys, d_m, key_idx, pk->N, gm);
+  if (!pair_x) MPE_LAUNCH_1D(enc_gm_kernel, B, st, B, pk->nkeys, d_m, key_idx, pk->N, gm);
   if (x_pre) {
     x = const_cast<uint32_t*>(x_pre);
   } else if (ctx->use_multiexp) {
-    MPE_TRY(modexp_nn2(ctx, pk, B, ksel, rows(d_r, 64, nullptr, 64), Nrow, 64, c_a, k, kw, x, st));
+    MPE_TRY(modexp_nn2(ctx, pk, B, ksel, rows(d_r, 64, nullptr, 64), Nrow, 64, c_a, k, kw, x, st, pair_x));
   } else {
     MPE_TRY(modexp_nn(ctx, pk, B, ksel, rows(d_r, 64, nullptr, 64), Nrow, 64, false, x, st));
     MPE_TRY(modexp_nn(ctx, pk, B, ksel, c_a, k, kw, false, y, st));
     MPE_TRY(launch_modmul(ctx, pk->ms_nn, B, ksel, rows(x, 128), rows(y, 128), x, st));
   }
+  if (pair_x) return gamma_finish_nn(ctx, pk, B, ksel, x, rows(d_m, 64), 64, d_out, st);
   return launch_modmul(ctx, pk->ms_nn, B, ksel, rows(x, 128), rows(gm, 128), d_out, st);
 }
 
diff --git a/multi_party_ecdsa_amd/csrc/mpe_pair1024.hip b/multi_party_ecdsa_amd/csrc/mpe_pair1024.hip
--- a/multi_party_ecdsa_amd/csrc/mpe_pair1024.hip
+++ b/multi_party_ecdsa_amd/csrc/mpe_pair1024.hip
@@ -6,8 +6,8 @@
   return pairset_create_impl<Cfg1024>(count, d_moduli, out, st);
 }
 int pair_modexp_1024(mpe_ctx* ctx, const mpe_pairset* ps, int batch, Rows mod_sel, Rows base, Rows exps, int exp_words,
-                     Rows base2, Rows exps2, int exp2_words, int half, uint32_t* out, hipStream_t st, int public_exp) {
-  return pair_modexp_dispatch<1024, 2>(ctx, ps, batch, mod_sel, base, exps, exp_words, base2, exps2, exp2_words, half, out, st, public_exp);
+                     Rows base2, Rows exps2, int exp2_words, int half, uint32_t* out, hipStream_t st, int public_exp, int raw) {
+  return pair_modexp_dispatch<1024, 2>(ctx, ps, batch, mod_sel, base, exps, exp_words, base2, exps2, exp2_words, half, out, st, public_exp, raw);
 }
 
 }
diff --git a/multi_party_ecdsa_amd/csrc/mpe_pair2048.hip b/multi_party_ecdsa_amd/csrc/mpe_pair2048.hip
--- a/multi_party_ecdsa_amd/csrc/mpe_pair2048.hip
+++ b/multi_party_ecdsa_amd/csrc/mpe_pair2048.hip
@@ -6,8 +6,8 @@
   return pairset_create_impl<Cfg2048>(count, d_moduli, out, st);
 }
 int pair_modexp_2048(mpe_ctx* ctx, const mpe_pairset* ps, int batch, Rows mod_sel, Rows base, Rows exps, int exp_words,
-                     Rows base2, Rows exps2, int exp2_words, int half, uint32_t* out, hipStream_t st, int public_exp) {
-  return pair_modexp_dispatch<2048, 4>(ctx, ps, batch, mod_sel, base, exps, exp_words, base2, exps2, exp2_words, half, out, st, public_exp);
+                     Rows base2, Rows exps2, int exp2_words, int half, uint32_t* out, hipStream_t st, int public_exp, int raw) {
+  return pair_modexp_dispatch<2048, 4>(ctx, ps, batch, mod_sel, base, exps, exp_words, base2, exps2, exp2_words, half, out, st, public_exp, raw);
 }
 
 }
diff --git a/multi_party_ecdsa_amd/csrc/mpe_pairexp.h b/multi_party_ecdsa_amd/csrc/mpe_pairexp.h
--- a/multi_party_ecdsa_amd/csrc/mpe_pairexp.h
+++ b/multi_party_ecdsa_amd/csrc/mpe_pairexp.h
@@ -705,7 +705,7 @@
 
 template <class C>
 int pair_modexp_impl(mpe_ctx* ctx, const mpe_pairset* ps, int batch, Rows mod_sel, Rows base, Rows exps, int exp_words,
-                     Rows base2, Rows exps2, int exp2_words, int half, uint32_t* d_out, hipStream_t st, int public_exp) {
+                     Rows base2, Rows exps2, int exp2_words, int half, uint32_t* d_out, hipStream_t st, int public_exp, int raw) {
   const int units = (batch + C::GROUPS - 1) / C::GROUPS;
   const int grid = ladder_grid(ctx, units, ctx->cus * ctx->modexp_waves_per_cu);
   int wb = exp_words <= 8 ? 4 : (exp_words < 48 ? 5 : 6);
@@ -748,7 +748,7 @@
       hipLaunchKernelGGL(pair_slide_audit_kernel, dim3(blocks_for(units, 64)), dim3(64), 0, st, batch, (int)C::GROUPS, exps,
                          exp_words, wb, dual ? exp2_words : 0, perm, ctr);
   }
-  hipLaunchKernelGGL(pair_finish_kernel<C::K32>, dim3(blocks_for(batch, 64)), dim3(64), 0, st, batch, mod_sel, ps->mod_words, d_out);
+  if (!raw) hipLaunchKernelGGL(pair_finish_kernel<C::K32>, dim3(blocks_for(batch, 64)), dim3(64), 0, st, batch, mod_sel, ps->mod_words, d_out);
   hipError_t e = hipGetLastError();
   if (e != hipSuccess) { mpe_set_error("pair_modexp_kernel", e); return MPE_E_HIP; }
   ctx->last.waves = grid;
@@ -762,7 +762,7 @@
 
 template <int BITS, int TPI>
 int pair_modexp_dispatch(mpe_ctx* ctx, const mpe_pairset* ps, int batch, Rows mod_sel, Rows base, Rows exps, int exp_words,
-                         Rows base2, Rows exps2, int exp2_words, int half, uint32_t* out, hipStream_t st, int public_exp) {
+                         Rows base2, Rows exps2, int exp2_words, int half, uint32_t* out, hipStream_t st, int public_exp, int raw) {
   using Base = Cfg<BITS, MPE_W, MPE_L, TPI>;
   using Wide = Cfg<BITS, MPE_W, MPE_L / 2, 2 * TPI>;
   using XWide = Cfg<BITS, MPE_W, 5, 4 * TPI>;
@@ -771,10 +771,10 @@
   const long resident = (long)ctx->cus * ctx->modexp_waves_per_cu * Base::GROUPS / ctx->device_share;
   const int xdiv = ctx->xwide_div;
   if (ctx->adaptive_lanes && xdiv > 0 && (long)xdiv * batch <= resident)
-    return pair_modexp_impl<XWide>(ctx, ps, batch, mod_sel, base, exps, exp_words, base2, exps2, exp2_words, half, out, st, public_exp);
+    return pair_modexp_impl<XWide>(ctx, ps, batch, mod_sel, base, exps, exp_words, base2, exps2, exp2_words, half, out, st, public_exp, raw);
   if (ctx->adaptive_lanes && (long)ctx->wide_div * batch <= resident)
-    return pair_modexp_impl<Wide>(ctx, ps, batch, mod_sel, base, exps, exp_words, base2, exps2, exp2_words, half, out, st, public_exp);
-  return pair_modexp_impl<Base>(ctx, ps, batch, mod_sel, base, exps, exp_words, base2, exps2, exp2_words, half, out, st, public_exp);
-}
-
-}
+    return pair_modexp_impl<Wide>(ctx, ps, batch, mod_sel, base, exps, exp_words, base2, exps2, exp2_words, half, out, st, public_exp, raw);
+  return pair_modexp_impl<Base>(ctx, ps, batch, mod_sel, base, exps, exp_words, base2, exps2, exp2_words, half, out, st, public_exp, raw);
+}
+
+}
diff --git a/multi_party_ecdsa_amd/csrc/mpe_proofs.h b/multi_party_ecdsa_amd/csrc/mpe_proofs.h
--- a/multi_party_ecdsa_amd/csrc/mpe_proofs.h
+++ b/multi_party_ecdsa_amd/csrc/mpe_proofs.h
@@ -199,14 +199,19 @@
     if (rc == MPE_OK) rc = launch_modexp(ctx, ms, B, sel, base, no_rows(), exps, ew, o, st);
     return o;
   }
-  uint32_t* modexp_nn(const mpe_paillier* pk, Rows sel, Rows base, Rows exps, int ew, bool holder, bool pow_n = false) {
+  uint32_t* modexp_nn(const mpe_paillier* pk, Rows sel, Rows base, Rows exps, int ew, bool holder, bool pow_n = false, bool raw = false) {
     uint32_t* o = words(128);
-    if (rc == MPE_OK) rc = mpe::modexp_nn(ctx, pk, B, sel, base, exps, ew, holder, o, st, pow_n);
-    return o;
-  }
-  uint32_t* modexp_nn2(const mpe_paillier* pk, Rows sel, Rows base, Rows exps, int ew, Rows base2, Rows exps2, int ew2) {
+    if (rc == MPE_OK) rc = mpe::modexp_nn(ctx, pk, B, sel, base, exps, ew, holder, o, st, pow_n, nullptr, 0, raw);
+    return o;
+  }
+  uint32_t* modexp_nn2(const mpe_paillier* pk, Rows sel, Rows base, Rows exps, int ew, Rows base2, Rows exps2, int ew2, bool raw = false) {
     uint32_t* o = words(128);
-    if (rc == MPE_OK) rc = mpe::modexp_nn2(ctx, pk, B, sel, base, exps, ew, base2, exps2, ew2, o, st);
+    if (rc == MPE_OK) rc = mpe::modexp_nn2(ctx, pk, B, sel, base, exps, ew, base2, exps2, ew2, o, st, raw);
+    return o;
+  }
+  uint32_t* gamma_finish(const mpe_paillier* pk, Rows sel, const uint32_t* zz, Rows x, int xw, uint32_t* o = nullptr) {
+    if (!o) o = words(128);
+    if (rc == MPE_OK) rc = mpe::gamma_finish_nn(ctx, pk, B, sel, zz, x, xw, o, st);
     return o;
   }
   uint32_t* modexp_n(const mpe_paillier* pk, const int32_t* key_idx, Rows sel, Rows base, Rows exps, int ew) {
@@ -320,29 +325,33 @@
   uint32_t* a1 = q2.fb_modexp(stm, ssel, 0, h1,pr.s1, 25);
   uint32_t* a2 = q2.fb_modexp(stm, ssel, 1, h2,pr.s2, 89);
   uint32_t* a12 = q2.modmul(stm->ms, ssel, rows(a1, 64), rows(a2, 64));
-  uint32_t* gs1 = q.words(128);
-  q.muladd(pr.s1, 25, Nrow, 64, no_rows(), 0, gs1, 128);
+  const bool pf = nn_pair_form(ctx);
+  uint32_t* gs1 = pf ? nullptr : q.words(128);
+  if (!pf) q.muladd(pr.s1, 25, Nrow, 64, no_rows(), 0, gs1, 128);
+  auto gamma_s1 = [&](const uint32_t* pw) {
+    return pf ? q.gamma_finish(pk, ksel, pw, pr.s1, 25) : q.modmul(pk->ms_nn, ksel, rows(gs1, 128), rows(pw, 128));
+  };
   uint32_t *u = nullptr, *b12 = nullptr, *cie = nullptr;
   if (m_pre) {
     inv_ok2 = const_cast<uint8_t*>(inv_ok_pre);
     m_pre.wait(f.s(0));
-    u = q.modmul(pk->ms_nn, ksel, rows(gs1, 128), rows(m_pre.p, 128));
+    u = gamma_s1(m_pre.p);
   } else if (f.on) {
-    uint32_t* sn = q.modexp_nn(pk, ksel, with_words(pr.s, 64), Nrow, 64, false);
-    b12 = q.modmul(pk->ms_nn, ksel, rows(gs1, 128), rows(sn, 128));
+    uint32_t* sn = q.modexp_nn(pk, ksel, with_words(pr.s, 64), Nrow, 64, false, false, pf);
+    b12 = gamma_s1(sn);
     uint32_t* cred = q2.modmul(pk->ms_nn, ksel, cipher, rows(pk->ms_nn->one_words, 0, nullptr, 1));
     uint32_t* cinv = q2.modinv(pk->ms_nn, ksel, rows(cred, 128), inv_ok2);
     cie = q2.modexp_nn(pk, ksel, rows(cinv, 128), pr.e, 8, false);
   } else if (ctx->use_multiexp) {
     uint32_t* cred = q.modmul(pk->ms_nn, ksel, cipher, rows(pk->ms_nn->one_words, 0, nullptr, 1));
     uint32_t* cinv = q.modinv(pk->ms_nn, ksel, rows(cred, 128), inv_ok2);
-    uint32_t* m = q.modexp_nn2(pk, ksel, with_words(pr.s, 64), Nrow, 64, rows(cinv, 128), pr.e, 8);
-    u = q.modmul(pk->ms_nn, ksel, rows(gs1, 128), rows(m, 128));
+    uint32_t* m = q.modexp_nn2(pk, ksel, with_words(pr.s, 64), Nrow, 64, rows(cinv, 128), pr.e, 8, pf);
+    u = gamma_s1(m);
   } else {
     uint32_t* ce = q.modexp_nn(pk, ksel, cipher, pr.e, 8, false);
     uint32_t* cei = q.modinv(pk->ms_nn, ksel, rows(ce, 128), inv_ok2);
-    uint32_t* sn = q.modexp_nn(pk, ksel, with_words(pr.s, 64), Nrow, 64, false);
-    uint32_t* b12n = q.modmul(pk->ms_nn, ksel, rows(gs1, 128), rows(sn, 128));
+    uint32_t* sn = q.modexp_nn(pk, ksel, with_words(pr.s, 64), Nrow, 64, false, false, pf);
+    uint32_t* b12n = gamma_s1(sn);
     u = q.modmul(pk->ms_nn, ksel, rows(b12n, 128), rows(cei, 128));
   }
   f.join();
@@ -426,12 +435,16 @@
     hipLaunchKernelGGL(pdl_u1_check_kernel, dim3(blocks_for(B, 64)), dim3(64), 0, f.s(1), B, pr.s1, e, Gp, Qp, pr.u1, ok);
   }
   uint8_t *inv_ok1 = q.flags(), *inv_ok2 = q.flags();
-  uint32_t* g1 = q.words(128);
-  q.muladd(pr.s1, 25, Nrow, 64, no_rows(), 0, g1, 128);
+  const bool pf = nn_pair_form(ctx);
+  uint32_t* g1 = pf ? nullptr : q.words(128);
+  if (!pf) q.muladd(pr.s1, 25, Nrow, 64, no_rows(), 0, g1, 128);
+  auto gamma_s1 = [&](const uint32_t* pw) {
+    return pf ? q.gamma_finish(pk, ksel, pw, pr.s1, 25) : q.modmul(pk->ms_nn, ksel, rows(g1, 128), rows(pw, 128));
+  };
   uint32_t *u2 = nullptr, *t2s = nullptr, *cies = nullptr;
   if (f.on) {
-    uint32_t* s2n = q.modexp_nn(pk, ksel, with_words(pr.s2, 64), Nrow, 64, false);
-    t2s = q.modmul(pk->ms_nn, ksel, rows(g1, 128), rows(s2n, 128));
+    uint32_t* s2n = q.modexp_nn(pk, ksel, with_words(pr.s2, 64), Nrow, 64, false, false, pf);
+    t2s = gamma_s1(s2n);
     uint32_t* cred = q1.modmul(pk->ms_nn, ksel, cipher, rows(pk->ms_nn->one_words, 0, nullptr, 1));
     uint32_t* cinv = q1.modinv(pk->ms_nn, ksel, rows(cred, 128), inv_ok1);
     cies = q1.modexp_nn(pk, ksel, rows(cinv, 128), rows(e, 8), 8, false);
@@ -439,11 +452,11 @@
     uint32_t* cred = q.modmul(pk->ms_nn, ksel, cipher, rows(pk->ms_nn->one_words, 0, nullptr, 1));
     uint32_t* cinv = q.modinv(pk->ms_nn, ksel, rows(cred, 128), inv_ok1);
     if (ctx->use_multiexp) {
-      uint32_t* m = q.modexp_nn2(pk, ksel, with_words(pr.s2, 64), Nrow, 64, rows(cinv, 128), rows(e, 8), 8);
-      u2 = q.modmul(pk->ms_nn, ksel, rows(g1, 128), rows(m, 128));
+      uint32_t* m = q.modexp_nn2(pk, ksel, with_words(pr.s2, 64), Nrow, 64, rows(cinv, 128), rows(e, 8), 8, pf);
+      u2 = gamma_s1(m);
     } else {
-      uint32_t* s2n = q.modexp_nn(pk, ksel, with_words(pr.s2, 64), Nrow, 64, false);
-      uint32_t* t2 = q.modmul(pk->ms_nn, ksel, rows(g1, 128), rows(s2n, 128));
+      uint32_t* s2n = q.modexp_nn(pk, ksel, with_words(pr.s2, 64), Nrow, 64, false, false, pf);
+      uint32_t* t2 = gamma_s1(s2n);
       uint32_t* cie = q.modexp_nn(pk, ksel, rows(cinv, 128), rows(e, 8), 8, false);
       u2 = q.modmul(pk->ms_nn, ksel, rows(t2, 128), rows(cie, 128));
     }
```

Result: no change. 19330, median of 6 (+0.5%).
